# tvlearn/evo

Measured on AMD Instinct MI355X. Metric: E-step candidate-state evals/sec (NxS), full EM iteration, higher is better.
Workload: dtype f64; 1 GPU; ES3C D=256 H=512 S=200 N=100k f64 (north-star shape); algo=es3c, N_total=100000, N_rank0=100000, D=256, H=512, S=200, step=10 full EM iterations, world_size_rccl=1, ea=fit/randflip 10 parents x 1 child x 1 gen, states=p_init_Kn=1/H (init_states default), rng=device, mstep=device, parallelism=dp1

## Files before the change

evo_amd/_lib.py:

```python
import ctypes
import os

import numpy as np

_HERE = os.path.dirname(os.path.abspath(__file__))
LIB_PATH = os.path.join(_HERE, "libevo_amd.so")

MODEL_BSC, MODEL_SSSC = 0, 1

GEN_KEEP = {"s": 1, "z": 2, "y_mean": 4}
GEN_WHAT = {"y": 0, "s": 1, "z": 2, "y_mean": 3}

SEED_INCOMPLETE = 1

PSAMP_KEEP = {"slot": 1, "s": 2, "z": 4, "y": 8}
PSAMP_WHAT = {"slot": 0, "s": 1, "z": 2, "y": 3}

LLE_WHAT = {"s": 0, "inside": 1, "log_r": 2, "lpj": 3}

VALIDITY_BITS = (
    "have_data", "have_params", "have_cand", "B_valid", "rows_fresh", "stats_rows_valid", "yhat_valid", "rec_resident",
    "yrec_valid", "yrec_from_pass", "rec_in_stats", "keep_x_valid", "rec_uses_keep", "need_known", "res_need0",
    "res_need1", "res_need2", "cand_from_device", "lists_clean", "clist_clean", "acc_clean", "wq_copy_valid",
    "h_theta_fresh", "theta_bak_valid", "kn_lost", "last_estep_fused", "reduce_pending", "bins_dirty", "gen_kept",
    "prefetch_current", "census_current", "rows_kn_current",
)
VALIDITY_WORDS = ("gen", "kn_gen", "theta_gen", "pending_skip", "census_skip", "kn_refill", "pred_N")

KERNEL_IDS = {
    "lpj_resident": 0, "lpj_candidates": 1, "lpj_overflow": 2, "row_lse": 3, "vary_kn": 4,
    "stats": 5, "stats_overflow": 6, "gemm_f64": 7, "evolve": 8, "misc": 9, "mstep_device": 10,
    "lpj_pass": 11, "stats_pass": 12, "lpj_k3_4": 13, "lpj_k5_8": 14, "lpj_k9plus": 15,
    "stats_k3_4": 16, "stats_k5_8": 17, "stats_k9plus": 18, "allreduce": 19, "estep_fused": 20,
    "patches": 21, "init_states": 22,
}
KERNEL_IDS_EXTRA = {"posterior_sample": 23, "seed_states": 24, "loglik_proposal": 25, "loglik_lpj": 26, "loglik_fold": 27,
                    "remap_latents": 28}


def kernel_id(name):
    return KERNEL_IDS[name] if name in KERNEL_IDS else KERNEL_IDS_EXTRA[name]

_c_dp = ctypes.POINTER(ctypes.c_double)
_c_u8p = ctypes.POINTER(ctypes.c_uint8)
_c_i32p = ctypes.POINTER(ctypes.c_int32)
_c_u64p = ctypes.POINTER(ctypes.c_uint64)
_vp = ctypes.c_void_p
_I, _I64, _U64, _DBL = ctypes.c_int, ctypes.c_int64, ctypes.c_uint64, ctypes.c_double

SIGNATURES = {
    "evoamd_abi_version": (_I, []),
    "evoamd_last_error": (ctypes.c_char_p, []),
    "evoamd_device_count": (_I, [ctypes.POINTER(_I)]),
    "evoamd_ctx_create": (_I, [_I, ctypes.POINTER(_vp)]),
    "evoamd_ctx_destroy": (None, [_vp]),
    "evoamd_synchronize": (_I, [_vp]),
    "evoamd_debug_live_buffers": (_I, [ctypes.POINTER(_I64)]),
    "evoamd_debug_validity": (_I, [_vp, ctypes.POINTER(_I64)]),
    "evoamd_set_option": (_I, [_vp, ctypes.c_char_p, _I]),
    "evoamd_configure": (_I, [_vp, _I, _I64, _I, _I, _I, _I, _I]),
    "evoamd_upload_data": (_I, [_vp, _c_dp]),
    "evoamd_upload_states": (_I, [_vp, _c_u8p]),
    "evoamd_download_states": (_I, [_vp, _c_u8p]),
    "evoamd_upload_states_packed": (_I, [_vp, _c_u8p, _I64, _I64]),
    "evoamd_download_states_packed": (_I, [_vp, _c_u8p, _I64, _I64]),
    "evoamd_init_states": (_I, [_vp, _DBL, _U64, _I, _c_u8p]),
    "evoamd_seed_states": (_I, [_vp, _I, _c_i32p, _c_dp]),
    "evoamd_seed_states_ex": (_I, [_vp, _I, ctypes.c_uint, _c_i32p, _c_dp]),
    "evoamd_upload_lpj": (_I, [_vp, _c_dp]),
    "evoamd_download_lpj": (_I, [_vp, _c_dp]),
    "evoamd_set_params_bsc": (_I, [_vp, _c_dp, _DBL, _DBL, _c_dp]),
    "evoamd_set_params_sssc": (_I, [_vp, _c_dp, _c_dp, _c_dp, _c_dp, _DBL, _c_dp]),
    "evoamd_lpj_resident": (_I, [_vp]),
    "evoamd_lpj_candidates": (_I, [_vp, _c_u8p, _c_i32p, _I, _c_dp]),
    "evoamd_set_candidates": (_I, [_vp, _c_u8p, _c_i32p, _I, _c_dp]),
    "evoamd_lpj_shared": (_I, [_vp, _c_u8p, _I, _c_dp]),
    "evoamd_lpj_single": (_I, [_vp, _c_dp, _c_u8p, _I, _c_dp, _c_i32p]),
    "evoamd_vary_kn": (_I, [_vp, _I, _c_dp]),
    "evoamd_evolve_randflip": (_I, [_vp, _I, _I, _U64, _I]),
    "evoamd_estep": (_I, [_vp, _I, _I, _U64, _I, _I, ctypes.POINTER(_I)]),
    "evoamd_estep_counters": (_I, [_vp, ctypes.POINTER(_I64)]),
    "evoamd_evolve_states": (_I, [_vp, _I, _I, _I, _I, _I, _U64, _DBL, _DBL]),
    "evoamd_download_candidates": (_I, [_vp, _c_u8p, _c_i32p, _c_dp]),
    "evoamd_refine_states": (_I, [_vp, _I, _I, _I, _I, _I, _I, _U64, _U64, _DBL, _DBL, _I, _I, _I, _DBL, _c_dp,
                                  ctypes.POINTER(_I)]),
    "evoamd_posterior_scores": (_I, [_vp, _c_dp, _c_dp, _c_i32p, _c_i32p, _c_dp]),
    "evoamd_remap_latents": (_I, [_vp, _c_i32p, _I, _c_i32p, ctypes.POINTER(_I64)]),
    "evoamd_adopt_remapped_states": (_I, [_vp]),
    "evoamd_latent_map_counts": (_I, [_vp, ctypes.POINTER(_I64)]),
    "evoamd_acc_size": (_I64, [_vp]),
# ... 94 lines not shown
```

evo_amd/csrc/evo_amd.hip:

```cpp
#include "../../include/evo_amd.h"

#include <dlfcn.h>
#include <math.h>
#include <stdarg.h>
#include <stdio.h>
#include <stdlib.h>
#include <string.h>

#include <atomic>
#include <chrono>
#include <memory>
#include <string>
#include <type_traits>
#include <vector>

#include "common.hpp"
#include "gemm_f64.hpp"
#include "kernels_bsc.hpp"
#include "kernels_common.hpp"
#include "kernels_evolve.hpp"
#include "kernels_mstep.hpp"
#include "kernels_sssc.hpp"
#include "kernels_sssc_quad.hpp"
#include "kernels_fused.hpp"
// ... 67 lines not shown
    h = dlopen(nm, RTLD_NOW | RTLD_LOCAL);
    if (h) break;
  }
  if (!h) return fail(EVOAMD_E_RCCL, "cannot dlopen librccl: %s", dlerror());
  g_rccl.GetUniqueId = (int (*)(RcclId *))dlsym(h, "ncclGetUniqueId");
  g_rccl.CommInitRank = (int (*)(void **, int, RcclId, int))dlsym(h, "ncclCommInitRank");
  g_rccl.AllReduce =
      (int (*)(const void *, void *, size_t, int, int, void *, hipStream_t))dlsym(h, "ncclAllReduce");
  g_rccl.CommDestroy = (int (*)(void *))dlsym(h, "ncclCommDestroy");
  g_rccl.GetErrorString = (const char *(*)(int))dlsym(h, "ncclGetErrorString");
  if (!g_rccl.GetUniqueId || !g_rccl.CommInitRank || !g_rccl.AllReduce || !g_rccl.CommDestroy)
    return fail(EVOAMD_E_RCCL, "librccl is missing a required symbol");
  g_rccl.handle = h;
  return 0;
}
#define RCCL_TRY(expr)                                                                         \
  do {                                                                                         \
    int _r = (expr);                                                                           \
    if (_r != 0)                                                                               \
      return fail(EVOAMD_E_RCCL, "%s failed: %s", #expr,                                       \
                  g_rccl.GetErrorString ? g_rccl.GetErrorString(_r) : "?");                    \
  } while (0)

enum {
  KID_LPJ_RES = 0,
  KID_LPJ_CAND,
  KID_LPJ_OVF,
  KID_ROW_LSE,
  KID_VARY_KN,
  KID_STATS,
  KID_STATS_OVF,
  KID_GEMM,
  KID_EVOLVE,
  KID_MISC,
  KID_MSTEP,
  KID_LPJ_PASS,
  KID_STATS_PASS,
  KID_LPJ_K34,
  KID_LPJ_K58,
  KID_LPJ_K9P,
  KID_STATS_K34,
  KID_STATS_K58,
  KID_STATS_K9P,
  KID_ALLREDUCE,
  KID_ESTEP_FUSED,
  KID_PATCHES,
  KID_INIT_STATES,
  KID_POSTERIOR_SAMPLE,
  KID_SEED_STATES,
  KID_LLE_PROPOSAL,
  KID_LLE_LPJ,
  KID_LLE_FOLD,
  KID_REMAP,
  KID_COUNT
};

struct TimedSpan {
  hipEvent_t a, b;
  int kid;
};

static int sync_streams(evoamd_ctx *c);
static std::atomic<int64_t> g_live_dev{0}, g_live_pinned{0};

template <typename T>
class DevBuf {
  T *p_ = nullptr;
  size_t n_ = 0;

  hipError_t alloc_raw(size_t n) {
    reset();
    if (n == 0) n = 1;
    hipError_t e = hipMalloc((void **)&p_, n * sizeof(T));
    if (e != hipSuccess) {
      p_ = nullptr;
      return e;
    }
    n_ = n;
    g_live_dev++;
    return hipSuccess;
  }

 public:
  DevBuf() = default;
  DevBuf(const DevBuf &) = delete;
  DevBuf &operator=(const DevBuf &) = delete;
  DevBuf(DevBuf &&o) noexcept : p_(o.p_), n_(o.n_) { o.p_ = nullptr, o.n_ = 0; }
  DevBuf &operator=(DevBuf &&o) noexcept {
    if (this != &o) {
      reset();
      p_ = o.p_, n_ = o.n_;
      o.p_ = nullptr, o.n_ = 0;
    }
    return *this;
  }
  ~DevBuf() { reset(); }
  operator T *() const { return p_; }
  T *get() const { return p_; }
  size_t size() const { return n_; }
  void reset() {
    if (p_) {
      (void)hipFree(p_);
      g_live_dev--;
    }
    p_ = nullptr;
    n_ = 0;
// ... 153 lines not shown
  bool use_digest = true;
  bool spd_inverse = true;
  long spd_fallbacks = 0;
  bool rows_fresh = false;
  int model = 0;
  i64 N = 0;
  int D = 0, H = 0, S = 0, S_perm = 0, Cmax = 0, HW = 0, L = 0;
  DevBuf<double> Y, yy, y2sum;
  int ldY = 0;
  PinnedBuf<double> h_acc, h_par;
  PinnedBuf<double> h_theta;
  double *h_theta_dev = nullptr;
  bool h_theta_fresh = false;
  DevBuf<double> theta_bak;
  bool theta_bak_valid = false;
  unsigned long long mbox_seq = 0;
  DevBuf<unsigned> mbox_counter;
  PinnedBuf<int> h_err;
  DevBuf<u64> states, cand;
  DevBuf<u64> dig, cand_dig;
  DevBuf<double> lpj, cand_lpj;
  DevBuf<double> lpj_alt;
  DevBuf<int> cand_counts;
  DevBuf<u64> cand_raw, dupold;
  DevBuf<int> gen_start;
  DevBuf<unsigned> flags;
  DevBuf<double> rowmax, rowsum, partial, partial2, diag;
  DevBuf<uint8_t> stage;
  DevBuf<double> W, Wt, G, Psi, Bm, mus, pilbar_v;
  DevBuf<double2> GP;
  DevBuf<double4> DG;
  DevBuf<double4> D1;
  DevBuf<PairEntry> PT;
  DevBuf<double> pies;
  double *dpar = nullptr;
  PinnedBuf<double> h_dpar;
  DevBuf<double> colpart;
  DevBuf<double> gjwork;
  DevBuf<double> tmpA, tmpB, tmpC;
  double ljc = 0;
  double *acc = nullptr;
  i64 acc_n = 0;
  DevBuf<double> acc_base;
  i64 ovf_n = 0;
  DevBuf<double> Es_own;
  double *Es = nullptr;
  DevBuf<int> list1, list2, list3, list_n, err;
  DevBuf<int> clist, clist_n;
  size_t clist_words() const { return clist.size() / 3; }
  DevBuf<OvfRec> ovf_rec;
  unsigned long long kn_gen = 1, census_gen = 0;
  int census_opt = 1;
  int merge_small = 1;
  int stats_flat = 0;
  int fused_opt = 0;
  DevBuf<double> rowF;
  DevBuf<int> rowcnt, defer;
  DevBuf<double> fpart;
  DevBuf<unsigned long long> fprof;
  bool last_estep_fused = false;
  bool reduce_pending = false;
  long fused_calls = 0, unfused_calls = 0;
  int debug_poison_list = 0;
  int debug_fail_stats = 0;
  int census_skip = 0;
  DevBuf<double> tmp_y, tmp_lpj;
  DevBuf<u64> tmp_states;
  DevBuf<double> exact_buf;
  DevBuf<double> patch_img, patch_Y;
  DevBuf<double> patch_V;
  DevBuf<double> pred_buf, pred_Wt;
  DevBuf<int> pred_status;
  i64 pred_N = 0;
  int pred_D = 0;
  DevBuf<int> ps_slot, ps_status;
  DevBuf<u64> ps_s;
  DevBuf<double> ps_z, ps_y;
  i64 ps_N = 0, ps_T = 0;
  int ps_D = 0, ps_H = 0, ps_keep = -1;
  DevBuf<double> lle_d, lle_keep_d, lle_rho;
  DevBuf<int> lle_i;
  DevBuf<unsigned> lle_flags;
  DevBuf<u64> lle_keep_s, lle_hash;
  DevBuf<uint8_t> lle_keep_in;
  i64 lle_N = 0, lle_T = 0;
  int lle_H = 0, lle_keep = -1;
  DevBuf<uint8_t> codes_buf;
  unsigned long long rows_kn_gen = 0;
  int codes_path = -1;
  int init_home = -1;
  DevBuf<u64> init_scratch;
  DevBuf<double2> seed_gpt;
  DevBuf<double> seed_rows;
  DevBuf<double> refine_trace, score_buf;
  DevBuf<u64> remap_states, remap_dig;
  DevBuf<int> remap_i;
  DevBuf<unsigned long long> remap_sum, map_counts;
  i64 remap_N = 0;
  int remap_S = 0, remap_H = 0;
  bool kn_lost = false;
  i64 kn_refill = 0;
  DevBuf<double> gen_par, gen_y, gen_z, gen_ymean;
  DevBuf<u64> gen_sin, gen_s;
  i64 gen_N = 0;
  int gen_D = 0, gen_H = 0, gen_keep = -1;
  void *comm = nullptr;
  int rank = 0, world = 1;
  bool timing = false;
  unsigned timing_mask = 0xFFFFFFFFu;
  std::vector<TimedSpan> spans;
  std::vector<hipEvent_t> pool;
  double t_ms[KID_COUNT] = {0};
  i64 t_n[KID_COUNT] = {0};
};

static void drop_stats_products(evoamd_ctx *c) { c->yhat_valid = c->stats_rows_valid = c->rec_resident = c->yrec_from_pass = false; }
static void drop_prefetch(evoamd_ctx *c) { c->prefetch_gen = ~0ull; }
static void made_prefetch(evoamd_ctx *c) { c->prefetch_gen = c->gen; }
static void drop_B(evoamd_ctx *c) { c->B_valid = false; }
static void made_B(evoamd_ctx *c) { c->B_valid = true; }
static int next_theta_stamp(evoamd_ctx *c) { return ++c->theta_gen; }

static void on_configure(evoamd_ctx *c) {
  c->gen++;
  c->kn_gen++;
  c->census_gen = 0;
  c->pending_skip = c->census_skip = 0;
  c->have_data = c->have_params = c->have_cand = c->rows_fresh = c->acc_clean = c->clist_clean = false;
  c->h_theta_fresh = c->theta_bak_valid = c->yrec_valid = c->rec_in_stats = c->keep_x_valid = c->kn_lost = false;
  c->lists_clean = c->need_known = c->cand_from_device = false;
  if (c->model == EVOAMD_MODEL_SSSC) c->last_estep_fused = false;
  drop_stats_products(c);
  c->pred_N = 0;
  c->rel_frac = -1.0;
  c->pays_agreed = -1;
}
static void on_option(evoamd_ctx *c) { c->gen++; }
static void on_option_changes_derived(evoamd_ctx *c) { c->have_params = false; }
static void on_data_uploaded(evoamd_ctx *c) {
  c->have_data = true;
  c->gen++;
  c->B_valid = false;
  c->rec_resident = false;
}
static void on_masks_changed(evoamd_ctx *c, bool present) {
  c->yrec_valid = c->rec_resident = c->yrec_from_pass = false;
  if (present) c->B_valid = false;
}
static void on_yrec_uploaded(evoamd_ctx *c) { c->yrec_valid = true, c->rec_resident = c->yrec_from_pass = false; }
static void on_theta_installed(evoamd_ctx *c) {
  c->have_params = true;
  c->gen++;
  c->h_theta_fresh = false;
  drop_stats_products(c);
}
static void on_theta_update_begun(evoamd_ctx *c) { c->gen++; }
static void on_theta_updated(evoamd_ctx *c, bool backup_rode_along) {
  c->B_valid = false;
  if (backup_rode_along) c->theta_bak_valid = true;
  c->stats_rows_valid = false;
}
static void on_theta_restored(evoamd_ctx *c) {
  c->gen++;
  c->h_theta_fresh = false;
  c->B_valid = false;
  c->have_params = true;
  drop_prefetch(c);
}
static void on_theta_update_failed(evoamd_ctx *c) { c->prefetch_gen = ~0ull, c->have_params = false; }
static void made_theta_backup(evoamd_ctx *c) { c->theta_bak_valid = true; }
static void drop_theta_backup(evoamd_ctx *c) { c->theta_bak_valid = false; }
static void made_theta_mailbox(evoamd_ctx *c, bool holds_theta) { c->h_theta_fresh = holds_theta; }
enum KnBy { KN_BY_CALLER, KN_BY_SELECTION };
static void on_kn_changed(evoamd_ctx *c, KnBy by) {
  c->gen++;
  c->kn_gen++;
  if (by == KN_BY_CALLER) c->need_known = false;
}
static void on_kn_complete(evoamd_ctx *c) { c->kn_lost = false; }
static void on_kn_init_begun(evoamd_ctx *c) {
  c->kn_lost = true, c->kn_refill = 0;
  on_kn_changed(c, KN_BY_CALLER);
}
static void on_kn_rows_uploaded(evoamd_ctx *c, i64 n0, i64 n) {
  on_kn_changed(c, KN_BY_CALLER);
  if (c->kn_lost && n0 <= c->kn_refill && n0 + n > c->kn_refill) {
    c->kn_refill = n0 + n;
    if (c->kn_refill >= c->N) c->kn_lost = false;
  }
}
static void on_estep_route(evoamd_ctx *c, bool fused) { c->last_estep_fused = fused; }
static void on_lpj_overwritten(evoamd_ctx *c) { c->rows_fresh = false; }
static void made_row_stats(evoamd_ctx *c) { c->rows_fresh = true; }
static void on_lists_claimed(evoamd_ctx *c) {
  if (!c->lists_clean) c->pending_skip = 0;
  c->lists_clean = false;
}
static void made_clean_lists(evoamd_ctx *c) {
  c->lists_clean = c->model == EVOAMD_MODEL_SSSC;
  if (c->lists_clean) c->pending_skip = 0;
}
static void on_levels_skipped(evoamd_ctx *c, bool census_route, int skipped, int served, bool any) {
  if (census_route) {
    c->census_skip |= skipped;
    if (any && !(served & 2)) c->pending_skip |= 2;
  } else {
    c->pending_skip = (c->pending_skip | skipped) & ~served;
  }
}
static void made_selection(evoamd_ctx *c, bool census_cleared, bool acc_zeroed) {
  made_row_stats(c);
  if (census_cleared) {
    c->clist_clean = true;
    c->census_skip = 0;
  }
  c->acc_clean = acc_zeroed;
  made_clean_lists(c);
}
static void on_census_claimed(evoamd_ctx *c) { c->clist_clean = false, c->census_skip = 0; }
static void made_census(evoamd_ctx *c) { c->census_gen = c->kn_gen; }
static void on_census_poisoned(evoamd_ctx *c) { c->kn_gen++; }
static void on_cand_installed(evoamd_ctx *c, bool near_parents) { c->cand_from_device = near_parents; }
static void made_cand_lpj(evoamd_ctx *c) { c->have_cand = true; }
static void drop_cand_batch(evoamd_ctx *c) { c->have_cand = false, c->cand_from_device = false; }
static void made_fused_estep(evoamd_ctx *c, bool inkernel_census) {
  on_kn_changed(c, KN_BY_SELECTION);
  if (inkernel_census) made_census(c);
  made_row_stats(c);
  c->have_cand = false, c->cand_from_device = true;
  on_estep_route(c, true);
}
static void made_fused_rows(evoamd_ctx *c, bool reduced) { c->reduce_pending = !reduced; }
static void on_bins_append(evoamd_ctx *c) { c->bins_dirty = true; }
static void made_bins_clean(evoamd_ctx *c) { c->bins_dirty = false; }
static void on_stats_pass_begun(evoamd_ctx *c) {
  c->bins_dirty = false;
  c->acc_clean = false;
  drop_stats_products(c);
}
static void made_stats_rows(evoamd_ctx *c) { c->stats_rows_valid = true, c->rows_kn_gen = c->kn_gen; }
static void made_level_hints(evoamd_ctx *c, const double *dpar_host) {
  if (c->model != EVOAMD_MODEL_SSSC) return;
  for (int j = 0; j < 3; j++) {
    c->res_cnt[j] = dpar_host[DP_NGT2 + j];
    c->res_need[j] = c->res_cnt[j] > 0.0;
  }
  c->need_known = true;
}
static void made_wq_copy(evoamd_ctx *c, bool present) { c->wq_copy_valid = present; }
static void made_yhat(evoamd_ctx *c) { c->yhat_valid = true; }
static void made_yrec_from_pass(evoamd_ctx *c, bool in_stats) {
  c->yrec_valid = c->yrec_from_pass = true;
  if (in_stats) c->rec_in_stats = false;
}
static void drop_resident_rec(evoamd_ctx *c) { c->rec_resident = false; }
static void on_keep_mask(evoamd_ctx *c, bool uploaded) { c->keep_x_valid = uploaded; }
static void made_resident_rec(evoamd_ctx *c, bool uses_keep) { c->rec_uses_keep = uses_keep, c->rec_resident = true; }
static void made_predictive(evoamd_ctx *c, i64 N) { c->pred_N = N; }
static void made_generated(evoamd_ctx *c, int keep) { c->gen_keep = keep; }
static void made_posterior_samples(evoamd_ctx *c, int keep) { c->ps_keep = keep; }
static void made_remap(evoamd_ctx *c, i64 N, int S, int H_new) { c->remap_N = N, c->remap_S = S, c->remap_H = H_new; }
static void made_loglik_draws(evoamd_ctx *c, int keep) { c->lle_keep = keep; }

struct SpanGuard {
  evoamd_ctx *c;
  int kid;
  hipStream_t stream;
  hipEvent_t a = nullptr, b = nullptr;
  SpanGuard(evoamd_ctx *ctx, int k, hipStream_t s = nullptr) : c(ctx), kid(k), stream(s ? s : ctx->stream) {
    if (!c->timing || !((c->timing_mask >> k) & 1u)) return;
    auto get = [&]() {
      hipEvent_t e;
      if (!c->pool.empty()) {
        e = c->pool.back();
        c->pool.pop_back();
      } else {
        (void)hipEventCreate(&e);
      }
      return e;
    };
    a = get();
// ... 45 lines not shown
extern "C" int evoamd_device_count(int *count) {
  REQUIRE(count, "count is NULL");
  int n = 0;
  hipError_t e = hipGetDeviceCount(&n);
  if (e != hipSuccess) {
    *count = 0;
    return fail(EVOAMD_E_NODEVICE, "hipGetDeviceCount: %s", hipGetErrorString(e));
  }
  *count = n;
  return 0;
}

static int set_kernel_lds_limits() {
  HIP_TRY(hipFuncSetAttribute((const void *)sssc_stats_flat_kernel, hipFuncAttributeMaxDynamicSharedMemorySize, 150 * 1024));
  HIP_TRY(hipFuncSetAttribute((const void *)sssc_big_kernel<0>, hipFuncAttributeMaxDynamicSharedMemorySize,
                              136 * 1024));
  HIP_TRY(hipFuncSetAttribute((const void *)sssc_big_kernel<0, 0>, hipFuncAttributeMaxDynamicSharedMemorySize,
                              136 * 1024));
  HIP_TRY(hipFuncSetAttribute((const void *)sssc_big_kernel<0, 1>, hipFuncAttributeMaxDynamicSharedMemorySize,
                              136 * 1024));
  HIP_TRY(hipFuncSetAttribute((const void *)sssc_big_kernel<1>, hipFuncAttributeMaxDynamicSharedMemorySize,
                              136 * 1024));
  HIP_TRY(hipFuncSetAttribute((const void *)posterior_codes_kernel<CODES_LDS>, hipFuncAttributeMaxDynamicSharedMemorySize,
                              CODES_WAVES * CODES_LDS_H * (int)sizeof(double)));
  HIP_TRY(hipFuncSetAttribute((const void *)gemm_tn128_f64, hipFuncAttributeMaxDynamicSharedMemorySize,
                              (int)GEMM128_LDS_BYTES));
  HIP_TRY(hipFuncSetAttribute((const void *)gemm_tn128_rows_f64, hipFuncAttributeMaxDynamicSharedMemorySize,
                              (int)GEMM128_LDS_BYTES));
  HIP_TRY(hipFuncSetAttribute((const void *)gemm_tn128_sk_f64, hipFuncAttributeMaxDynamicSharedMemorySize,
                              (int)GEMM128_LDS_BYTES));
  HIP_TRY(hipFuncSetAttribute((const void *)gemm_tn128_sk_f32, hipFuncAttributeMaxDynamicSharedMemorySize,
                              (int)GEMM128_LDS_BYTES));
  HIP_TRY(hipFuncSetAttribute((const void *)gemm_tn128_store_f32, hipFuncAttributeMaxDynamicSharedMemorySize,
                              (int)GEMM128_LDS_BYTES));
  {
    const int lds = (int)(PRED_WAVES * pred_lds_doubles(PRED_MAX_K, true) * sizeof(double));
    const void *pk[] = {(const void *)predictive_kernel<1, true>, (const void *)predictive_kernel<2, true>,
                        (const void *)predictive_kernel<4, true>, (const void *)predictive_kernel<8, true>};
    for (const void *f : pk) HIP_TRY(hipFuncSetAttribute(f, hipFuncAttributeMaxDynamicSharedMemorySize, lds));
    const void *sk[] = {(const void *)posterior_sample_kernel<1, true>, (const void *)posterior_sample_kernel<2, true>,
                        (const void *)posterior_sample_kernel<4, true>, (const void *)posterior_sample_kernel<8, true>};
    for (const void *f : sk) HIP_TRY(hipFuncSetAttribute(f, hipFuncAttributeMaxDynamicSharedMemorySize, lds));
  }
  HIP_TRY(hipFuncSetAttribute((const void *)remap_latents_kernel, hipFuncAttributeMaxDynamicSharedMemorySize, REMAP_LDS_BYTES));
  HIP_TRY(hipFuncSetAttribute((const void *)seed_states_kernel<true>, hipFuncAttributeMaxDynamicSharedMemorySize, 150 * 1024));
  HIP_TRY(hipFuncSetAttribute((const void *)seed_states_kernel<false>, hipFuncAttributeMaxDynamicSharedMemorySize, 150 * 1024));
  HIP_TRY(hipFuncSetAttribute((const void *)seed_states_masked_kernel<true>, hipFuncAttributeMaxDynamicSharedMemorySize, 150 * 1024));
  HIP_TRY(hipFuncSetAttribute((const void *)seed_states_masked_kernel<false>, hipFuncAttributeMaxDynamicSharedMemorySize, 150 * 1024));
  {
    const void *wk[] = {(const void *)sssc_stats_wave_kernel<0, 4>,  (const void *)sssc_stats_wave_kernel<1, 4>,
                        (const void *)sssc_stats_wave_kernel<2, 4>,  (const void *)sssc_stats_wave_kernel<4, 4>,
                        (const void *)sssc_stats_wave_kernel<8, 4>,  (const void *)sssc_stats_wave_kernel<16, 4>,
                        (const void *)sssc_stats_wave_kernel<0, 1>,  (const void *)sssc_stats_wave_kernel<0, 8>,
                        (const void *)sssc_stats_wave_kernel<0, 16>};
    for (const void *f : wk) HIP_TRY(hipFuncSetAttribute(f, hipFuncAttributeMaxDynamicSharedMemorySize, 150 * 1024));
    HIP_TRY(hipFuncSetAttribute((const void *)pair_bins_reduce_kernel, hipFuncAttributeMaxDynamicSharedMemorySize, 3 * PB_TILE * 8));
    HIP_TRY(hipFuncSetAttribute((const void *)sssc_small_kernel<4, 1, 2, 256>, hipFuncAttributeMaxDynamicSharedMemorySize, 120 * 1024));
    HIP_TRY(hipFuncSetAttribute((const void *)sssc_small_kernel<8, 1, 2, 256>, hipFuncAttributeMaxDynamicSharedMemorySize, 120 * 1024));
  }
  {
    const void *fk[] = {(const void *)sssc_estep_fused_kernel<1, false>,  (const void *)sssc_estep_fused_kernel<1, true>,
                        (const void *)sssc_estep_fused_kernel<2, false>,  (const void *)sssc_estep_fused_kernel<2, true>,
                        (const void *)sssc_estep_fused_kernel<4, false>,  (const void *)sssc_estep_fused_kernel<4, true>,
                        (const void *)sssc_estep_fused_kernel<8, false>,  (const void *)sssc_estep_fused_kernel<8, true>,
                        (const void *)sssc_estep_fused_kernel<16, false>, (const void *)sssc_estep_fused_kernel<16, true>};
    for (const void *fp : fk) HIP_TRY(hipFuncSetAttribute(fp, hipFuncAttributeMaxDynamicSharedMemorySize, 160 * 1024));
  }
  return 0;
}

extern "C" int evoamd_ctx_create(int device, evoamd_ctx **out) {
  REQUIRE(out, "out is NULL");
  int n = 0;
  if (hipGetDeviceCount(&n) != hipSuccess || n <= 0)
    return fail(EVOAMD_E_NODEVICE, "no HIP device visible (libevo_amd needs an MI355X / gfx950 GPU)");
  REQUIRE(device >= 0 && device < n, "device index out of range");
  HIP_TRY(hipSetDevice(device));
  hipDeviceProp_t prop;
  HIP_TRY(hipGetDeviceProperties(&prop, device));
  if (strncmp(prop.gcnArchName, "gfx950", 6) != 0)
    return fail(EVOAMD_E_NODEVICE, "device %d is %s; libevo_amd is built for gfx950 only", device,
                prop.gcnArchName);
  std::unique_ptr<evoamd_ctx> guard(new evoamd_ctx());
  evoamd_ctx *c = guard.get();
  c->device = device;
  c->n_cu = prop.multiProcessorCount > 0 ? prop.multiProcessorCount : 256;
  {
    int prio_lo = 0, prio_hi = 0;
    HIP_TRY(hipDeviceGetStreamPriorityRange(&prio_lo, &prio_hi));
    HIP_TRY(hipStreamCreateWithPriority(&c->stream, hipStreamNonBlocking, prio_hi));
    HIP_TRY(hipStreamCreateWithPriority(&c->stream2, hipStreamNonBlocking, prio_lo));
  }
  HIP_TRY(hipEventCreateWithFlags(&c->ev_fork, hipEventDisableTiming));
  HIP_TRY(hipEventCreateWithFlags(&c->ev_join, hipEventDisableTiming));
  HIP_TRY(hipStreamCreateWithFlags(&c->stream_copy, hipStreamNonBlocking));
  HIP_TRY(hipEventCreateWithFlags(&c->ev_theta, hipEventDisableTiming));
  HIP_TRY(hipEventCreateWithFlags(&c->ev_theta_done, hipEventDisableTiming));
  HIP_TRY(hipEventCreateWithFlags(&c->ev_mbox, hipEventDisableTiming));
  HIP_TRY(hipEventCreateWithFlags(&c->ev_bak, hipEventDisableTiming));
  for (int i = 0; i < 16; i++) HIP_TRY(hipEventCreateWithFlags(&c->ev_chunk[i], hipEventDisableTiming));
  TRY(set_kernel_lds_limits());
  *out = guard.release();
  return 0;
}

static int sync_streams(evoamd_ctx *c) {
  for (hipStream_t s : {c->stream, c->stream2, c->stream_copy})
    if (s) HIP_TRY(hipStreamSynchronize(s));
  return 0;
// ... 61 lines not shown
  const char *err = nullptr;
  void (*after)(evoamd_ctx *) = nullptr;
};
#define OPT_INT(f) &evoamd_ctx::f, nullptr
#define OPT_BOOL(f) nullptr, &evoamd_ctx::f
static int opt_flag(int v) { return v != 0; }
static const OptionRow OPTIONS[] = {
    {"sssc_k8", OPT_INT(k8_mode), [](int v) { return v < 0 ? -1 : (int)(v != 0); }},
    {"ebsc_f32", OPT_BOOL(f32_opt), opt_flag},
    {"bsc_direct", OPT_BOOL(bsc_direct), opt_flag, 0, 0, nullptr, nullptr,
     on_option_changes_derived},
    {"reconstruct_in_stats", OPT_BOOL(rec_in_stats), opt_flag},
    {"codes_path", OPT_INT(codes_path), nullptr, -1, CODES_GMEM, nullptr, "codes_path: -1 (auto), 0 registers, 1 LDS, 2 global memory"},
    {"merge_select_fused", OPT_INT(merge_select_fused), opt_flag},
    {"prefetch_lpj", OPT_BOOL(prefetch_lpj), opt_flag},
    {"inverse_block", OPT_INT(spd_block), nullptr, 0, 0, [](int v) { return v == 0 || v == 16 || v == 32; },
     "inverse_block: 0 (auto), 16 or 32"},
    {"overlap_gemm", OPT_INT(overlap_gemm)},
    {"stats_stage", OPT_INT(stats_stage)},
    {"stats_waves", OPT_INT(stats_waves)},
    {"pair_bins", OPT_INT(pair_bins)},
    {"gemm_streamk", OPT_INT(gemm_streamk)},
    {"b_transposed", OPT_INT(b_tn_opt)},
    {"pair_bins_scale", OPT_INT(bins_scale), nullptr, 1, 64, nullptr, "pair_bins_scale: 1 .. 64"},
    {"pair_bins_nwg", OPT_INT(bins_nwg), nullptr, 0, 0, [](int v) { return v >= 256 && v <= 2048 && (v % 256) == 0; },
     "pair_bins_nwg: 256 .. 2048, multiple of 256"},
    {"pair_bins_auto", OPT_INT(bins_auto), opt_flag},
    {"pair_bins_min", OPT_INT(bins_min)},
    {"bsc_stats_wave", OPT_INT(bsc_wave_opt)},
    {"gemm_workspace", OPT_INT(gemm_ws_opt)},
    {"sssc_precision", OPT_INT(sssc_prec32), [](int v) { return (int)(v == 32); }, 0, 0, [](int v) { return v == 64 || v == 32; },
     "sssc_precision: 64 or 32"},
    {"lpj_main_unstaged", OPT_INT(main_unstaged), opt_flag},
    {"lpj_singular_screen", OPT_INT(sing_screen), nullptr, 0, 2, nullptr, "lpj_singular_screen: 0 (never), 1 (automatic) or 2 (always)"},
    {"gemm_grouped", OPT_INT(gemm_grouped), opt_flag},
    {"gemm_per_xcd", OPT_INT(gemm_per_xcd)},
    {"init_states_home", OPT_INT(init_home), nullptr, -1, 1, nullptr, "init_states_home: -1 (auto), 0 LDS, 1 global memory"},
    {"background_unit", OPT_INT(bg_unit), opt_flag},
    {"fold_clear", OPT_INT(fold_clear), opt_flag},
    {"early_fork", OPT_INT(early_fork)},
    {"merge_small_levels", OPT_INT(merge_small), opt_flag},
    {"stats_flat", OPT_INT(stats_flat), opt_flag},
    {"theta_copy_engine", OPT_INT(theta_copy_engine), opt_flag},
    {"census_lists", OPT_INT(census_opt), opt_flag},
    {"sk_spare", OPT_INT(sk_spare), nullptr, -1, 32, nullptr, "sk_spare: -1 (automatic) or 0 .. 32 workgroups per XCD"},
    {"stats_chunks", OPT_INT(stats_chunks), nullptr, 1, 16, nullptr, "stats_chunks: 1 .. 16"},
    {"mailbox_side_stream", OPT_INT(mbox_side), opt_flag},
    {"fused_estep", OPT_INT(fused_opt), nullptr, 0, 2, nullptr, "fused_estep: 0 (never), 1 (automatic) or 2 (whenever the shape allows it)"},
    {"debug_poison_list", OPT_INT(debug_poison_list), opt_flag},
    {"debug_fail_stats", OPT_INT(debug_fail_stats), opt_flag},
    {"state_digest", OPT_BOOL(use_digest), opt_flag},
    {"inverse_spd", OPT_BOOL(spd_inverse), opt_flag},
};
#undef OPT_INT
#undef OPT_BOOL

extern "C" int evoamd_set_option(evoamd_ctx *c, const char *name, int value) {
  REQUIRE(c && name, "bad arguments");
  on_option(c);
  for (const OptionRow &o : OPTIONS) {
    if (strcmp(name, o.name) != 0) continue;
    if (o.err && !(o.accepts ? o.accepts(value) : (value >= o.lo && value <= o.hi))) return fail(EVOAMD_E_INVALID, "%s", o.err);
    const int v = o.norm ? o.norm(value) : value;
    if (o.ifield) c->*o.ifield = v;
    else c->*o.bfield = v != 0;
    if (o.after) o.after(c);
    return 0;
  }
  return fail(EVOAMD_E_INVALID, "unknown option '%s'", name);
}

static int join_fork(evoamd_ctx *c);

extern "C" int evoamd_synchronize(evoamd_ctx *c) {
  REQUIRE(c, "ctx is NULL");
  TRY(join_fork(c));
  HIP_TRY(hipStreamSynchronize(c->stream));
  return 0;
}

static i64 acc_len(const evoamd_ctx *c) {
  const i64 H = c->H, D = c->D;
  return (c->model == EVOAMD_MODEL_BSC) ? H * D + H * H + H + 1 + 8 : 2 * H + 4 * H * H + D * H + D + 8;
}
struct AccLayout {
  i64 Wp, Wq, pies, sigma;
  i64 xs, xss, xsz, xszsz, s_sz, sz_sz, sWp, y2;
  i64 tail;
};
static AccLayout acc_layout(const evoamd_ctx *c) {
  AccLayout a = {};
  const i64 H = c->H, D = c->D;
  if (c->model == EVOAMD_MODEL_BSC) {
    a.Wp = 0;
    a.Wq = H * D;
    a.pies = a.Wq + H * H;
    a.sigma = a.pies + H;
    a.tail = a.sigma + 1;
  } else {
    a.xs = 0;
    a.xss = H;
    a.xsz = a.xss + H * H;
    a.xszsz = a.xsz + H;
    a.sWp = a.xszsz + H * H;
    a.s_sz = a.sWp + D * H;
    a.sz_sz = a.s_sz + H * H;
    a.y2 = a.sz_sz + H * H;
    a.tail = a.y2 + D;
  }
  return a;
}

static int alloc_pair_bins(evoamd_ctx *c, int scale) {
  const i64 N = c->N;
  const int H = c->H, S = c->S;
  c->pb_ent.reset();
  c->pb_gcnt.reset();
  c->pb_part.reset();
  c->pbins = PairBins{};
  c->bins_scale_cur = 0;
  if (H >= 2 && H <= 1024) {
    PairBins pb = {};
    pb.rf = std::max(1, PB_TILE / (2 * H));
    const int nfold = (H - 1 + 1) / 2;
    pb.nb = (int)cdiv(nfold, pb.rf);
    pb.nwg = c->bins_nwg;
    pb.nsh = std::max((i64)N * S >= (i64)8 << 20 ? 8 : 4, std::min(PB_NSH_MAX, 256 / std::max(1, pb.nb)));
    pb.cap = (int)std::max<i64>(64, (i64)scale * cdiv((i64)N * S, (i64)pb.nb * pb.nwg));
    const size_t ne = (size_t)pb.nb * pb.nwg * pb.cap;
    if (c->pb_ent.try_alloc(ne) && c->pb_part.try_alloc((size_t)pb.nb * pb.nsh * 3 * 2 * pb.rf * H) &&
        c->pb_gcnt.try_alloc((size_t)pb.nb * pb.nwg)) {
      pb.ent = c->pb_ent;
      pb.part = c->pb_part;
      pb.gcnt = c->pb_gcnt;
      HIP_TRY(hipMemsetAsync(pb.gcnt, 0, c->pb_gcnt.size() * sizeof(int), c->stream));
      c->pbins = pb;
      c->bins_scale_cur = scale;
      made_bins_clean(c);
    } else {
      c->pb_ent.reset();
      c->pb_part.reset();
      c->pb_gcnt.reset();
    }
  }
  return 0;
}

static int ensure_bins_capacity(evoamd_ctx *c) {
  if (c->model != EVOAMD_MODEL_SSSC || !c->need_known || !c->pbins.ent || c->bins_auto == 0) return 0;
  const double NS = (double)c->N * c->S;
  const double n34 = c->res_cnt[0] - c->res_cnt[1], n58 = c->res_cnt[1] - c->res_cnt[2];
  const double entries = (NS - c->res_cnt[0]) + 6.0 * n34 + 28.0 * n58;
  int want = (int)std::ceil(3.0 * 1.25 * entries / NS);
  if (want > 64) want = 64;
  if (want <= c->bins_scale_cur) return 0;
  HIP_TRY(hipStreamSynchronize(c->stream));
  if (c->stream2) HIP_TRY(hipStreamSynchronize(c->stream2));
  const int before = c->bins_scale_cur;
  TRY(alloc_pair_bins(c, want));
  if (!c->pbins.ent) {
    TRY(alloc_pair_bins(c, before));
    c->bins_auto = 0;
  }
  return 0;
}

static int configure_validate(const evoamd_ctx *c, int model, i64 N, int D, int H, int S, int S_perm, int Cmax) {
  REQUIRE(model == EVOAMD_MODEL_BSC || model == EVOAMD_MODEL_SSSC, "unknown model");
  REQUIRE(N > 0 && D > 0 && H > 0 && S > 0, "N, D, H, S must be positive");
  REQUIRE(S_perm == 0 || S_perm == 1, "S_perm must be 0 or 1");
  REQUIRE(Cmax >= 1 && Cmax <= 64 * VK_MAX_C_PER_LANE, "Cmax must be in [1, 256]");
  REQUIRE(S <= 64 * VK_MAX_S_PER_LANE, "S must be <= 1024");
  REQUIRE((i64)N * (S > Cmax ? S : Cmax) < 2147483647LL, "N * max(S, Cmax) must fit in int32");
  if (model == EVOAMD_MODEL_BSC && c->f32_opt)
    REQUIRE((H % 4) == 0 && (D % 4) == 0, "float32 mode needs H and D to be multiples of 4 (16-byte rows)");
  return 0;
}

static void configure_geometry(evoamd_ctx *c, int model, i64 N, int D, int H, int S, int S_perm, int Cmax) {
  c->model = model;
  c->N = N;
  c->D = D;
  c->H = H;
  c->S = S;
  c->S_perm = S_perm;
  c->Cmax = Cmax;
  c->HW = (H + 63) / 64;
  c->L = S + S_perm;
  c->ldY = (model == EVOAMD_MODEL_SSSC) ? D + 3 * H : D;
  c->f32 = model == EVOAMD_MODEL_BSC && c->f32_opt;
  c->acc_n = acc_len(c);
  c->pre_n = (model == EVOAMD_MODEL_SSSC) ? 4 + (i64)CS_SLICES * 3 * H : 4 + (i64)BSC_CS_SLICES * H;
  c->ovf_n = c->pre_n + ((model == EVOAMD_MODEL_SSSC) ? 2 * (i64)H * H : 0);
}

static void configure_drop(evoamd_ctx *c) {
  for (DevBuf<uint8_t> *b : {&c->mask_infr, &c->mask_x, &c->keep_x, &c->row_any}) b->reset();
  c->Yrec.reset();
  c->cand_raw.reset();
  c->dupold.reset();
  c->gen_start.reset();
  c->tmpWt.reset();
  c->Wt.reset();
  c->init_scratch.reset();
  c->seed_gpt.reset();
  c->seed_rows.reset();
  c->ps_slot.reset();
  c->ps_status.reset();
  c->ps_s.reset();
  c->ps_z.reset();
  c->ps_y.reset();
  made_posterior_samples(c, -1);
  c->lle_d.reset();
  c->lle_keep_d.reset();
  c->lle_rho.reset();
  c->lle_hash.reset();
  c->lle_i.reset();
  c->lle_flags.reset();
  c->lle_keep_s.reset();
  c->lle_keep_in.reset();
  made_loglik_draws(c, -1);
  c->huge.reset();
  c->huge_ctl.reset();
  c->huge_slots = c->huge_kc = 0;
  for (DevBuf<float> *b : {&c->Yf, &c->Ytf, &c->Wf, &c->Bf, &c->Esf}) b->reset();
  c->Yt.reset();
}

static int configure_alloc_common(evoamd_ctx *c) {
  const size_t N = (size_t)c->N, D = (size_t)c->D, H = (size_t)c->H, S = (size_t)c->S, Cmax = (size_t)c->Cmax, HW = (size_t)c->HW;
  TRY(c->Y.alloc(N * c->ldY));
  TRY(c->yy.alloc(N));
  TRY(c->y2sum.alloc(D));
  TRY(c->states.alloc(N * S * HW));
  TRY(c->cand.alloc(N * Cmax * HW));
  if (H <= DIG_MAX_H) {
    TRY(c->dig.alloc(N * S));
    TRY(c->cand_dig.alloc(N * Cmax));
  } else {
    c->dig.reset();
    c->cand_dig.reset();
  }
  TRY(c->lpj.alloc(N * c->L));
  TRY(c->lpj_alt.alloc(N * c->L));
  TRY(c->cand_lpj.alloc(N * Cmax));
// ... 31 lines not shown
  TRY(c->Wt.alloc(H * D));
  TRY(c->Bm.alloc(c->f32 ? 1 : N * H));
  if (c->f32) {
    c->ldYt = ((c->N + 3) / 4) * 4;
    TRY(c->Yf.alloc(N * D));
    TRY(c->Ytf.alloc(D * c->ldYt));
    TRY(c->Wf.alloc(D * H));
    TRY(c->Bf.alloc(N * H));
    TRY(c->Esf.alloc(N * H));
  }
  return 0;
}

static int configure_alloc_es3c(evoamd_ctx *c) {
  const size_t N = (size_t)c->N, H = (size_t)c->H;
  c->Es_own.reset();
  c->Es = c->Y + c->D;
  TRY(c->Psi.alloc(H * H));
  TRY(c->GP.alloc(H * H));
  TRY(c->DG.alloc(H));
  TRY(c->D1.alloc(H));
  TRY(c->PT.alloc(H * H));
  TRY(c->Bm.alloc(N * H));
  TRY(c->mus.alloc(H));
  TRY(c->pilbar_v.alloc(H));
  TRY(c->pies.alloc(H));
  TRY(c->rowF.alloc(N));
  TRY(c->rowcnt.alloc(N));
  TRY(c->defer.alloc(2 * (N + 1) + 2));
  TRY(c->fpart.alloc((size_t)3 * R3_THREADS));
  if (c->H > SSSC_KCAP) {
    const size_t slot = big_slot_doubles(c->H);
    c->huge_kc = c->H;
    c->huge_slots = (int)std::max<size_t>(1, std::min<size_t>(16, ((size_t)256 << 20) / (slot * sizeof(double))));
    TRY(c->huge.alloc(slot * (size_t)c->huge_slots));
    TRY(c->huge_ctl.alloc((size_t)c->huge_slots));
  }
  return 0;
}

static int configure_alloc_lists(evoamd_ctx *c) {
  const size_t words = list_cap(c->N * (i64)std::max(c->S, c->Cmax)) * LIST_SHARDS;
  TRY(c->list1.alloc(words));
  TRY(c->list2.alloc(words));
  TRY(c->list3.alloc(words));
  TRY(c->list_n.alloc(4 * LIST_SHARDS));
  c->clist.reset();
  c->clist_n.reset();
  c->ovf_rec.reset();
  if (c->census_opt) {
    TRY(c->clist.alloc(3 * list_cap(c->N * (i64)c->S) * LIST_SHARDS));
    TRY(c->clist_n.alloc(4 * LIST_SHARDS));
    TRY(c->ovf_rec.alloc((size_t)c->N * c->S));
  }
  return 0;
}

static int configure_alloc_host(evoamd_ctx *c) {
  const size_t par_n = (size_t)c->D * c->H + (size_t)c->H * c->H + 3 * (size_t)c->H;
  if (!c->h_err) TRY(c->h_err.alloc(4));
  if (!c->h_dpar) TRY(c->h_dpar.alloc(DP_COUNT + 8));
  TRY(c->h_acc.alloc((size_t)c->acc_n + DP_COUNT));
  TRY(c->h_par.alloc(par_n));
  c->h_theta_dev = nullptr;
  TRY(c->h_theta.alloc(par_n + MAILBOX_HDR, hipHostMallocCoherent | hipHostMallocMapped));
  memset(c->h_theta, 0, MAILBOX_HDR * sizeof(double));
  HIP_TRY(hipHostGetDevicePointer((void **)&c->h_theta_dev, c->h_theta, 0));
  if (!c->mbox_counter) {
    TRY(c->mbox_counter.alloc(1));
    HIP_TRY(hipMemset(c->mbox_counter, 0, sizeof(unsigned)));
  }
  return 0;
}

static int configure_clear(evoamd_ctx *c) {
  auto zero = [&](auto &b) { return hipMemsetAsync(b.get(), 0, b.size() * sizeof(*b.get()), c->stream); };
  if (c->huge_ctl) HIP_TRY(zero(c->huge_ctl));
  if (c->Yt) HIP_TRY(zero(c->Yt));
  if (c->f32) HIP_TRY(zero(c->Ytf));
  if (c->model == EVOAMD_MODEL_SSSC) {
    HIP_TRY(zero(c->defer));
    if (c->clist_n) HIP_TRY(zero(c->clist_n));
  }
  HIP_TRY(zero(c->Y));
  HIP_TRY(zero(c->flags));
  HIP_TRY(zero(c->cand_counts));
  HIP_TRY(zero(c->acc_base));
  HIP_TRY(zero(c->err));
  HIP_TRY(hipStreamSynchronize(c->stream));
  return 0;
}

extern "C" int evoamd_configure(evoamd_ctx *c, int model, int64_t N, int D, int H, int S, int S_perm,
                                int Cmax) {
  REQUIRE(c, "ctx is NULL");
  c->configured = false;
  TRY(configure_validate(c, model, N, D, H, S, S_perm, Cmax));
  HIP_TRY(hipSetDevice(c->device));
  configure_geometry(c, model, N, D, H, S, S_perm, Cmax);
  configure_drop(c);
  TRY(configure_alloc_common(c));
  if (model == EVOAMD_MODEL_BSC) {
    TRY(configure_alloc_ebsc(c));
  } else {
    TRY(configure_alloc_es3c(c));
    TRY(configure_alloc_lists(c));
// ... 833 lines not shown
static void with_cpl(int Cmax, F &&f) {
  if (Cmax <= 64) f(std::integral_constant<int, 1>{});
  else f(std::integral_constant<int, 4>{});
}

struct Es3cLists {
  ListOut o1, o2, o3;
  ListIn i1, i2, i3;
  ListIn cA, cB, cC;
  ListIn empty;
  ListOut none_out;
  ListIn none_in;
};

static Es3cLists es3c_lists(const evoamd_ctx *c, int cap) {
  Es3cLists ls = {};
  ls.o1 = {c->list1, c->list_n + 0 * LIST_SHARDS, cap};
  ls.o2 = {c->list2, c->list_n + 1 * LIST_SHARDS, cap};
  ls.o3 = {c->list3, c->list_n + 2 * LIST_SHARDS, cap};
  ls.i1 = {ls.o1.items, ls.o1.counts, cap};
  ls.i2 = {ls.o2.items, ls.o2.counts, cap};
  ls.i3 = {ls.o3.items, ls.o3.counts, cap};
  if (c->clist && c->clist_n) {
    ls.cA = {c->clist, c->clist_n, cap};
    ls.cB = {c->clist + c->clist_words(), c->clist_n + LIST_SHARDS, cap};
    ls.cC = {c->clist + 2 * c->clist_words(), c->clist_n + 2 * LIST_SHARDS, cap};
    ls.empty = {c->clist, c->clist_n + 3 * LIST_SHARDS, 0};
  }
  return ls;
}

template <int MODE, int TAG>
static int census_wavefront_levels(evoamd_ctx *c, const SsscArgs &a, const Es3cLists &ls, const bool need[3], bool few4,
                                   const LevelHints &lv, i64 total) {
  if (few4) {
    sssc_big_kernel<MODE, TAG><<<std::max(64u, level_grid(c, lv, 1, total * 256, 1024, 1)), 64, big_lds(SSSC_KCAP), c->stream>>>(
        a, need[1] ? ls.cB : ls.empty, ls.none_out, SSSC_KCAP, need[2] ? ls.cC : ls.empty, ls.i3);
    return 4;
  }
  sssc_big_kernel<MODE, TAG><<<std::max(256u, level_grid(c, lv, 2, total * 256, 8192, 1)), 64, big_lds(16), c->stream>>>(
      a, need[2] ? ls.cC : ls.empty, ls.o2, 16, ls.i3);
  if (!need[2]) return 4;
  sssc_big_kernel<MODE, TAG><<<level_grid(c, lv, 2, total * 256, 1024, 1), 64, big_lds(SSSC_KCAP), c->stream>>>(
      a, ls.i2, ls.none_out, SSSC_KCAP);
  return 2 | 4;
}

#define MAIN_LPJ_LDS_MAX (48 * 1024)

static size_t main_lpj_lds(int C, int H) {
  return ((size_t)(1024 / C + 2) * H + (H <= 512 ? (size_t)4 * H : 0)) * sizeof(double);
}

enum LpjRoute {
  LPJ_MASKED,
  LPJ_CENSUS,
  LPJ_CHAINS,
  LPJ_ROUND2
};
enum LpjMain {
  LPJ_MAIN_NONE,
  LPJ_MAIN_CENSUS,
  LPJ_MAIN_STAGED,
  LPJ_MAIN_UNSTAGED,
  LPJ_MAIN_SMALL
};

struct LpjPlan {
  LpjRoute route;
  LevelHints lv;
  int kid_main;
  i64 total;
  int cap;
  Es3cLists ls;
  bool need[3];
  bool any;
  LpjMain main;
  int rows_cap, stage_dg;
  size_t lds;
  unsigned grid;
  bool few4;
  bool k8;
  bool few_dense;
};

static void lpj_plan(const evoamd_ctx *c, const SsscArgs &a, int tag, const LevelHints &lv, int kid_main, LpjPlan &p) {
  p = LpjPlan{};
  p.lv = lv;
  p.kid_main = kid_main;
  p.total = a.N * (i64)a.C;
  p.cap = (int)list_cap(p.total);
  p.ls = es3c_lists(c, p.cap);
  levels_for(c, lv, p.need);
  p.any = p.need[0] || p.need[1] || p.need[2];
  const bool tables = !a.shared && (a.H % 2) == 0;
  const bool staged = tables && main_lpj_lds(a.C, a.H) <= MAIN_LPJ_LDS_MAX;
  if (a.mask)
    p.route = LPJ_MASKED;
  else if (tag == 0 && a.states == c->states && census_mode(c) && staged)
    p.route = LPJ_CENSUS;
  else
    p.route = c->census_opt ? LPJ_CHAINS : LPJ_ROUND2;
  p.stage_dg = a.H <= 512;
  p.grid = cdiv(p.total, 1024);
  if (staged) {
    p.main = p.route == LPJ_CENSUS ? (lv.levels_only ? LPJ_MAIN_NONE : LPJ_MAIN_CENSUS) : LPJ_MAIN_STAGED;
    p.rows_cap = 1024 / a.C + 2;
    p.lds = main_lpj_lds(a.C, a.H);
  } else if (tables && a.dig && c->main_unstaged) {
    p.main = LPJ_MAIN_UNSTAGED;
    p.lds = (p.stage_dg ? (size_t)4 * a.H : 0) * sizeof(double);
  } else {
    p.main = LPJ_MAIN_SMALL;
    p.grid = cdiv(p.total, 512);
  }
  p.few4 = p.route != LPJ_ROUND2 && few_above4(c, lv);
  p.k8 = p.route == LPJ_ROUND2 && use_k8_kernel(c, lv);
  p.few_dense = p.route == LPJ_ROUND2 && few_dense_states(c, lv);
}

static int lpj_sssc_masked(evoamd_ctx *c, const SsscArgs &a, const LpjPlan &p) {
  SpanGuard g(c, p.kid_main);
  const int gridm = (int)std::min<i64>(p.total, 65536);
  sssc_big_kernel<0><<<gridm, 64, big_lds(8), c->stream>>>(a, p.ls.none_in, p.ls.o3, 8);
  sssc_big_kernel<0><<<1024, 64, big_lds(SSSC_KCAP), c->stream>>>(a, p.ls.i3, p.ls.none_out, SSSC_KCAP);
  HIP_TRY(hipGetLastError());
  return 0;
}

template <int TAG>
static int lpj_sssc_main(evoamd_ctx *c, const SsscArgs &a, const LpjPlan &p) {
  if (p.main == LPJ_MAIN_NONE) return 0;
  SpanGuard g(c, p.kid_main);
  if (p.main == LPJ_MAIN_SMALL)
    sssc_small_kernel<2, 0, TAG, 512><<<p.grid, 512, 0, c->stream>>>(a, p.ls.none_in, p.ls.o1, PairBins{});
  else
    with_hw(a.HW, [&](auto hw) {
      constexpr int HWT = decltype(hw)::value;
      if (p.main == LPJ_MAIN_CENSUS)
        sssc_main_lpj_kernel<TAG, 512, HWT, 2, false><<<p.grid, 512, p.lds, c->stream>>>(a, p.ls.none_out, p.rows_cap, p.stage_dg);
      else if (p.main == LPJ_MAIN_STAGED)
        sssc_main_lpj_kernel<TAG, 512, HWT, 2><<<p.grid, 512, p.lds, c->stream>>>(a, p.ls.o1, p.rows_cap, p.stage_dg);
      else
        sssc_main_lpj_kernel<TAG, 512, HWT, 2, true, false><<<p.grid, 512, p.lds, c->stream>>>(a, p.ls.o1, 0, p.stage_dg);
    });
  HIP_TRY(hipGetLastError());
  DBG_SYNC(c, p.main == LPJ_MAIN_CENSUS ? "sssc lpj main (census)" : "sssc lpj main");
  return 0;
}

template <int TAG>
static int lpj_sssc_census_levels(evoamd_ctx *c, const SsscArgs &a, const LpjPlan &p, int &served) {
  const Es3cLists &ls = p.ls;
  SpanGuard g(c, KID_LPJ_OVF);
  if (p.need[0]) {
    SpanGuard gl(c, KID_LPJ_K34);
    sssc_quad_kernel<1, 0, TAG><<<quad_grid(c, p.lv, 0, p.total, 2048), 256, 0, c->stream>>>(a, ls.cA, ls.none_out, ls.o3, PairBins{}, nullptr);
  }
  DBG_SYNC(c, "sssc lpj quad level 3..4");
  if (p.need[1] && !p.few4) {
    SpanGuard gl(c, KID_LPJ_K58);
    sssc_quad_kernel<2, 0, TAG><<<quad_grid(c, p.lv, 1, p.total, 2048), 256, 0, c->stream>>>(a, ls.cB, ls.none_out, ls.o3, PairBins{}, nullptr);
  }
  DBG_SYNC(c, "sssc lpj quad level 5..8");
  SpanGuard gl(c, KID_LPJ_K9P);
  served = census_wavefront_levels<0, TAG>(c, a, ls, p.need, p.few4, p.lv, p.total);
  HIP_TRY(hipGetLastError());
  DBG_SYNC(c, p.few4 ? "sssc lpj census levels (merged)" : "sssc lpj census levels");
// ... 3 lines not shown
template <int TAG>
static int lpj_sssc_chain_levels(evoamd_ctx *c, const SsscArgs &a, const LpjPlan &p, int &served) {
  const Es3cLists &ls = p.ls;
  SpanGuard g(c, KID_LPJ_OVF);
  if (p.need[0])
    sssc_quad_kernel<1, 0, TAG><<<quad_grid(c, p.lv, 0, p.total, 2048), 256, 0, c->stream>>>(a, ls.i1, ls.o2, ls.o3, PairBins{}, nullptr);
  DBG_SYNC(c, "sssc lpj chain 3..4");
  if (p.few4) {
    sssc_big_kernel<0, TAG><<<std::max(64u, level_grid(c, p.lv, 1, p.total * 256, 1024, 1)), 64, big_lds(SSSC_KCAP), c->stream>>>(
        a, ls.i2, ls.none_out, SSSC_KCAP, ls.i3);
    served = 2 | 4;
  } else {
    if (p.need[1])
      sssc_quad_kernel<2, 0, TAG><<<quad_grid(c, p.lv, 1, p.total, 2048), 256, 0, c->stream>>>(a, ls.i2, ls.o3, ls.o3, PairBins{}, nullptr);
    DBG_SYNC(c, "sssc lpj chain 5..8");
    sssc_big_kernel<0, TAG><<<level_grid(c, p.lv, 2, p.total * 256, 1024, 1), 64, big_lds(SSSC_KCAP), c->stream>>>(
        a, ls.i3, ls.none_out, SSSC_KCAP);
    served = 4;
  }
  HIP_TRY(hipGetLastError());
  DBG_SYNC(c, p.few4 ? "sssc lpj chain wavefront level (merged)" : "sssc lpj chain wavefront level");
  return 0;
}

template <int TAG>
static int lpj_sssc_round2_levels(evoamd_ctx *c, const SsscArgs &a, const LpjPlan &p, int &served) {
  const Es3cLists &ls = p.ls;
  SpanGuard g(c, KID_LPJ_OVF);
  if (p.need[0])
    sssc_small_kernel<4, 0, TAG, 256><<<level_grid(c, p.lv, 0, p.total, 1024, 256), 256, 0, c->stream>>>(a, ls.i1, ls.o2, PairBins{}, ls.o3);
  DBG_SYNC(c, "sssc lpj K=4 level");
  bool merged23 = false;
  if (p.k8) {
    if (p.need[1])
      sssc_small_kernel<8, 0, TAG, 256><<<level_grid(c, p.lv, 1, p.total, 256, 256), 256, 0, c->stream>>>(a, ls.i2, ls.o3, PairBins{}, ls.o3);
  } else if (p.need[1] && p.few_dense) {
    sssc_big_kernel<0, TAG><<<level_grid(c, p.lv, 1, p.total * 256, 1024, 1), 64, big_lds(SSSC_KCAP), c->stream>>>(
        a, ls.i2, ls.none_out, SSSC_KCAP, ls.i3);
    merged23 = true;
  } else if (p.need[1]) {
    sssc_big_kernel<0, TAG><<<level_grid(c, p.lv, 1, p.total * 256, 4096, 1), 64, big_lds(8), c->stream>>>(a, ls.i2, ls.o3, 8);
  }
  DBG_SYNC(c, "sssc lpj K=8 level");
  if ((p.need[2] || c->sing_screen) && !merged23)
    sssc_big_kernel<0, TAG><<<level_grid(c, p.lv, 2, p.total * 256, 1024, 1), 64, big_lds(SSSC_KCAP), c->stream>>>(
        a, ls.i3, ls.none_out, SSSC_KCAP);
  served = (merged23 || p.need[2] || c->sing_screen) ? 4 : 0;
  HIP_TRY(hipGetLastError());
  DBG_SYNC(c, "sssc lpj wavefront level");
  return 0;
}

template <int TAG>
static int launch_sssc_lpj(evoamd_ctx *c, const SsscArgs &a, int kid_main, const LevelHints &lv) {
  TRY(zero_lists(c));
  LpjPlan p;
  lpj_plan(c, a, TAG, lv, kid_main, p);
  if (p.route == LPJ_MASKED) return lpj_sssc_masked(c, a, p);
  if (p.route == LPJ_CENSUS) TRY(ensure_census(c));
  TRY(lpj_sssc_main<TAG>(c, a, p));
  int served = 0;
  if (p.any)
    TRY(p.route == LPJ_CENSUS   ? lpj_sssc_census_levels<TAG>(c, a, p, served)
        : p.route == LPJ_CHAINS ? lpj_sssc_chain_levels<TAG>(c, a, p, served)
                                : lpj_sssc_round2_levels<TAG>(c, a, p, served));
  on_levels_skipped(c, p.route == LPJ_CENSUS, skip_mask(p.need), served, p.any);
  return 0;
}

static int launch_lpj(evoamd_ctx *c, const Batch &b, const LevelHints &lv) {
  if (c->model == EVOAMD_MODEL_BSC) return launch_bsc_lpj(c, b);
  SsscArgs a = sssc_args(c, b);
  if (b.tag == 0) return launch_sssc_lpj<0>(c, a, b.kid, lv);
  if (b.tag == 1) return launch_sssc_lpj<1>(c, a, b.kid, lv);
  return launch_sssc_lpj<2>(c, a, b.kid, lv);
}

static int check_err(evoamd_ctx *c) {
  int *e = c->h_err;
  HIP_TRY(hipMemcpyAsync(e, c->err, 4 * sizeof(int), hipMemcpyDeviceToHost, c->stream));
  HIP_TRY(hipStreamSynchronize(c->stream));
  if (e[0]) {
    HIP_TRY(hipMemsetAsync(c->err, 0, sizeof(int), c->stream));
    if (e[0] & 4) return fail(EVOAMD_E_INVALID, "internal: an ES3C overflow level was skipped although its list was not empty");
    if (e[0] & EVO_ERR_LIST_FULL) return fail(EVOAMD_E_INVALID, "internal: an ES3C overflow list was full, states were dropped");
    if (e[0] & EVO_ERR_BAD_ENTRY) return fail(EVOAMD_E_INVALID, "internal: an ES3C list entry or latent index read back from LDS was out of range");
    if (e[0] & 1) return fail(EVOAMD_E_KLIMIT, "ES3C: a state has more than %d active latents", SSSC_KCAP);
    return fail(EVOAMD_E_SINGULAR, "ES3C: exactly singular k x k system (the reference takes pinv here)");
  }
  return 0;
}

static int lpj_resident_launch(evoamd_ctx *c, double *out, const LevelHints &lv) {
  TRY(ensure_B(c));
  on_lpj_overwritten(c);
  if (c->S_perm) {
    allzero_lpj_kernel<<<cdiv(c->N, 256), 256, 0, c->stream>>>(c->yy, c->N, c->dpar, c->model == EVOAMD_MODEL_SSSC,
                                                               out, c->L, c->flags + 2 * c->N, c->err);
    HIP_TRY(hipGetLastError());
  }
  Batch b = {c->states, nullptr, c->Y, c->Bm, c->yy, c->N, c->S, 0, out, c->L, c->S_perm, c->flags, KID_LPJ_RES, 0};
  b.mask = c->mask_infr;
  SpanGuard pass(c, KID_LPJ_PASS);
  return launch_lpj(c, b, lv);
}

static int estep_resident_pass(evoamd_ctx *c) {
  if (c->prefetch_gen == c->gen) {
    drop_prefetch(c);
    std::swap(c->lpj, c->lpj_alt);
// ... 107 lines not shown
  TRY(c->tmp_lpj.ensure(c, (size_t)C + 2));
  TRY(c->tmp_y.ensure(c, (size_t)c->D + c->H + 2));
  TRY(c->stage.ensure(c, (size_t)C * c->H));
  if (c->model == EVOAMD_MODEL_SSSC) TRY(ensure_lists(c, C));
  double *dy = c->tmp_y, *db = c->tmp_y + c->D, *dyy = c->tmp_y + c->D + c->H;
  unsigned *dfl = (unsigned *)(c->tmp_lpj + C);
  HIP_TRY(hipMemcpyAsync(dy, y, (size_t)c->D * sizeof(double), hipMemcpyHostToDevice, c->stream));
  uint8_t *dmask = nullptr;
  if (x_infr) {
    TRY(c->stage.ensure(c, (size_t)C * c->H + c->D));
    dmask = c->stage + (size_t)C * c->H;
    HIP_TRY(hipMemcpyAsync(dmask, x_infr, (size_t)c->D, hipMemcpyHostToDevice, c->stream));
    mask_apply_kernel<<<cdiv(c->D, 256), 256, 0, c->stream>>>(dy, c->D, dmask, 1, c->D);
  }
  HIP_TRY(hipMemcpyAsync(c->stage, states_bool, (size_t)C * c->H, hipMemcpyHostToDevice, c->stream));
  HIP_TRY(hipMemsetAsync(dfl, 0, sizeof(unsigned), c->stream));
  pack_states_kernel<<<cdiv((i64)C * c->HW, 256), 256, 0, c->stream>>>(c->stage, c->tmp_states, C, c->H, c->HW);
  row_sqnorm_kernel<<<1, 256, 0, c->stream>>>(dy, c->D, 1, c->D, dyy);
  if (c->model == EVOAMD_MODEL_SSSC) TRY(launch_gemm_nn(c, dy, c->D, c->W, c->H, db, c->H, 1, c->H, c->D));
  Batch b = {c->tmp_states, nullptr, dy, db, dyy, 1, C, 1, c->tmp_lpj, C, 0, dfl, KID_MISC, 2};
  b.mask = dmask;
  TRY(launch_lpj(c, b, batch_hints(c, b.tag)));
  unsigned fl = 0;
  HIP_TRY(hipMemcpyAsync(lpj_out, c->tmp_lpj, (size_t)C * sizeof(double), hipMemcpyDeviceToHost, c->stream));
  HIP_TRY(hipMemcpyAsync(&fl, dfl, sizeof(unsigned), hipMemcpyDeviceToHost, c->stream));
  HIP_TRY(hipStreamSynchronize(c->stream));
  if (flags_out) {
    flags_out[0] = (fl & EVO_FLAG_NAN) ? 1 : 0;
    flags_out[1] = (fl & EVO_FLAG_NEGINF) ? 1 : 0;
    flags_out[2] = (fl & (EVO_FLAG_NEGINF | EVO_FLAG_POSINF)) ? 1 : 0;
  }
  if (c->model == EVOAMD_MODEL_SSSC) return check_err(c);
  return 0;
}

extern "C" int evoamd_lpj_single(evoamd_ctx *c, const double *y, const uint8_t *states_bool, int C,
                                 double *lpj_out, int32_t *flags_out) {
  return lpj_single_impl(c, y, nullptr, states_bool, C, lpj_out, flags_out);
}

extern "C" int evoamd_lpj_single_masked(evoamd_ctx *c, const double *y, const uint8_t *x_infr,
                                        const uint8_t *states_bool, int C, double *lpj_out, int32_t *flags_out) {
  REQUIRE(x_infr, "x_infr is NULL");
  return lpj_single_impl(c, y, x_infr, states_bool, C, lpj_out, flags_out);
}

static int estep_select(evoamd_ctx *c, int Mprime, double *sums_out) {
  on_kn_changed(c, KN_BY_SELECTION);
  {
    SpanGuard g(c, KID_VARY_KN);
    int *cl_n = census_mode(c) ? c->clist_n : nullptr;
    const i64 zero_n = c->fold_clear ? (i64)(c->ovf_n + c->acc_n) : 0;
    if (!c->fold_clear) cl_n = nullptr;
    with_spl(c->S, [&](auto spl) {
      with_cpl(c->Cmax, [&](auto cpl) {
        vary_kn_kernel<decltype(spl)::value, decltype(cpl)::value><<<cdiv(c->N, 4), 256, 0, c->stream>>>(
            c->states, c->lpj, c->cand, c->cand_lpj, c->cand_counts, c->N, c->S, c->S_perm, c->HW, c->Cmax, Mprime, c->rowmax,
            c->rowsum, c->partial, c->list_n, 4 * LIST_SHARDS, c->dig, c->cand_dig, (c->use_digest && c->dig) ? 1 : 0,
            c->pending_skip, c->err, cl_n, 4 * LIST_SHARDS, c->census_skip, c->acc_base, zero_n);
      });
    });
    reduce3_partials_kernel<<<1, R3_THREADS, 0, c->stream>>>(c->partial, cdiv(c->N, 4), c->dpar);
    HIP_TRY(hipGetLastError());
    DBG_SYNC(c, "vary_kn");
    made_selection(c, cl_n != nullptr, zero_n > 0);
  }
  if (sums_out) {
    HIP_TRY(hipMemcpyAsync(sums_out, c->dpar + DP_ECNT0, 2 * sizeof(double), hipMemcpyDeviceToHost, c->stream));
    HIP_TRY(hipStreamSynchronize(c->stream));
  }
  return 0;
}

extern "C" int evoamd_vary_kn(evoamd_ctx *c, int Mprime, double *sums_out) {
  REQUIRE(c && c->configured && c->have_cand, "no resident candidate batch (call lpj_candidates / evolve first)");
  TRY(estep_check_mprime(c, Mprime));
  REQUIRE_KN(c);
  HIP_TRY(hipSetDevice(c->device));
  return estep_select(c, Mprime, sums_out);
}

extern "C" int evoamd_set_estep_counts(evoamd_ctx *c, double sum_nunique, double sum_sub) {
  REQUIRE(c && c->configured, "configure first");
  HIP_TRY(hipSetDevice(c->device));
  double v[2] = {sum_nunique, sum_sub};
  HIP_TRY(hipMemcpyAsync(c->dpar + DP_ECNT0, v, sizeof(v), hipMemcpyHostToDevice, c->stream));
  HIP_TRY(hipStreamSynchronize(c->stream));
  return 0;
}

static int estep_children(evoamd_ctx *c, int n_parents, int n_children, uint64_t seed, int fit_parents) {
  {
    SpanGuard g(c, KID_EVOLVE);
    with_spl(c->S, [&](auto spl) {
      evolve_randflip_kernel<decltype(spl)::value><<<cdiv(c->N, 4), 256, 0, c->stream>>>(
          c->states, c->lpj, c->N, c->S, c->S_perm, c->H - c->bg_unit, c->HW, n_parents, n_children, c->Cmax, seed, fit_parents,
          c->cand, c->cand_counts, c->list_n, c->model == EVOAMD_MODEL_SSSC ? 4 * LIST_SHARDS : 0, c->cand_dig, c->pending_skip,
          c->err);
    });
    HIP_TRY(hipGetLastError());
    DBG_SYNC(c, "evolve");
    made_clean_lists(c);
    on_cand_installed(c, true);
  }
  TRY(eval_candidates(c));
  made_cand_lpj(c);
  return 0;
}

extern "C" int evoamd_evolve_randflip(evoamd_ctx *c, int n_parents, int n_children, uint64_t seed, int fit_parents) {
  TRY(estep_check_randflip(c, n_parents, n_children));
  REQUIRE_KN(c);
  HIP_TRY(hipSetDevice(c->device));
  return estep_children(c, n_parents, n_children, seed, fit_parents);
}

static bool fused_shape_ok(const evoamd_ctx *c, int n_parents, int n_children) {
  return c->model == EVOAMD_MODEL_SSSC && c->S_perm == 0 && !c->bg_unit && !c->mask_infr && c->use_digest && c->dig && census_mode(c) &&
// ... 493 lines not shown
  if (c->ar_gemm_pending) {
    c->ar_gemm_pending = false;
    const AccLayout a = acc_layout(c);
    SpanGuard g(c, KID_ALLREDUCE);
    RCCL_TRY(g_rccl.AllReduce(c->acc + a.sWp, c->acc + a.sWp, (size_t)(a.y2 - a.sWp),  8,  0,
                              c->comm, c->stream));
  }
  return 0;
}

static TailArgs make_tail_args(evoamd_ctx *c, const AccLayout &a, i64 N, bool census, int skipped) {
  TailArgs ta = {};
  ta.tail = c->acc + a.tail;
  ta.N = (double)N;
  ta.dpar = c->dpar;
  ta.flags = c->flags;
  ta.nflags3 = 3 * N;
  ta.nper = N;
  ta.err = c->err;
  ta.list_n = c->model == EVOAMD_MODEL_SSSC ? (census ? c->clist_n : c->list_n) : nullptr;
  ta.nshards = LIST_SHARDS;
  ta.skipped_mask = skipped;
  ta.census = c->census;
  ta.census_lists = census ? 1 : 0;
  ta.fly_n = (census && c->model == EVOAMD_MODEL_SSSC) ? c->list_n : nullptr;
  ta.fly_skip = c->pending_skip;
  return ta;
}

static double contraction_flops(const evoamd_ctx *c) {
  return c->model == EVOAMD_MODEL_SSSC ? 2.0 * (double)c->N * (c->D + 2.0 * c->H) * c->H : 2.0 * (double)c->N * c->D * c->H;
}

struct StatsPlan {
  AccLayout a;
  i64 N;
  int H, D;
  bool masked;
  LevelHints lv;
  bool gemm_timed;
  double gemm_flops;
  bool pays;
  bool early;
  bool fork_gemm;
  i64 rpb;
  int nblk;
  int nchunks;
  i64 rows_per_chunk;
  bool second_stream;
  int gemm_spare;
  int waves;
  bool census;
  bool bsc_wave;
};

struct StatsBlock {
  int ci;
  i64 n0, nc;
  int blk0, nblk_c;
};

struct StatsFlow {
  bool early_recorded = false;
  bool tail_done = false;
  bool served3 = false;
  int skipped = 0;
  int bsc_grid = 0;
  PairBins bsc_pb = {};
  PairBins pb = {};
};

struct Es3cPass {
  double *Es, *Ez, *Ed;
  SsscArgs sa = {};
  bool need[3] = {true, true, true};
  Es3cLists ls = {};
};

struct Es3cBlock {
  SsscArgs sc;
  i64 total;
  LevelHints lv;
  int flatG = 0;
  size_t flat_lds = 0;
  bool few4;
};

static bool stats_bins_pay(const evoamd_ctx *c) {
  return c->pbins.ent && (c->pair_bins == 2 || (c->pair_bins == 1 && c->N * (i64)c->S >= (i64)c->bins_min * 1024));
}

static int stats_per_cu(size_t lds_per_wg, int wave_lim) {
  int per_cu = (int)((160 * 1024) / lds_per_wg);
  if (per_cu > wave_lim) per_cu = wave_lim;
  if (per_cu > 8) per_cu = 8;
  if (per_cu < 1) per_cu = 1;
  return per_cu;
}

static int rows_written(evoamd_ctx *c, const StatsPlan &p, StatsFlow &fl) {
  if (p.second_stream && p.nchunks == 1 && p.early && !p.masked) {
    HIP_TRY(hipEventRecord(c->ev_chunk[0], c->stream));
    fl.early_recorded = true;
  }
  return 0;
}

static int reconstruct_rows(evoamd_ctx *c, const char *asked_msg = nullptr) {
  TRY(compute_reconstruction(c));
  if (asked_msg) REQUIRE(c->rec_in_stats, asked_msg);
  select_rec_kernel<<<cdiv(c->N, 4), 256, 0, c->stream>>>(c->Y, c->ldY, c->mask_x, c->mask_infr, c->yhat, c->N, c->D, c->Yrec);
  HIP_TRY(hipGetLastError());
  made_yrec_from_pass(c, true);
  return 0;
}

static int stats_plan(evoamd_ctx *c, bool fork_gemm, StatsPlan &p) {
  p = StatsPlan{};
  p.a = acc_layout(c);
  p.N = c->N;
  p.H = c->H;
  p.D = c->D;
  p.masked = c->mask_infr != nullptr;
  p.lv.known_tag = c->cand_from_device ? 1 : 2;
  p.lv.one_bit = c->cand_from_device;
  p.gemm_timed = c->timing && (c->timing_mask & ((1u << KID_MSTEP) | (1u << KID_MISC) |
                                                 (1u << KID_STATS) | (1u << KID_STATS_OVF)));
  const double gemm_flops = p.gemm_flops = contraction_flops(c);
  bool pays = (c->model == EVOAMD_MODEL_SSSC && gemm_flops >= 8e9) || (c->model == EVOAMD_MODEL_BSC && !c->comm && gemm_flops >= 5e10);
  const bool early = p.early = c->early_fork == 1 || (c->early_fork < 0 && gemm_flops < 2e10);
  if (c->model == EVOAMD_MODEL_SSSC && !c->comm && early && gemm_flops >= 5e8 && !c->mask_infr) pays = true;
  if (c->model == EVOAMD_MODEL_BSC && !c->comm && early && gemm_flops >= 5e8 && !c->mask_infr && c->bsc_wave_opt &&
      dig_for(c, c->states) && cdiv(c->S, 64) <= 4 && (size_t)5 * c->H * sizeof(double) <= 150 * 1024 && !c->f32)
    pays = true;
  if (c->comm && c->model == EVOAMD_MODEL_SSSC) {
    if (c->pays_agreed < 0) {
      double v = pays ? 1.0 : 0.0;
      TRY(evoamd_comm_allreduce_host(c, &v, 1, 1));
      c->pays_agreed = v > 0.0 ? 1 : 0;
    }
    pays = c->pays_agreed == 1;
  }
  p.pays = pays;
  p.fork_gemm = fork_gemm && (c->overlap_gemm == 2 || (c->overlap_gemm == 1 && pays)) &&
                (!c->comm || c->model == EVOAMD_MODEL_SSSC) && !p.gemm_timed && !c->mask_infr;
  p.rpb = ((std::max<i64>(256, cdiv(p.N, 128)) + 3) / 4) * 4;
  p.nblk = (int)cdiv(p.N, p.rpb);
  int nchunks = 1;
  if (!p.masked && !p.gemm_timed && c->overlap_gemm != 0 && c->stats_chunks > 1 && (gemm_flops >= 8e9 || c->overlap_gemm == 2))
    nchunks = std::min<int>(c->stats_chunks, p.nblk);
  p.waves = (c->stats_waves == 4 || c->stats_waves == 8 || c->stats_waves == 16)
                ? c->stats_waves
                : ((size_t)(4 * 2 + 3) * p.H * sizeof(double) <= 150 * 1024 ? 4 : 1);
  p.census = census_mode(c) && !p.masked && p.waves == 4;
  if (p.census) nchunks = 1;
  p.rows_per_chunk = (i64)cdiv(p.nblk, nchunks) * p.rpb;
  p.nchunks = nchunks = (int)cdiv(p.N, p.rows_per_chunk);
  p.second_stream = p.fork_gemm || nchunks > 1;
  {
    const double chain_us = c->H >= 256 ? 15.0 * cdiv(c->H, 32) : 8.5 * cdiv(c->H, 16);
    p.gemm_spare = !(p.fork_gemm && nchunks == 1) ? 0 : ((gemm_flops / 65e6 >= 3.0 * chain_us && c->H <= 512) ? 4 : 8);
  }
  const int SRb = (int)cdiv(c->S, 64);
  p.bsc_wave = c->model == EVOAMD_MODEL_BSC && c->bsc_wave_opt && dig_for(c, c->states) &&
               (SRb == 1 || SRb == 2 || SRb == 4 || SRb == 3) && nchunks == 1 && (size_t)5 * p.H * sizeof(double) <= 150 * 1024;
  return 0;
}

static int stats_bsc_wave(evoamd_ctx *c, const StatsPlan &p, const StatsBlock &blk, StatsFlow &fl) {
  const AccLayout &a = p.a;
  const i64 nc = blk.nc;
  const int H = p.H;
  const u64 *bdig = dig_for(c, c->states);
  const int SRb = (int)cdiv(c->S, 64);
  SpanGuard g(c, KID_STATS);
  const size_t ldsb = (size_t)5 * H * sizeof(double);
  const int per_cu = stats_per_cu(ldsb + 2048, 8);
  PairBins &bsc_pb = fl.bsc_pb;
  bsc_pb = PairBins{};
  if (stats_bins_pay(c)) bsc_pb = c->pbins;
  int sgrid = (int)std::min<i64>(cdiv(nc, 4), (i64)c->n_cu * per_cu * 2);
  if (sgrid > 2048) sgrid = 2048;
  if (bsc_pb.ent && sgrid > bsc_pb.nwg) sgrid = bsc_pb.nwg;
  PB_GRID_CHECK(bsc_pb, sgrid);
  if (bsc_pb.ent) on_bins_append(c);
  fl.bsc_grid = sgrid;
  void *EsP = c->f32 ? (void *)c->Esf : (void *)c->Es;
  double *csb = c->acc_base + 4;
#define BSC_WAVE(SR)                                                                                                      \
  bsc_stats_wave_kernel<SR><<<sgrid, 256, ldsb, c->stream>>>(c->states, c->lpj, c->rowmax, c->rowsum, c->yy, nc, c->S,     \
                                                            c->S_perm, H, c->HW, c->dpar, EsP, c->acc + a.Wq, c->partial2, \
                                                            bdig, c->f32 ? 1 : 0, bsc_pb, csb)
  if (SRb == 1) BSC_WAVE(1);
  else if (SRb == 2) BSC_WAVE(2);
  else BSC_WAVE(4);
#undef BSC_WAVE
  HIP_TRY(hipGetLastError());
  DBG_SYNC(c, "bsc stats (wave)");
  TRY(rows_written(c, p, fl));
  if (bsc_pb.ent) {
    pair_bins_reduce_kernel<<<bsc_pb.nb * bsc_pb.nsh, PB_RTHREADS, (size_t)3 * 2 * bsc_pb.rf * H * sizeof(double), c->stream>>>(
        bsc_pb, H, 0);
    HIP_TRY(hipGetLastError());
    made_bins_clean(c);
  }
  return 0;
}

static int stats_bsc_classic(evoamd_ctx *c, const StatsPlan &p, const StatsBlock &blk) {
  const AccLayout &a = p.a;
  const i64 n0 = blk.n0, nc = blk.nc;
  const int H = p.H;
  {
    SpanGuard g(c, KID_STATS);
    with_hw(c->HW, [&](auto hw) {
      bsc_stats_kernel<decltype(hw)::value><<<cdiv(nc, 4), 256, (size_t)4 * H * sizeof(double), c->stream>>>(
          c->states + (size_t)n0 * c->S * c->HW, c->lpj + (size_t)n0 * c->L, c->rowmax + n0, c->rowsum + n0, c->yy + n0, nc,
          c->S, c->S_perm, H, c->HW, c->dpar,
          c->f32 ? (void *)(c->Esf + (size_t)n0 * H) : (void *)(c->Es + (size_t)n0 * H), c->acc + a.Wq, c->partial2 + n0 / 4,
          dig_for(c, c->states) ? dig_for(c, c->states) + (size_t)n0 * c->S : nullptr, c->f32 ? 1 : 0);
    });
    HIP_TRY(hipGetLastError());
    DBG_SYNC(c, "bsc stats");
  }
  {
    SpanGuard g(c, KID_MISC);
    if (c->f32)
      colsum_partial_f32_kernel<<<dim3(cdiv(H, 64), blk.nblk_c), 256, 0, c->stream>>>(c->Esf + (size_t)n0 * H, H, nc, H, p.rpb,
                                                                                      c->colpart + (size_t)blk.blk0 * H);
    else
      colsum_partial_kernel<<<dim3(cdiv(H, 64), blk.nblk_c), 256, 0, c->stream>>>(c->Es + (size_t)n0 * H, H, nc, H, p.rpb,
                                                                                  c->colpart + (size_t)blk.blk0 * H);
    HIP_TRY(hipGetLastError());
  }
  return 0;
}

static int stats_bsc_block(evoamd_ctx *c, const StatsPlan &p, const StatsBlock &blk, StatsFlow &fl, const double *&Ywp, int &ldwp) {
  TRY(p.bsc_wave ? stats_bsc_wave(c, p, blk, fl) : stats_bsc_classic(c, p, blk));
  if (p.masked) {
    if (c->rec_in_stats) {
      TRY(reconstruct_rows(c));
    }
    REQUIRE(c->yrec_valid, "incomplete data: the M-step needs y_reconstructed (bsc.py:186); reconstruct or upload it");
    Ywp = c->Yrec;
    ldwp = p.D;
  }
  return 0;
}

static int stats_sssc_masked_block(evoamd_ctx *c, const StatsPlan &p, const Es3cPass &ep) {
  const i64 N = p.N;
  const int H = p.H;
  const i64 total = N * (i64)c->S;
// ... 46 lines not shown
static int stats_sssc_census_quads(evoamd_ctx *c, const StatsPlan &p, const Es3cPass &ep, const Es3cBlock &eb, StatsFlow &fl) {
  const bool *need = ep.need;
  const PairBins &pb = fl.pb;
  TRY(ensure_census(c));
  if (need[0] || need[1]) {
    SpanGuard g(c, KID_STATS_OVF);
    const unsigned gcap = pb.ent ? (unsigned)std::min(2048, pb.nwg) : 2048u;
    const size_t dl = (size_t)p.H * sizeof(double);
    if (need[0]) {
      SpanGuard gl(c, KID_STATS_K34);
      const unsigned qg = quad_grid(c, eb.lv, 0, eb.total, gcap);
      PB_GRID_CHECK(pb, qg);
      sssc_quad_kernel<1, 1, 2><<<qg, 256, dl, c->stream>>>(eb.sc, ep.ls.cA, ep.ls.none_out, ep.ls.o3, pb, c->ovf_rec);
    }
    if (need[1] && !eb.few4) {
      SpanGuard gl(c, KID_STATS_K58);
      const unsigned qg = quad_grid(c, eb.lv, 1, eb.total, gcap);
      PB_GRID_CHECK(pb, qg);
      sssc_quad_kernel<2, 1, 2><<<qg, 256, dl, c->stream>>>(eb.sc, ep.ls.cB, ep.ls.none_out, ep.ls.o3, pb, c->ovf_rec);
    }
    HIP_TRY(hipGetLastError());
    DBG_SYNC(c, "sssc stats quad levels");
  }
  return 0;
}

static int stats_sssc_main(evoamd_ctx *c, const StatsPlan &p, const Es3cPass &ep, const Es3cBlock &eb, const StatsBlock &blk,
                           StatsFlow &fl) {
  const PairBins &pb = fl.pb;
  const SsscArgs &sc = eb.sc;
  const ListOut &o1 = ep.ls.o1;
  const i64 nc = blk.nc;
  const int H = p.H;
  const bool census = p.census;
  if (eb.flatG >= 1) {
    SpanGuard g(c, KID_STATS);
    int fgrid = (int)std::min<i64>(cdiv(nc, eb.flatG), (i64)c->n_cu);
    if (pb.ent && fgrid > pb.nwg) fgrid = pb.nwg;
    PB_GRID_CHECK(pb, fgrid);
    sssc_stats_flat_kernel<<<fgrid, FLAT_T, eb.flat_lds, c->stream>>>(sc, pb, c->ovf_rec, eb.flatG);
    HIP_TRY(hipGetLastError());
    DBG_SYNC(c, "sssc stats main (flat)");
    return 0;
  }
  const int Wv = p.waves;
  size_t lds = (size_t)(Wv * 2 + 3) * H * sizeof(double);
  const size_t lds_static = 1024 + (size_t)Wv * 512 + 128;
  REQUIRE(lds <= 150 * 1024, "ES3C statistics: H too large for the LDS rows (H <= 3800)");
  const size_t lds_staged = lds + (size_t)(Wv + 4) * H * sizeof(double);
  const int stage = (H % 2) == 0 && 2 * (lds_staged + lds_static) <= 160 * 1024 && c->stats_stage != 0;
  if (stage) lds = lds_staged;
  const int per_cu = stats_per_cu(lds + lds_static, 32 / Wv);
  SpanGuard g(c, KID_STATS);
  int sgrid = (int)std::min<i64>(cdiv(nc, Wv), (i64)c->n_cu * per_cu * 4);
  if (pb.ent && sgrid > pb.nwg) sgrid = pb.nwg;
  PB_GRID_CHECK(pb, sgrid);
  auto wave4 = [&](auto hw) {
    constexpr int HWT = decltype(hw)::value;
    if (census)
      sssc_stats_wave_kernel<HWT, 4, true><<<sgrid, 256, lds, c->stream>>>(sc, o1, pb, stage, c->ovf_rec, eb.few4 ? 4 : 8);
    else
      sssc_stats_wave_kernel<HWT, 4><<<sgrid, 256, lds, c->stream>>>(sc, o1, pb, stage);
  };
  REQUIRE(!census || Wv == 4, "census lists need the 4-wave statistics kernel (option stats_waves)");
  if (Wv == 1) {
    sssc_stats_wave_kernel<0, 1><<<sgrid, 64, lds, c->stream>>>(sc, o1, pb, stage);
  } else if (Wv == 8) {
    sssc_stats_wave_kernel<0, 8><<<sgrid, 512, lds, c->stream>>>(sc, o1, pb, stage);
  } else if (Wv == 16) {
    sssc_stats_wave_kernel<0, 16><<<sgrid, 1024, lds, c->stream>>>(sc, o1, pb, stage);
  } else if (!stage || !sc.dig) {
    wave4(std::integral_constant<int, 0>{});
  } else {
    with_hw(c->HW, wave4);
  }
  HIP_TRY(hipGetLastError());
  DBG_SYNC(c, "sssc stats main");
  return 0;
}

static int stats_sssc_census_levels(evoamd_ctx *c, const Es3cPass &ep, const Es3cBlock &eb) {
  const bool *need = ep.need;
  if (need[0] || need[1] || need[2]) {
    SpanGuard g(c, KID_STATS_OVF);
    SpanGuard gl(c, KID_STATS_K9P);
    const int served = census_wavefront_levels<1, 2>(c, eb.sc, ep.ls, need, eb.few4, eb.lv, eb.total);
    on_levels_skipped(c, true, 0, served, true);
    HIP_TRY(hipGetLastError());
    DBG_SYNC(c, "sssc stats wavefront level (census)");
  }
  return 0;
}

static int stats_sssc_chain_levels(evoamd_ctx *c, const StatsPlan &p, const Es3cPass &ep, const Es3cBlock &eb, StatsFlow &fl) {
  const bool *need = ep.need;
  const PairBins &pb = fl.pb;
  const SsscArgs &sc = eb.sc;
  const i64 total = eb.total;
  const LevelHints &lv = eb.lv;
  if (need[0] || need[1] || need[2]) {
    SpanGuard g(c, KID_STATS_OVF);
    const size_t cs_lds = sc.cs ? (size_t)3 * p.H * sizeof(double) : 0;
    bool merged23 = false;
    if (need[0]) {
      const unsigned g4 = pb_clamp(pb, level_grid(c, lv, 0, total, 1024, 256));
      PB_GRID_CHECK(pb, g4);
      sssc_small_kernel<4, 1, 2, 256><<<g4, 256, cs_lds, c->stream>>>(sc, ep.ls.i1, ep.ls.o2, pb, ep.ls.o3);
    }
    if (c->k8_mode == 1) {
      if (need[1]) {
        const unsigned g8 = pb_clamp(pb, level_grid(c, lv, 1, total, 256, 256));
        PB_GRID_CHECK(pb, g8);
        sssc_small_kernel<8, 1, 2, 256><<<g8, 256, cs_lds, c->stream>>>(sc, ep.ls.i2, ep.ls.o3, pb, ep.ls.o3);
      }
    } else if (need[1] && few_dense_states(c, lv)) {
      sssc_big_kernel<1><<<level_grid(c, lv, 1, total * 256, 1024, 1), 64, big_lds(SSSC_KCAP), c->stream>>>(
          sc, ep.ls.i2, ep.ls.none_out, SSSC_KCAP, ep.ls.i3);
      fl.served3 = true;
      merged23 = true;
    } else if (need[1]) {
      sssc_big_kernel<1><<<level_grid(c, lv, 1, total * 256, 4096, 1), 64, big_lds(8), c->stream>>>(sc, ep.ls.i2, ep.ls.o3, 8);
    }
    if ((need[2] || c->sing_screen) && !merged23) {
      sssc_big_kernel<1><<<level_grid(c, lv, 2, total * 256, 1024, 1), 64, big_lds(SSSC_KCAP), c->stream>>>(
          sc, ep.ls.i3, ep.ls.none_out, SSSC_KCAP);
      fl.served3 = true;
    }
    HIP_TRY(hipGetLastError());
    DBG_SYNC(c, "sssc stats overflow levels");
  }
  return 0;
}

static int stats_sssc_block(evoamd_ctx *c, const StatsPlan &p, const Es3cPass &ep, const StatsBlock &blk, StatsFlow &fl,
                            bool debug_fail) {
  PairBins &pb = fl.pb;
  const Es3cBlock eb = sssc_block_setup(c, p, ep, blk);
  if (pb.ent) on_bins_append(c);
  if (blk.ci > 0) {
    census_lists_kernel<<<1, 256, 0, c->stream>>>(c->list_n, LIST_SHARDS, skip_mask(ep.need), c->err, c->census);
    HIP_TRY(hipGetLastError());
  }
  if (eb.flatG >= 1 && pb.ent) {
    const i64 per_bin = (i64)pb.nwg * pb.cap;
    pb.nwg = std::min(pb.nwg, c->n_cu);
    pb.cap = (int)std::min<i64>(per_bin / pb.nwg, 1 << 30);
  }
  if (p.census) TRY(stats_sssc_census_quads(c, p, ep, eb, fl));
  TRY(stats_sssc_main(c, p, ep, eb, blk, fl));
  if (debug_fail)
    return fail(EVOAMD_E_INVALID, "debug_fail_stats: statistics pass stopped after its main kernel");
  TRY(p.census ? stats_sssc_census_levels(c, ep, eb) : stats_sssc_chain_levels(c, p, ep, eb, fl));
  TRY(rows_written(c, p, fl));
  if (pb.ent) {
    SpanGuard g(c, KID_STATS);
    pair_bins_reduce_kernel<<<pb.nb * pb.nsh, PB_RTHREADS, (size_t)3 * 2 * pb.rf * p.H * sizeof(double), c->stream>>>(pb, p.H, blk.ci > 0);
    HIP_TRY(hipGetLastError());
    made_bins_clean(c);
    DBG_SYNC(c, "pair bins reduce");
  }
  fl.skipped = skip_mask(ep.need) & ~(fl.served3 ? 4 : 0);
  return 0;
}

static int stats_finish(evoamd_ctx *c, const StatsPlan &p, const Es3cPass &ep, StatsFlow &fl) {
  const AccLayout &a = p.a;
  const i64 N = p.N;
  const int H = p.H, D = p.D;
  const bool masked = p.masked;
  SpanGuard g(c, KID_MISC);
  if (c->model == EVOAMD_MODEL_BSC) {
    TailArgs ta = {};
    if (p.nchunks == 1 && !masked && !c->reduce_pending) {
      ta = make_tail_args(c, a, N, false, fl.skipped);
      fl.tail_done = true;
    }
    double *wq_copy = (!c->comm && !masked && c->tmpA) ? c->tmpA : nullptr;
    made_wq_copy(c, wq_copy != nullptr);
    const unsigned fgrid = cdiv((i64)H * H, 256) + (fl.tail_done ? 1 : 0);
    if (p.bsc_wave)
      bsc_finish_kernel<<<fgrid, 256, 0, c->stream>>>(c->acc + a.Wq, c->acc + a.pies, c->acc_base + 4, BSC_CS_SLICES, H,
                                                       c->partial2, fl.bsc_grid, c->acc + a.sigma, fl.bsc_pb, ta, wq_copy);
    else
      bsc_finish_kernel<<<fgrid, 256, 0, c->stream>>>(c->acc + a.Wq, c->acc + a.pies, c->colpart, p.nblk, H, c->partial2,
                                                       cdiv(N, 4), c->acc + a.sigma, PairBins{}, ta, wq_copy);
  } else {
    const SsscArgs &sa = ep.sa;
    const i64 nthr = (i64)H * H > D ? (i64)H * H : D;
    TailArgs ta = {};
    if (p.nchunks == 1 && !masked && !c->reduce_pending) {
      ta = make_tail_args(c, a, N, p.census, fl.skipped);
      fl.tail_done = true;
    }
    sssc_finish_kernel<<<cdiv(nthr, 256) + (fl.tail_done ? 1 : 0), 256, 0, c->stream>>>(
        c->acc + a.xss, c->acc + a.xszsz, c->acc + a.xs, c->acc + a.xsz, masked ? c->colpart : sa.cs,
        masked ? p.nblk : CS_SLICES, H, c->y2sum, c->acc + a.y2, D, sa.xss_o, sa.xszsz_o, masked ? nullptr : c->PT, fl.pb, ta);
  }
  HIP_TRY(hipGetLastError());
  DBG_SYNC(c, "colsum + finish");
  return 0;
}

static int stats_contract_block(evoamd_ctx *c, const StatsPlan &p, const Es3cPass &ep, const StatsBlock &blk, const StatsFlow &fl,
                                const double *Ywp, int ldwp) {
  const AccLayout &a = p.a;
  const i64 n0 = blk.n0, nc = blk.nc;
  const int H = p.H, D = p.D, ci = blk.ci;
  GemmTnOpts o;
  if (p.second_stream) {
    if (!fl.early_recorded) HIP_TRY(hipEventRecord(c->ev_chunk[ci], c->stream));
    HIP_TRY(hipStreamWaitEvent(c->stream2, c->ev_chunk[ci], 0));
    o.stream = c->stream2;
    o.spare = c->sk_spare >= 0 ? c->sk_spare : p.gemm_spare;
  }
  o.c_is_zero = true;
  o.accumulate = p.nchunks > 1;
  o.mirror = ci == p.nchunks - 1;
  if (c->model == EVOAMD_MODEL_BSC && c->f32)
    return launch_gemm_tn_f32(c, c->Esf + (size_t)n0 * H, H, c->Yf + (size_t)n0 * D, D, c->acc + a.Wp, D, H, D, nc, o);
  if (c->model == EVOAMD_MODEL_BSC)
    return launch_gemm_tn(c, c->Es + (size_t)n0 * H, H, Ywp + (size_t)n0 * ldwp, ldwp, c->acc + a.Wp, D, H, D, nc, o);
  o.sym_row0 = ((D + H) % GEMM_BM) == 0 ? D + H : -1;
  return launch_gemm_tn(c, c->Y + (size_t)n0 * c->ldY, c->ldY, ep.Ez + (size_t)n0 * c->ldY, c->ldY, c->acc + a.sWp, H,
                        D + 2 * H, H, nc, o);
}

static int stats_sssc_masked_products(evoamd_ctx *c, const StatsPlan &p, const Es3cPass &ep) {
  const AccLayout &a = p.a;
  const int H = p.H, D = p.D;
  TRY(reconstruct_rows(c, "ES3C on incomplete data needs do_reconstruction in every step (sssc.py:630-633)"));
  GemmTnOpts o;
  o.c_is_zero = true;
  o.sym_row0 = (H % GEMM_BM) == 0 ? H : -1;
  TRY(launch_gemm_tn(c, ep.Es, c->ldY, ep.Ez, c->ldY, c->acc + a.sWp + (size_t)D * H, H, 2 * H, H, p.N, o));
  o.sym_row0 = -1;
  return launch_gemm_tn(c, c->Yrec, D, ep.Ez, c->ldY, c->acc + a.sWp, H, D, H, p.N, o);
}

static int stats_epilogue(evoamd_ctx *c, const StatsPlan &p, const StatsFlow &fl) {
  const AccLayout &a = p.a;
  const i64 N = p.N;
  if (p.second_stream) {
    HIP_TRY(hipEventRecord(c->ev_join, c->stream2));
    if (p.fork_gemm)
      c->gemm_forked = true;
    else
      HIP_TRY(hipStreamWaitEvent(c->stream, c->ev_join, 0));
  }
  TRY(flush_reduce(c));
  {
    SpanGuard g(c, KID_MISC);
    if (!fl.tail_done) tail_kernel<<<1, 256, 0, c->stream>>>(make_tail_args(c, a, N, p.census, fl.skipped));
    HIP_TRY(hipGetLastError());
    DBG_SYNC(c, "stats contraction + tail");
    made_clean_lists(c);
    if (c->model == EVOAMD_MODEL_SSSC && c->mask_infr) {
      masked_sqsum_kernel<<<256, 256, 0, c->stream>>>(c->yhat, c->mask_infr, N * (i64)p.D, c->acc + a.tail + 7);
      HIP_TRY(hipGetLastError());
    }
  }
  if (c->comm && c->gemm_forked) {
    SpanGuard g(c, KID_ALLREDUCE);
    RCCL_TRY(g_rccl.AllReduce(c->acc, c->acc, (size_t)a.sWp,  8,  0, c->comm, c->stream));
    RCCL_TRY(g_rccl.AllReduce(c->acc + a.y2, c->acc + a.y2, (size_t)(c->acc_n - a.y2), 8, 0, c->comm, c->stream));
    c->ar_gemm_pending = true;
  } else if (c->comm) {
    SpanGuard g(c, KID_ALLREDUCE);
    RCCL_TRY(g_rccl.AllReduce(c->acc, c->acc, (size_t)c->acc_n,  8,  0, c->comm, c->stream));
  }
  return 0;
}

static int stats_sssc_pass(evoamd_ctx *c, const StatsPlan &p, Es3cPass &ep) {
  const AccLayout &a = p.a;
  const i64 N = p.N;
  const int H = p.H, D = p.D;
  ep.Es = c->model == EVOAMD_MODEL_SSSC ? c->Y + D : c->Es;
  ep.Ez = c->Y + D + H;
  ep.Ed = c->Y + D + 2 * H;
  if (c->model != EVOAMD_MODEL_SSSC) return 0;
  SsscArgs &sa = ep.sa;
  Batch b = {c->states, nullptr, c->Y, c->Bm, c->yy, N, c->S, 0, nullptr, c->L, c->S_perm, c->flags, KID_STATS, 0};
  b.mask = c->mask_infr;
  sa = sssc_args(c, b);
  sa.lpj_in = c->lpj;
  sa.rowmax = c->rowmax;
  sa.rowsum = c->rowsum;
  sa.Es = ep.Es;
  sa.Ez = ep.Ez;
  sa.Ed = ep.Ed;
  sa.ldE = c->ldY;
  sa.xss = c->acc + a.xss;
  sa.xszsz = c->acc + a.xszsz;
  sa.xss_o = c->acc_base + c->pre_n;
  sa.xszsz_o = c->acc_base + c->pre_n + (size_t)H * H;
  if (!p.masked) sa.cs = c->acc_base + 4;
  ep.ls = es3c_lists(c, (int)list_cap(N * (i64)c->S));
  levels_for(c, p.lv, ep.need);
  return zero_lists(c);
}

static int stats_compute(evoamd_ctx *c, bool fork_gemm = false) {
  REQUIRE(c && c->configured && c->have_data && c->have_params, "configure, upload_data and set_params first");
  REQUIRE_KN(c);
  StatsPlan p;
  TRY(stats_plan(c, fork_gemm, p));
  TRY(join_fork(c));
  HIP_TRY(hipSetDevice(c->device));
  TRY(ensure_bins_capacity(c));
  if (c->bins_dirty && c->pbins.gcnt)
    HIP_TRY(hipMemsetAsync(c->pbins.gcnt, 0, (size_t)c->pbins.nb * c->pbins.nwg * sizeof(int), c->stream));
  const bool debug_fail = c->debug_fail_stats != 0;
  c->debug_fail_stats = 0;
  if (!c->acc_clean)
    HIP_TRY(hipMemsetAsync(c->acc_base, 0, (size_t)(c->ovf_n + c->acc_n) * sizeof(double), c->stream));
  on_stats_pass_begun(c);
  TRY(ensure_B(c));
  if (!c->rows_fresh) {
    TRY(row_lse(c, c->lpj, p.N, c->L, c->rowmax, c->rowsum, c->dpar + DP_FS));
  }
  StatsFlow fl;
  std::unique_ptr<SpanGuard> pass(new SpanGuard(c, KID_STATS_PASS));
  TRY(c->colpart.ensure(c, (size_t)p.nblk * (c->model == EVOAMD_MODEL_BSC ? p.H : 3 * p.H)));
  Es3cPass ep;
  TRY(stats_sssc_pass(c, p, ep));
  const double *Ywp = c->Y;
  int ldwp = c->ldY;
  if (c->model == EVOAMD_MODEL_SSSC && !p.masked && stats_bins_pay(c)) fl.pb = c->pbins;
  for (int ci = 0; ci < p.nchunks; ci++) {
    const i64 n0 = (i64)ci * p.rows_per_chunk;
    const i64 nc = std::min<i64>(p.rows_per_chunk, p.N - n0);
    const StatsBlock blk = {ci, n0, nc, (int)(n0 / p.rpb), (int)cdiv(nc, p.rpb)};
    TRY(c->model == EVOAMD_MODEL_BSC ? stats_bsc_block(c, p, blk, fl, Ywp, ldwp)
        : p.masked                   ? stats_sssc_masked_block(c, p, ep)
                                     : stats_sssc_block(c, p, ep, blk, fl, debug_fail));
    if (ci == p.nchunks - 1) {
      TRY(stats_finish(c, p, ep, fl));
      pass.reset();
    }
    if (c->model == EVOAMD_MODEL_SSSC && p.masked) continue;
    TRY(stats_contract_block(c, p, ep, blk, fl, Ywp, ldwp));
  }
  if (c->model == EVOAMD_MODEL_SSSC && p.masked) TRY(stats_sssc_masked_products(c, p, ep));
  TRY(stats_epilogue(c, p, fl));
  made_stats_rows(c);
  return 0;
}

extern "C" int evoamd_stats(evoamd_ctx *c, double *acc_out) {
  REQUIRE(acc_out, "acc_out is NULL");
  TRY(stats_compute(c));
  HIP_TRY(hipMemcpyAsync(c->h_acc, c->acc, ((size_t)c->acc_n + DP_COUNT) * sizeof(double), hipMemcpyDeviceToHost,
                         c->stream));
  const int r = check_err(c);
  if (c->sssc_prec32 && c->model == EVOAMD_MODEL_SSSC) {
    const AccLayout a = acc_layout(c);
    for (i64 i = 0; i < a.sWp; i++) c->h_acc[i] = (double)(float)c->h_acc[i];
    for (i64 i = a.s_sz; i < a.y2; i++) c->h_acc[i] = (double)(float)c->h_acc[i];
  }
  memcpy(acc_out, c->h_acc, (size_t)c->acc_n * sizeof(double));
  if (!r) made_level_hints(c, c->h_acc + c->acc_n);
  return r;
}

static int launch_inverse_pivoted(evoamd_ctx *c, double *A, double *B, int n) {
  if (n <= GJR_N) {
    gj_inverse_reg_kernel<<<B ? 2 : 1, MS_T, 0, c->stream>>>(A, B, n, c->dpar + DP_STATUS);
    HIP_TRY(hipGetLastError());
    return 0;
  }
  double *mats[2] = {A, B};
  const dim3 ugrid(cdiv(n, 64), cdiv(n, 64));
  if (n <= 1024) {
    const int nmat = B ? 2 : 1;
    GjMats gm;
    gm.a[0] = A;
    gm.a[1] = B ? B : A;
    gm.w[0] = c->gjwork;
    gm.w[1] = c->gjwork + (size_t)n * n;
    double *Dp = c->gjwork + (size_t)2 * n * n;
    double *Pn = Dp + (size_t)64 * n;
// ... 1590 lines not shown
  TRY(d.alloc((size_t)n));
  HIP_TRY(hipMemcpyAsync(d, buf, (size_t)n * sizeof(double), hipMemcpyHostToDevice, c->stream));
  int rc = g_rccl.AllReduce(d, d, (size_t)n, 8, op == 1 ? 2 : 0, c->comm, c->stream);
  if (rc != 0) return fail(EVOAMD_E_RCCL, "ncclAllReduce failed: %s", g_rccl.GetErrorString ? g_rccl.GetErrorString(rc) : "?");
  HIP_TRY(hipMemcpyAsync(buf, d, (size_t)n * sizeof(double), hipMemcpyDeviceToHost, c->stream));
  HIP_TRY(hipStreamSynchronize(c->stream));
  return 0;
}

extern "C" int evoamd_comm_destroy(evoamd_ctx *c) {
  REQUIRE(c, "ctx is NULL");
  if (c->comm) {
    HIP_TRY(hipStreamSynchronize(c->stream));
    RCCL_TRY(g_rccl.CommDestroy(c->comm));
    c->comm = nullptr;
    c->world = 1;
    c->rank = 0;
  }
  return 0;
}

extern "C" int evoamd_timing_enable(evoamd_ctx *c, int on) {
  REQUIRE(c, "ctx is NULL");
  if (!on && c->timing) TRY(resolve_spans(c));
  c->timing = on != 0;
  c->timing_mask = (unsigned)on;
  return 0;
}

extern "C" int evoamd_timing_reset(evoamd_ctx *c) {
  REQUIRE(c, "ctx is NULL");
  TRY(resolve_spans(c));
  for (int i = 0; i < KID_COUNT; i++) {
    c->t_ms[i] = 0;
    c->t_n[i] = 0;
  }
  return 0;
}

extern "C" int evoamd_kernel_time_ms(evoamd_ctx *c, int kid, double *avg_ms, int64_t *launches) {
  REQUIRE(c && kid >= 0 && kid < KID_COUNT, "bad kernel id");
  TRY(resolve_spans(c));
  if (avg_ms) *avg_ms = c->t_n[kid] ? c->t_ms[kid] / (double)c->t_n[kid] : 0.0;
  if (launches) *launches = c->t_n[kid];
  return 0;
}

extern "C" const char *evoamd_kernel_name(int kid) {
  static const char *names[KID_COUNT] = {"lpj_resident", "lpj_candidates", "lpj_overflow", "row_lse",  "vary_kn",
                                         "stats",        "stats_overflow", "gemm_f64",     "evolve",   "misc", "mstep_device",
                                         "lpj_pass",     "stats_pass",     "lpj_k3_4",     "lpj_k5_8", "lpj_k9plus",
                                         "stats_k3_4",   "stats_k5_8",     "stats_k9plus", "allreduce",    "estep_fused",
                                         "patches",      "init_states",    "posterior_sample", "seed_states",
                                         "loglik_proposal", "loglik_lpj",  "loglik_fold",     "remap_latents"};
  return (kid >= 0 && kid < KID_COUNT) ? names[kid] : "?";
}
```

evo_amd/csrc/kernels_common.hpp:

```cpp
#pragma once
#include "common.hpp"
#include "kernels_mstep.hpp"

__device__ __forceinline__ void clear_lists_checked(int *__restrict__ list_n, int n_list, int skipped_mask,
                                                    int *__restrict__ err) {
  const int per = n_list / 4;
  for (int i = threadIdx.x; i < n_list; i += blockDim.x) {
    if (skipped_mask && list_n[i] != 0 && ((skipped_mask >> (i / per)) & 1)) atomicOr(err, 4);
    list_n[i] = 0;
  }
}

__global__ __launch_bounds__(256) void census_lists_kernel(int *__restrict__ list_n, int nshards, int skipped_mask,
                                                           int *__restrict__ err, double *__restrict__ census) {
  __shared__ int lvl[3];
  if (threadIdx.x < 3) lvl[threadIdx.x] = 0;
  __syncthreads();
  for (int i = threadIdx.x; i < 3 * nshards; i += 256) {
    const int v = list_n[i];
    if (v) atomicAdd(&lvl[i / nshards], v);
  }
  __syncthreads();
  if (threadIdx.x < 3) {
    if (lvl[threadIdx.x] != 0 && ((skipped_mask >> threadIdx.x) & 1)) atomicOr(err, 4);
// ... 354 lines not shown
#pragma unroll
  for (int i = 0; i < HW2; i++) v[i] = s2[i];
  u64 h = 0;
#pragma unroll
  for (int i = 0; i < HW2; i++) {
    h = (h ^ v[i].x) * 0x9E3779B97F4A7C15ull + (u64)(2 * i);
    h = (h ^ v[i].y) * 0x9E3779B97F4A7C15ull + (u64)(2 * i + 1);
  }
  return h;
}
__device__ __forceinline__ u64 hash_state(const u64 *sw, int HW) {
  switch (HW) {
    case 2: return hash_state_fixed<1>(sw);
    case 4: return hash_state_fixed<2>(sw);
    case 8: return hash_state_fixed<4>(sw);
    case 16: return hash_state_fixed<8>(sw);
    default: break;
  }
  u64 h = 0;
  if ((HW & 1) == 0) {
    const ulonglong2 *s2 = (const ulonglong2 *)sw;
    for (int w = 0; w < HW; w += 2) {
      const ulonglong2 v = s2[w >> 1];
      h = (h ^ v.x) * 0x9E3779B97F4A7C15ull + (u64)w;
      h = (h ^ v.y) * 0x9E3779B97F4A7C15ull + (u64)(w + 1);
    }
  } else {
    for (int w = 0; w < HW; w++) h = (h ^ sw[w]) * 0x9E3779B97F4A7C15ull + (u64)w;
  }
  return h;
}

#define VK_MAX_S_PER_LANE 16
#define VK_MAX_C_PER_LANE 4

__device__ __forceinline__ double readlane_f64(double v, int src) {
  const int lo = __builtin_amdgcn_readlane(__double2loint(v), src);
  const int hi = __builtin_amdgcn_readlane(__double2hiint(v), src);
  return __hiloint2double(hi, lo);
}

template <int SPL, int CPL>
__global__ __launch_bounds__(256) void vary_kn_kernel(u64 *__restrict__ states, double *__restrict__ lpj,
                                                      const u64 *__restrict__ cand,
                                                      const double *__restrict__ cand_lpj,
                                                      const int *__restrict__ counts, i64 N, int S,
                                                      int S_perm, int HW, int Cmax, int Mprime,
                                                      double *__restrict__ rowmax,
                                                      double *__restrict__ rowsum, double *__restrict__ fpartial,
                                                      int *__restrict__ list_n, int n_list,
                                                      u64 *__restrict__ dig, const u64 *__restrict__ cand_dig,
                                                      int dig_dedup, int skipped_mask, int *__restrict__ err,
                                                      int *__restrict__ clist_n = nullptr, int n_clist = 0, int census_skip = 0,
                                                      double *__restrict__ zero_ptr = nullptr, i64 zero_n = 0) {
  __shared__ int blk_uniq[4], blk_sub[4];
  if (blockIdx.x == 0 && list_n)
    clear_lists_checked(list_n, n_list, skipped_mask, err);
  if (blockIdx.x == 0 && clist_n) clear_lists_checked(clist_n, n_clist, census_skip, err);
  for (i64 i = (i64)blockIdx.x * 256 + threadIdx.x; i < zero_n; i += (i64)gridDim.x * 256) zero_ptr[i] = 0.0;
  __shared__ double wsum[4];
  __shared__ double new_v[4][64 * CPL];
  __shared__ int new_i[4][64 * CPL], old_i[4][64 * CPL];
  const int lane = lane_id(), wave = wave_id_uniform();
  const i64 n = (i64)blockIdx.x * 4 + wave;
  int n_uniq = 0, n_sub = 0;
  double f = 0.0;
  if (n < N) {
    const int L = S + S_perm;
    u64 *st_n = states + n * (i64)S * HW;
    double *lpj_n = lpj + n * L + S_perm;
    const u64 *cd_n = cand + n * (i64)Cmax * HW;
    const double *cl_n = cand_lpj + n * (i64)Cmax;
    int cnt = counts[n];
    if (cnt > Cmax) cnt = Cmax;
    double nv_raw[CPL], ov[SPL];
#pragma unroll
    for (int q = 0; q < CPL; q++) {
      const int c = lane + 64 * q;
      nv_raw[q] = (c < cnt) ? cl_n[c] : 0.0;
    }
#pragma unroll
    for (int q = 0; q < SPL; q++) {
      const int s = lane + 64 * q;
      ov[q] = (s < S) ? lpj_n[s] : 0.0;
    }
    u64 oh[SPL], ch[CPL];
#pragma unroll
    for (int q = 0; q < SPL; q++) {
      const int s = lane + 64 * q;
      u64 h = 0;
      if (s < S) h = dig_dedup ? dig[n * (i64)S + s] : hash_state(st_n + (i64)s * HW, HW);
      oh[q] = h;
    }
#pragma unroll
    for (int q = 0; q < CPL; q++) {
      const int c = lane + 64 * q;
      u64 h = 0;
      if (c < cnt) h = dig_dedup ? cand_dig[n * (i64)Cmax + c] : hash_state(cd_n + (i64)c * HW, HW);
      ch[q] = h;
    }
    u64 zero_hash = 0;
    for (int w = 0; w < HW; w++) zero_hash = (zero_hash ^ 0ull) * 0x9E3779B97F4A7C15ull + (u64)w;
    if (dig_dedup) zero_hash = 0;
    bool keep[CPL];
#pragma unroll
    for (int q = 0; q < CPL; q++) keep[q] = false;
    for (int c = 0; c < cnt; c++) {
// ... 68 lines not shown
      }
#pragma unroll
      for (int q = 0; q < CPL; q++) {
        const int c = lane + 64 * q;
        if (c < cnt && keep[q] && nrank[q] < M) {
          new_v[wave][nrank[q]] = nv[q];
          new_i[wave][nrank[q]] = c;
        }
      }
      __builtin_amdgcn_wave_barrier();
      __threadfence_block();
      int g = 0;
      {
        double ow[SPL];
#pragma unroll
        for (int q = 0; q < SPL; q++) ow[q] = (lane + 64 * q < S) ? ov[q] : INFINITY;
        for (int j = 0; j < M; j++) {
          double lm = ow[0];
#pragma unroll
          for (int q = 1; q < SPL; q++) lm = fmin(lm, ow[q]);
          const double gm = wave_min(lm);
          if (!(new_v[wave][j] > gm)) break;
          unsigned gi = 0xFFFFFFFFu;
#pragma unroll
          for (int q = 0; q < SPL; q++) {
            const u64 hit = __ballot(ow[q] == gm);
            if (gi == 0xFFFFFFFFu && hit != 0ull) gi = (unsigned)(64 * q + __ffsll((long long)hit) - 1);
          }
          if (lane == 0) old_i[wave][j] = (int)gi;
#pragma unroll
          for (int q = 0; q < SPL; q++)
            if ((unsigned)(lane + 64 * q) == gi) ow[q] = INFINITY;
          g++;
        }
      }
      __builtin_amdgcn_wave_barrier();
      __threadfence_block();
      n_sub = g;
#pragma unroll
      for (int q = 0; q < CPL; q++) {
        const int j = lane + 64 * q;
        if (j < g) {
          const int bi = new_i[wave][j], wi = old_i[wave][j];
          for (int w0 = 0; w0 < HW; w0 += 8) {
            u64 cv[8];
#pragma unroll
            for (int u = 0; u < 8; u++) cv[u] = (w0 + u < HW) ? cd_n[(i64)bi * HW + w0 + u] : 0ull;
#pragma unroll
            for (int u = 0; u < 8; u++)
              if (w0 + u < HW) st_n[(i64)wi * HW + w0 + u] = cv[u];
          }
          lpj_n[wi] = new_v[wave][j];
          if (dig) dig[n * (i64)S + wi] = cand_dig[n * (i64)Cmax + bi];
        }
      }
      for (int j = 0; j < g; j++) {
        const int wi = old_i[wave][j];
        const double v = new_v[wave][j];
#pragma unroll
        for (int q = 0; q < SPL; q++)
          if (lane + 64 * q == wi) ov[q] = v;
      }
    }
    double m = -INFINITY;
#pragma unroll
    for (int q = 0; q < SPL; q++)
      if (lane + 64 * q < S) m = fmax(m, ov[q]);
    const double perm = S_perm ? lpj_n[-1] : -INFINITY;
    if (S_perm && lane == 0) m = fmax(m, perm);
    m = wave_max(m);
    const double B = 0.0 - m;
    double z = 0.0;
#pragma unroll
    for (int q = 0; q < SPL; q++)
      if (lane + 64 * q < S) z += exp(ov[q] + B);
    if (S_perm && lane == 0) z += exp(perm + B);
    z = wave_sum(z);
    f = log(z) - B;
    if (lane == 0) {
      rowmax[n] = m;
      rowsum[n] = z;
    }
  }
  if (lane == 0) {
    blk_uniq[wave] = n_uniq;
    blk_sub[wave] = n_sub;
    wsum[wave] = f;
  }
  __syncthreads();
  if (threadIdx.x == 0) {
    const i64 nb = gridDim.x;
    fpartial[blockIdx.x] = ((wsum[0] + wsum[1]) + wsum[2]) + wsum[3];
    fpartial[nb + blockIdx.x] = (double)(blk_uniq[0] + blk_uniq[1] + blk_uniq[2] + blk_uniq[3]);
    fpartial[2 * nb + blockIdx.x] = (double)(blk_sub[0] + blk_sub[1] + blk_sub[2] + blk_sub[3]);
  }
}
```

evo_amd/csrc/kernels_sssc.hpp:

```cpp
#pragma once
#include "common.hpp"
#include "kernels_mstep.hpp"
#include "pair_bins.hpp"

struct __attribute__((aligned(64))) PairEntry {
  double g01;
  double L;
  double l00, l01, l10, l11;
  double pad[2];
};
__device__ __forceinline__ bool pair_singular_L(double L) { return L == __builtin_inf(); }
__device__ __forceinline__ bool pair_singular_lam(double l00) { return !(fabs(l00) <= 1.7976931348623157e308); }

struct __attribute__((aligned(16))) OvfRec {
  unsigned short idx[8];
  double qn;
  double pad;
  double z[8];
};
static_assert(sizeof(OvfRec) == 96, "OvfRec is six 16-byte loads");

#define CS_SLICES 16
struct SsscArgs {
  const u64 *states;
  const u64 *dig;
  const int *counts;
  const double *Bm;
  const double *yy;
  const double2 *GP;
  const double4 *DG;
  const double4 *D1;
  const PairEntry *PT;
  const double *mus;
  const double *pil_bar;
  double s2inv;
  const double *dpar;
  i64 N;
  int C;
  int shared;
  int H, HW;
  double *lpj_out;
  int ldo, col0;
  unsigned *flags;
  const double *lpj_in;
  const double *rowmax, *rowsum;
  double *Es, *Ez, *Ed;
  int ldE;
  double *cs;
  double *xss, *xszsz;
  double *xss_o, *xszsz_o;
  int *err;
  const int *sing_gen;
  int gen, screen;
  double *huge;
  int *huge_ctl;
  int huge_slots, huge_kc;
  const uint8_t *mask;
  const double *Wt;
  int D;
};

#define SSSC_KCAP 64

__device__ __forceinline__ bool sssc_exact_mode(const SsscArgs &a) {
  return a.screen == 2 || (a.screen == 1 && a.sing_gen != nullptr && *a.sing_gen == a.gen);
}

__device__ __forceinline__ bool lu2_exactly_singular(double a00, double a01, double a10, double a11) {
  const bool swap = fabs(a10) > fabs(a00);
  const double piv = swap ? a10 : a00, low = swap ? a00 : a10;
  if (piv == 0.0) return true;
  const double prow = swap ? a11 : a01, lrow = swap ? a01 : a11;
  const double l = __dmul_rn(low, __ddiv_rn(1.0, piv));
  return __dsub_rn(lrow, __dmul_rn(l, prow)) == 0.0;
}
__device__ __forceinline__ void pinv2_deficient(double a00, double a01, double a10, double a11, double &p00, double &p01,
                                                double &p10, double &p11) {
  const double f2 = a00 * a00 + a01 * a01 + a10 * a10 + a11 * a11;
  const double r = f2 > 0.0 ? 1.0 / f2 : 0.0;
  p00 = a00 * r;
  p01 = a10 * r;
  p10 = a01 * r;
  p11 = a11 * r;
}

__device__ __forceinline__ void pair_lam_singular_psi(double s, double G00, double G01, double G10, double G11, double P00,
                                                      double P01, double P10, double P11, double &l00, double &l01,
                                                      double &l10, double &l11) {
  double q00, q01, q10, q11;
  pinv2_deficient(P00, P01, P10, P11, q00, q01, q10, q11);
  const double M00 = s * G00 + q00, M01 = s * G01 + q01, M10 = s * G10 + q10, M11 = s * G11 + q11;
  if (lu2_exactly_singular(M00, M01, M10, M11)) {
    pinv2_deficient(M00, M01, M10, M11, l00, l01, l10, l11);
  } else {
    const double rm = 1.0 / (M00 * M11 - M01 * M10);
    l00 = M11 * rm;
    l01 = -M01 * rm;
    l10 = -M10 * rm;
    l11 = M00 * rm;
  }
}
// ... 492 lines not shown
      const int cw = __popcll(bits);
      if (cw) {
        const int h0 = __clzll((long long)bits);
        if (ktot == 0) idx0 = i * 64 + h0; else idx1 = i * 64 + h0;
        if (cw >= 2 && ktot == 0) idx1 = i * 64 + __clzll((long long)(bits & ~(0x8000000000000000ull >> h0)));
        ktot += cw;
      }
    }
  }
}

template <int BS, int PPT = 1>
__device__ __forceinline__ void append_begin(const ListOut &lo, int shard, const int (&value)[PPT],
                                             const bool (&over)[PPT], int *buf , int *ctl) {
  if (threadIdx.x == 0) ctl[0] = 0;
  lds_barrier();
#pragma unroll
  for (int p = 0; p < PPT; p++) {
    const u64 mask = __ballot(over[p]);
    if (mask != 0ull) {
      const int lane = lane_id();
      const int leader = __ffsll((long long)mask) - 1;
      int base = 0;
      if (lane == leader) base = atomicAdd(&ctl[0], __popcll(mask));
      base = __shfl(base, leader, 64);
      if (over[p]) buf[base + __popcll(mask & ((1ull << lane) - 1ull))] = value[p];
    }
  }
  lds_barrier();
  if (threadIdx.x == 0) {
    const int n = ctl[0];
    ctl[1] = n ? atomicAdd(&lo.counts[shard], n) : 0;
  }
}
template <int BS>
__device__ __forceinline__ void append_begin(const ListOut &lo, int shard, int value, bool over, int *buf, int *ctl) {
  const int v[1] = {value};
  const bool o[1] = {over};
  append_begin<BS, 1>(lo, shard, v, o, buf, ctl);
}
template <int BS>
__device__ __forceinline__ void append_end(const ListOut &lo, int shard, const int *buf, const int *ctl, int *err = nullptr) {
  lds_barrier();
  const int n = ctl[0], start = ctl[1];
  if (n == 0) return;
  if (start < 0 || start + n > lo.cap) {
    if (err && threadIdx.x == 0) atomicOr(err, EVO_ERR_LIST_FULL);
    return;
  }
  const i64 dst = (i64)shard * lo.cap + start;
  for (int i = threadIdx.x; i < n; i += BS) lo.items[dst + i] = buf[i];
}

__device__ __forceinline__ double sssc_k2_value(const int k, const int idx0, const int idx1, const double4 *D1t, const double *Bn,
                                                const PairEntry &pe, const double yyn, const double s, int *err) {
#pragma clang fp contract(off)
  double4 d0 = make_double4(0.0, 0.0, 0.0, 0.0), d1 = make_double4(0.0, 0.0, 0.0, 0.0);
  double b0 = 0.0, b1 = 0.0, g01 = 0.0, L = 0.0, l00 = 0.0, l01 = 0.0, l10 = 0.0, l11 = 0.0;
  if (k >= 1) {
    d0 = D1t[idx0];
    b0 = Bn[idx0];
    L = d0.y;
    l00 = d0.w;
  }
  if (k == 2) {
    d1 = D1t[idx1];
    b1 = Bn[idx1];
    g01 = pe.g01;
    L = pe.L;
    l00 = pe.l00;
    l01 = pe.l01;
    l10 = pe.l10;
    l11 = pe.l11;
    if (pair_singular_L(pe.L) && pair_singular_lam(pe.l00)) atomicOr(err, 2);
  }
  const double v0 = fma(-g01, d1.x, fma(-d0.z, d0.x, b0));
  const double v1 = fma(-d1.z, d1.x, fma(-g01, d0.x, b1));
  const double rr = fma(-d1.x, b1 + v1, fma(-d0.x, b0 + v0, yyn));
  const double t0 = fma(l01, v1, l00 * v0), t1 = fma(l11, v1, l10 * v0);
  const double quad = fma(v1, t1, v0 * t0);
  return fma(-0.5 * s, fma(-s, quad, rr), L);
}

template <int TAG, int BS, int HWT, int PPT, bool APPEND = true, bool STAGEB = true>
__global__ __launch_bounds__(BS) void sssc_main_lpj_kernel(SsscArgs a, ListOut lo, int rows_cap, int stage_dg) {
  a.s2inv = a.dpar[DP_S2INV];
  extern __shared__ double smem[];
  __shared__ int ovf_buf[BS * PPT];
  __shared__ int ovf_ctl[2];
  double *Bs = smem;
  double4 *DGs = (double4 *)(smem + (STAGEB ? (size_t)rows_cap * a.H : 0));
  const i64 total = a.N * (i64)a.C;
  const i64 t0 = (i64)blockIdx.x * (BS * PPT);
  const i64 n_first = t0 / a.C;
  i64 n_last = (t0 + BS * PPT - 1) / a.C;
  if (n_last > a.N - 1) n_last = a.N - 1;
  const int rows = (int)(n_last - n_first + 1);
  bool live[PPT], over[PPT];
  int nloc[PPT], c[PPT], ktot[PPT], idx0[PPT], idx1[PPT], tv[PPT];
  double yyn[PPT];
  const float rC = 1.0f / (float)a.C;
#pragma unroll
  for (int p = 0; p < PPT; p++) {
    const i64 t = t0 + threadIdx.x + (i64)p * BS;
    tv[p] = (int)t;
    live[p] = t < total;
    nloc[p] = c[p] = ktot[p] = idx0[p] = idx1[p] = 0;
    yyn[p] = 0.0;
    if (live[p]) {
      const int off = (int)(t - n_first * a.C);
      int r = (int)(((float)off + 0.5f) * rC);
      if (r * a.C > off) r--;
      if ((r + 1) * a.C <= off) r++;
      nloc[p] = r;
      c[p] = off - r * a.C;
      live[p] = !(a.counts && c[p] >= a.counts[n_first + r]);
    }
  }
  u64 dgv[PPT];
#pragma unroll
  for (int p = 0; p < PPT; p++) {
    dgv[p] = 0ull;
    if (a.dig) {
      const i64 tc = live[p] ? (n_first + nloc[p]) * (i64)a.C + c[p] : 0;
      dgv[p] = a.dig[tc];
    } else if (live[p]) {
      const i64 n = n_first + nloc[p];
      load_state_k2<HWT>(a.states + ((a.shared ? 0 : n * (i64)a.C) + c[p]) * a.HW, a.HW, ktot[p], idx0[p], idx1[p]);
    }
    yyn[p] = a.yy[live[p] ? n_first + nloc[p] : 0];
  }
  {
    if (STAGEB) {
      const double2 *src = (const double2 *)(a.Bm + n_first * a.H);
      double2 *dst = (double2 *)Bs;
      const int n2 = rows * a.H / 2;
      for (int i = threadIdx.x; i < n2; i += BS) dst[i] = src[i];
    }
    if (stage_dg)
      for (int i = threadIdx.x; i < a.H; i += BS) DGs[i] = a.D1[i];
  }
  PairEntry pe[PPT];
#pragma unroll
  for (int p = 0; p < PPT; p++) {
    if (a.dig && live[p]) {
      ktot[p] = dig_k(dgv[p]);
      idx0[p] = dig_idx(dgv[p], 0);
      idx1[p] = dig_idx(dgv[p], 1);
    }
    over[p] = live[p] && ktot[p] > 2;
    const bool pair = live[p] && ktot[p] == 2;
    pe[p] = a.PT[pair ? (i64)idx0[p] * a.H + idx1[p] : 0];
  }
  const int shard = (int)(blockIdx.x & (LIST_SHARDS - 1));
  if (APPEND)
    append_begin<BS, PPT>(lo, shard, tv, over, ovf_buf, ovf_ctl);
  else
    lds_barrier();
  const double4 *D1t = stage_dg ? DGs : a.D1;
  const double s = a.s2inv;
#pragma unroll
  for (int p = 0; p < PPT; p++) {
    if (live[p] && !over[p]) {
      const int k = ktot[p];
      const double *Bn = STAGEB ? Bs + (size_t)nloc[p] * a.H
                                : a.Bm + (n_first + nloc[p]) * (i64)a.H;
      const double val = sssc_k2_value(k, idx0[p], idx1[p], D1t, Bn, pe[p], yyn[p], s, a.err);
      unsigned fl = 0;
      const i64 n = n_first + nloc[p];
      a.lpj_out[n * a.ldo + a.col0 + c[p]] = clamp_lpj(val, fl);
      if (fl) {
        atomicOr(&a.flags[n], fl);
        atomicOr(&a.err[1], 1);
      }
    }
  }
  if (APPEND) append_end<BS>(lo, shard, ovf_buf, ovf_ctl, a.err);
}

template <int HWT, int W, bool CEN = false>
__global__ __launch_bounds__(64 * W, W == 4 ? 2 : 1) void sssc_stats_wave_kernel(SsscArgs a, ListOut lo, PairBins pb, int stage,
                                                                                const OvfRec *__restrict__ rec = nullptr,
                                                                                const int rec_kmax = 8) {
  a.s2inv = a.dpar[DP_S2INV];
  extern __shared__ double wrows[];
  __shared__ int bcnt[PB_MAX_BINS];
  constexpr int OVB = 64;
  __shared__ int obuf[W][2 * OVB];
  const int H = a.H, lane = lane_id(), wave = wave_id_uniform();
  double *rowS = wrows + (size_t)wave * 2 * H, *rowZ = rowS + H;
  double *accS = wrows + (size_t)W * 2 * H, *accZ = accS + H, *accD = accZ + H;
  double *rowB = accD + H + (size_t)wave * H;
  double4 *d1s = (double4 *)(accD + H + (size_t)W * H);
  const bool binned = pb.ent != nullptr;
  for (int i = threadIdx.x; i < 3 * H; i += 64 * W) accS[i] = 0.0;
  if (HWT > 0 || stage)
    for (int i = threadIdx.x; i < H; i += 64 * W) d1s[i] = a.D1[i];
  if (binned)
    for (int i = threadIdx.x; i < pb.nb; i += 64 * W) bcnt[i] = CEN ? pb.gcnt[(size_t)i * pb.nwg + blockIdx.x] : 0;
  __syncthreads();
  const int shard = (int)(blockIdx.x & (LIST_SHARDS - 1));
  const double s = a.s2inv;
  int ocnt = 0;
  auto flush_obuf = [&]() {
    int base = 0;
    if (lane == 0) base = atomicAdd(&lo.counts[shard], ocnt);
    base = __shfl(base, 0, 64);
    for (int i = lane; i < ocnt; i += 64) {
      const int pos = base + i;
      if (pos >= 0 && pos < lo.cap)
        lo.items[(i64)shard * lo.cap + pos] = obuf[wave][i];
      else
        atomicOr(a.err, EVO_ERR_LIST_FULL);
    }
    ocnt = 0;
    lds_wave_fence();
  };
  constexpr bool PF = HWT > 0;
  constexpr int HB = PF ? HWT : 1;
  struct Pre {
    double rmax, rsum, B[HB], l[4];
    u64 d[4];
  };
  auto issue = [&](i64 nn, Pre &p) {
    p.rmax = a.rowmax[nn];
    p.rsum = a.rowsum[nn];
    const double *Bnn = a.Bm + nn * H;
#pragma unroll
    for (int i = 0; i < HB; i++) {
      const int h = lane + 64 * i;
      p.B[i] = Bnn[h < H ? h : H - 1];
    }
    const double *lpn = a.lpj_in + nn * a.ldo + a.col0;
    const u64 *dgn = a.dig + nn * (i64)a.C;
#pragma unroll
    for (int u = 0; u < 4; u++) {
      const int c = 64 * u + lane, cc = c < a.C ? c : 0;
      p.d[u] = dgn[cc];
      p.l[u] = lpn[cc];
    }
  };
  const i64 n_first = (i64)blockIdx.x * W + wave, n_stride = (i64)gridDim.x * W;
  Pre cur = {};
  if (PF && n_first < a.N) issue(n_first, cur);
  for (i64 n = n_first; n < a.N; n += n_stride) {
    const i64 n_next = n + n_stride < a.N ? n + n_stride : n;
    for (int h = lane; h < 2 * H; h += 64) rowS[h] = 0.0;
    double rmax, rsum;
    const double *Bn = a.Bm + n * H;
    if (PF) {
      rmax = cur.rmax;
      rsum = cur.rsum + EVO_F64_TINY;
#pragma unroll
      for (int i = 0; i < HB; i++) {
        const int h = lane + 64 * i;
        if (h < H) rowB[h] = cur.B[i];
      }
      Bn = rowB;
    } else {
      rmax = a.rowmax[n];
      rsum = a.rowsum[n] + EVO_F64_TINY;
      if (stage) {
        for (int h = lane; h < H; h += 64) rowB[h] = Bn[h];
        Bn = rowB;
      }
    }
    const double4 *D1t = (PF || stage) ? d1s : a.D1;
    const double *lp = a.lpj_in + n * a.ldo + a.col0;
    lds_wave_fence();
    auto group = [&](const int c0, auto first_tag) {
      constexpr bool first = decltype(first_tag)::value;
      constexpr int RG = 4;
      bool live[RG];
      int k[RG], idx0[RG], idx1[RG];
      double l[RG];
#pragma unroll
      for (int u = 0; u < RG; u++) {
        const int c = c0 + 64 * u + lane;
        live[u] = c < a.C;
        k[u] = idx0[u] = idx1[u] = 0;
        l[u] = 0.0;
        if (first) {
          const u64 d = cur.d[u];
          k[u] = live[u] ? dig_k(d) : 0;
          idx0[u] = dig_idx(d, 0);
          idx1[u] = dig_idx(d, 1);
          l[u] = cur.l[u];
        } else {
          if (a.dig) {
            const u64 d = a.dig[n * (i64)a.C + (live[u] ? c : 0)];
            k[u] = live[u] ? dig_k(d) : 0;
            idx0[u] = dig_idx(d, 0);
            idx1[u] = dig_idx(d, 1);
          } else if (live[u]) {
            load_state_k2<0>(a.states + (n * (i64)a.C + c) * a.HW, a.HW, k[u], idx0[u], idx1[u]);
          }
          l[u] = lp[live[u] ? c : 0];
        }
      }
      bool over[RG];
      int n_over = 0, my_off[RG];
#pragma unroll
      for (int u = 0; u < RG; u++) {
        over[u] = live[u] && k[u] > 2;
        my_off[u] = 0;
        if (!CEN) {
          const u64 om = __ballot(over[u]);
          my_off[u] = n_over + __popcll(om & ((1ull << lane) - 1ull));
          n_over += __popcll(om);
        }
      }
      const bool o_direct = !CEN && n_over > OVB;
      int obase = 0;
      if (o_direct) {
        if (lane == 0) obase = atomicAdd(&lo.counts[shard], n_over);
        obase = __shfl(obase, 0, 64);
      }
      int ofirst = -1;
      bool omore = false;
      OvfRec orec = {};
      if (CEN) {
#pragma unroll
        for (int u = RG - 1; u >= 0; u--)
          if (over[u] && k[u] <= rec_kmax) {
            omore = ofirst >= 0;
            ofirst = u;
          }
      }
      bool act[RG], pair[RG];
      PairEntry pe[RG];
#pragma unroll
      for (int u = 0; u < RG; u++) {
        act[u] = live[u] && !over[u] && k[u] > 0;
        pair[u] = act[u] && k[u] == 2;
        pe[u] = a.PT[pair[u] ? (i64)idx0[u] * H + idx1[u] : 0];
      }
      if (CEN) {
        const OvfRec *rp = rec + (size_t)(n * a.C) + (ofirst >= 0 ? c0 + 64 * ofirst + lane : 0);
        const uint4 *r4 = (const uint4 *)rp;
        uint4 w0 = r4[0], w1 = r4[1], w2 = r4[2], w3 = r4[3], w4 = r4[4], w5 = r4[5];
        *(uint4 *)orec.idx = w0;
        orec.qn = __hiloint2double((int)w1.y, (int)w1.x);
        orec.z[0] = __hiloint2double((int)w2.y, (int)w2.x);
        orec.z[1] = __hiloint2double((int)w2.w, (int)w2.z);
        orec.z[2] = __hiloint2double((int)w3.y, (int)w3.x);
        orec.z[3] = __hiloint2double((int)w3.w, (int)w3.z);
        orec.z[4] = __hiloint2double((int)w4.y, (int)w4.x);
        orec.z[5] = __hiloint2double((int)w4.w, (int)w4.z);
        orec.z[6] = __hiloint2double((int)w5.y, (int)w5.x);
        orec.z[7] = __hiloint2double((int)w5.w, (int)w5.z);
      }
      if (first) {
        __builtin_amdgcn_sched_barrier(0);
        issue(n_next, cur);
        __builtin_amdgcn_sched_barrier(0);
      }
#pragma unroll
      for (int u = 0; u < RG; u++) {
        const double q = act[u] ? exp(l[u] + (0.0 - rmax)) : 0.0;
        if (q != 0.0) {
          const double qn = q / rsum;
          const double4 d0 = D1t[idx0[u]];
          const double b0 = Bn[idx0[u]];
          double g01 = 0.0, l00 = d0.w, l01 = 0.0, l10 = 0.0, l11 = 0.0, mu1 = 0.0, g11 = 0.0, bb1 = 0.0;
          if (pair[u]) {
            const double4 d1 = D1t[idx1[u]];
            g01 = pe[u].g01;
            l00 = pe[u].l00;
            l01 = pe[u].l01;
            l10 = pe[u].l10;
            l11 = pe[u].l11;
            mu1 = d1.x;
            g11 = d1.z;
            bb1 = Bn[idx1[u]];
            if (pair_singular_lam(pe[u].l00)) atomicOr(a.err, 2);
          }
          const double mu0 = d0.x;
          const double v0 = b0 - d0.z * mu0 - g01 * mu1;
          const double v1 = bb1 - g01 * mu0 - g11 * mu1;
          const double k0 = s * (l00 * v0 + l01 * v1) + mu0;
          const double k1 = s * (l10 * v0 + l11 * v1) + mu1;
          unsafeAtomicAdd(&rowS[idx0[u]], qn);
          unsafeAtomicAdd(&rowZ[idx0[u]], qn * k0);
          unsafeAtomicAdd(&accD[idx0[u]], qn * (l00 + k0 * k0));
          if (pair[u]) {
            unsafeAtomicAdd(&rowS[idx1[u]], qn);
            unsafeAtomicAdd(&rowZ[idx1[u]], qn * k1);
            unsafeAtomicAdd(&accD[idx1[u]], qn * (l11 + k1 * k1));
            const double pq = qn, pv = qn * (l01 + k0 * k1);
            const i64 o01 = (i64)idx0[u] * H + idx1[u];
            if (!binned) {
              unsafeAtomicAdd(&a.xss[o01], pq);
              unsafeAtomicAdd(&a.xszsz[o01], pv);
            } else {
              const double pw = qn * (l10 + k1 * k0);
              if (!pb_append(pb, bcnt, blockIdx.x, H, idx0[u], idx1[u], pq, pv, pw)) {
                unsafeAtomicAdd(&a.xss_o[o01], pq);
                unsafeAtomicAdd(&a.xszsz_o[o01], pv);
                unsafeAtomicAdd(&a.xszsz_o[(i64)idx1[u] * H + idx0[u]], pw);
              }
            }
          }
        }
      }
      if (CEN) {
        auto add_rec = [&](const OvfRec &r, int kk) {
          if (r.qn != 0.0) {
#pragma unroll
            for (int i = 0; i < 8; i++)
              if (i < kk) {
                const int h = (int)r.idx[i];
                unsafeAtomicAdd(&rowS[h], r.qn);
                unsafeAtomicAdd(&rowZ[h], r.z[i]);
// ... 17 lines not shown
      }
      if (!CEN && n_over) {
#pragma unroll
        for (int u = 0; u < RG; u++)
          if (over[u]) {
            const int e = (int)(n * a.C + c0 + 64 * u + lane);
            if (o_direct) {
              const int pos = obase + my_off[u];
              if (pos >= 0 && pos < lo.cap)
                lo.items[(i64)shard * lo.cap + pos] = e;
              else
                atomicOr(a.err, EVO_ERR_LIST_FULL);
            } else {
              obuf[wave][ocnt + my_off[u]] = e;
            }
          }
        if (!o_direct) {
          ocnt += n_over;
          if (ocnt >= OVB) {
            lds_wave_fence();
            flush_obuf();
          }
        }
      }
    };
    if (PF) {
      group(0, std::true_type{});
      for (int c0 = 4 * 64; c0 < a.C; c0 += 4 * 64) group(c0, std::false_type{});
    } else {
      for (int c0 = 0; c0 < a.C; c0 += 4 * 64) group(c0, std::false_type{});
    }
    lds_wave_fence();
    double *es = a.Es + n * a.ldE, *ez = a.Ez + n * a.ldE;
    for (int h = lane; h < H; h += 64) {
      const double vs = rowS[h], vz = rowZ[h];
      es[h] = vs;
      ez[h] = vz;
      if (vs != 0.0) {
        unsafeAtomicAdd(&accS[h], vs);
        unsafeAtomicAdd(&accZ[h], vz);
      }
    }
    lds_wave_fence();
  }
  if (ocnt) flush_obuf();
  __syncthreads();
  double *sl = a.cs + (size_t)(blockIdx.x % CS_SLICES) * 3 * H;
  for (int h = threadIdx.x; h < H; h += 64 * W) {
    if (accS[h] != 0.0) {
      unsafeAtomicAdd(&sl[h], accS[h]);
      unsafeAtomicAdd(&sl[H + h], accZ[h]);
    }
    if (accD[h] != 0.0) unsafeAtomicAdd(&sl[2 * H + h], accD[h]);
  }
  if (binned)
    for (int i = threadIdx.x; i < pb.nb; i += 64 * W) {
      const int cnt = bcnt[i];
      pb.gcnt[(size_t)i * pb.nwg + blockIdx.x] = cnt < pb.cap ? cnt : pb.cap;
    }
}

__global__ __launch_bounds__(256) void finish_sym_kernel(double *__restrict__ xss,
                                                              const double *__restrict__ xs, int H) {
  const i64 t = (i64)blockIdx.x * 256 + threadIdx.x;
  if (t >= (i64)H * H) return;
  const int i = (int)(t / H), j = (int)(t - (i64)i * H);
  if (i == j)
    xss[t] = xs[i];
  else if (i > j)
    xss[t] = xss[(i64)j * H + i];
}

template <int BAR>
__device__ __forceinline__ void big_bar() {
  if (BAR == 2)
    __syncthreads();
  else if (BAR == 1)
    lds_barrier();
  else
    lds_wave_fence();
}
template <int BAR, class F>
__device__ __forceinline__ void rows_of(const int lane, const int k, F f) {
  if (BAR == 2) {
    for (int r = lane; r < k; r += 64) f(r);
  } else {
    if (lane < k) f(lane);
  }
}
template <int BAR>
__device__ __forceinline__ int wave_idamax(const double *M, const int k, const int p, const int lane, double &m) {
  double v = -1.0;
  int vr = 0x7fffffff;
  rows_of<BAR>(lane, k, [&](int r) {
    if (r >= p) {
      const double x = fabs(M[r * k + p]);
      if (x > v || vr == 0x7fffffff) {
        v = x;
        vr = r;
      }
    }
  });
  m = wave_max(v);
  if (BAR == 2) return (int)wave_min_u32(v == m ? (unsigned)vr : 0x7fffffffu);
  return __ffsll((long long)__ballot(v == m)) - 1;
}
// ... 466 lines not shown
      if (q == 0.0) continue;
      qn = q / (a.rowsum[n] + EVO_F64_TINY);
    }
    double val = 0.0;
    int rc;
    if (huge) {
      int slot = -1;
      if (lane == 0) {
        int s0 = (int)(blockIdx.x % (unsigned)a.huge_slots);
        for (int tries = 0; tries < (1 << 22); tries++) {
          if (atomicCAS(&a.huge_ctl[s0], 0, 1) == 0) {
            slot = s0;
            break;
          }
          s0 = s0 + 1 < a.huge_slots ? s0 + 1 : 0;
          __builtin_amdgcn_s_sleep(8);
        }
      }
      slot = __shfl(slot, 0, 64);
      if (slot < 0) {
        if (lane == 0) {
          atomicOr(a.err, 1);
          if (MODE == 0) a.lpj_out[n * a.ldo + a.col0 + c] = EVO_F64_MIN;
        }
        continue;
      }
      __threadfence();
      BigLds Gl;
      Gl.carve(a.huge + (size_t)slot * big_slot_doubles(a.huge_kc), k);
      big_scan(sp, a.HW, k, Gl.idx, lane);
      __syncthreads();
      rc = big_solve<MODE, 2>(a, n, k, Gl, lane, exact, a.Bm + n * a.H, a.yy[n], val);
      if (MODE == 1) big_emit<2>(a, n, k, Gl, lane, qn);
      __syncthreads();
      __threadfence();
      if (lane == 0) atomicExch(&a.huge_ctl[slot], 0);
    } else {
      rc = big_solve<MODE, 1>(a, n, k, L, lane, exact, a.Bm + n * a.H, a.yy[n], val);
      if (MODE == 1) big_emit<1>(a, n, k, L, lane, qn);
    }
    if (MODE == 0) {
      if (lane == 0) {
        unsigned fl = 0;
        a.lpj_out[n * a.ldo + a.col0 + c] = clamp_lpj(rc == 2 ? __builtin_inf() : val, fl);
        if (fl) {
          atomicOr(&a.flags[n], fl);
          atomicOr(&a.err[1], 1);
        }
      }
    }
  }
}

__global__ __launch_bounds__(256) void sssc_finish_kernel(double *__restrict__ xss, double *__restrict__ xszsz,
                                                          double *__restrict__ xs, double *__restrict__ xsz,
                                                          const double *__restrict__ part, int nblk, int H,
                                                          const double *__restrict__ y2sum, double *__restrict__ y2out,
                                                          int D, const double *__restrict__ xss_o,
                                                          const double *__restrict__ xszsz_o,
                                                          const PairEntry *__restrict__ PT, PairBins pb,
                                                          TailArgs ta = TailArgs{}) {
  if (ta.tail && blockIdx.x == gridDim.x - 1) {
    tail_body(ta);
    return;
  }
  const i64 t = (i64)blockIdx.x * 256 + threadIdx.x;
  if (t < D) y2out[t] = y2sum[t];
  if (t >= (i64)H * H) return;
  const int i = (int)(t / H), j = (int)(t - (i64)i * H);
  const bool wide = H >= 3;
  if (i == j) {
    const double s = ordered_strided_sum(part + i, 3 * (i64)H, nblk);
    xs[i] = s;
    xss[t] = s;
  }
  if (wide ? (j == (i + 1 == H ? 0 : i + 1)) : (i == j)) xsz[i] = ordered_strided_sum(part + H + i, 3 * (i64)H, nblk);
  if (wide ? (j == (i + 2 >= H ? i + 2 - H : i + 2)) : (i == j))
    xszsz[(i64)i * H + i] = ordered_strided_sum(part + 2 * H + i, 3 * (i64)H, nblk);
  if (i < j) {
    const i64 tl = (i64)j * H + i;
    const double uss = xss[t], u = xszsz[t];
    double lower = u;
    if (PT && uss != 0.0) {
      const PairEntry pe = PT[t];
      lower = u + (pe.l10 - pe.l01) * uss;
    }
    double bq = 0.0, bu = 0.0, bl = 0.0;
    if (pb.part) pb_collect(pb, H, i, j, bq, bu, bl);
    const double ss = uss + xss_o[t] + bq;
    xss[t] = ss;
    xss[tl] = ss;
    xszsz[t] = u + xszsz_o[t] + bu;
    xszsz[tl] = lower + xszsz_o[tl] + bl;
  }
}

__global__ __launch_bounds__(256) void set_diag_kernel(double *__restrict__ M, const double *__restrict__ d, int H) {
  const int h = blockIdx.x * 256 + threadIdx.x;
  if (h < H) M[(i64)h * H + h] = d[h];
}

__global__ __launch_bounds__(256) void sssc_tables_kernel(const double *__restrict__ G, const double *__restrict__ Psi,
                                                          const double *__restrict__ mus,
                                                          const double *__restrict__ pil_bar,
                                                          const double *__restrict__ dpar, int H,
                                                          double4 *__restrict__ D1, PairEntry *__restrict__ PT,
                                                          double2 *__restrict__ GP, double4 *__restrict__ DG,
                                                          int *__restrict__ sing_gen, int gen) {
  const i64 t = (i64)blockIdx.x * 256 + threadIdx.x;
  if (t >= (i64)H * H) return;
  const int h0 = (int)(t / H), h1 = (int)(t - (i64)h0 * H);
  const double s = dpar[DP_S2INV];
  GP[t] = make_double2(G[t], Psi[t]);
  if (h0 == h1) {
    const double g = G[t], p = Psi[t];
    DG[h0] = make_double4(mus[h0], pil_bar[h0], g, p);
    const double T = 1.0 + s * p * g;
    double4 d = make_double4(mus[h0], pil_bar[h0] - 0.5 * log(fabs(T)), g, p / T);
    if (p == 0.0) {
      d.y = __builtin_inf();
      d.w = (s * g != 0.0) ? 1.0 / (s * g) : 0.0;
      atomicMax(sing_gen, gen);
    } else if (!(p > 0.0) && s * g + 1.0 / p == 0.0) {
      d.y = __builtin_inf();
      d.w = 0.0;
      atomicMax(sing_gen, gen);
    }
    D1[h0] = d;
    return;
  }
  if (h0 > h1) return;
  const double G00 = G[(i64)h0 * H + h0], G11 = G[(i64)h1 * H + h1], G01 = G[t], G10 = G[(i64)h1 * H + h0];
  const double P00 = Psi[(i64)h0 * H + h0], P11 = Psi[(i64)h1 * H + h1], P01 = Psi[t], P10 = Psi[(i64)h1 * H + h0];
  const double T00 = 1.0 + s * (P00 * G00 + P01 * G10);
  const double T01 = s * (P00 * G01 + P01 * G11);
  const double T10 = s * (P10 * G00 + P11 * G10);
  const double T11 = 1.0 + s * (P10 * G01 + P11 * G11);
  const double det = T00 * T11 - T01 * T10;
  const double rdet = 1.0 / det;
  PairEntry e;
  e.g01 = G01;
  e.L = pil_bar[h0] + pil_bar[h1] - 0.5 * log(fabs(det));
  e.l00 = (T11 * P00 - T01 * P10) * rdet;
  e.l01 = (T11 * P01 - T01 * P11) * rdet;
  e.l10 = (T00 * P10 - T10 * P00) * rdet;
// ... 15 lines not shown
```

evo_amd/csrc/pair_bins.hpp:

```cpp
#pragma once
#include "common.hpp"

#define PB_TILE 4096
#define PB_MAX_BINS 256
#define PB_NSH_MAX 16
#define PB_RTHREADS 1024
struct PairBins {
  double4 *ent;
  int *gcnt;
  double *part;
  int cap, nb, rf, nwg;
  int nsh;
};
__device__ __forceinline__ int pb_fold(int i, int H) { return i < H - 2 - i ? i : H - 2 - i; }

__device__ __forceinline__ bool pb_append(const PairBins &pb, int *bcnt, int wg, int H, int i, int j, double q,
                                          double vu, double vl) {
  const int f = pb_fold(i, H);
  const int bin = f / pb.rf;
  const int pos = atomicAdd(&bcnt[bin], 1);
  if (pos >= pb.cap) return false;
  const int r = 2 * (f - bin * pb.rf) + (i != f ? 1 : 0);
  const size_t at = ((size_t)bin * pb.nwg + wg) * pb.cap + pos;
  pb.ent[at] = make_double4(q, vu, vl, __longlong_as_double((long long)(((unsigned)r << 16) | (unsigned)j)));
  return true;
}

__global__ __launch_bounds__(PB_RTHREADS) void pair_bins_reduce_kernel(PairBins pb, int H, int accumulate) {
  extern __shared__ double pb_tile[];
  constexpr int NW = PB_RTHREADS / 64;
  __shared__ int pre_sh[NW][65];
  const int NSH = pb.nsh;
  const int bin = blockIdx.x / NSH, sh = blockIdx.x - bin * NSH;
  const int slots = 2 * pb.rf * H;
  double *tq = pb_tile, *tu = pb_tile + slots, *tl = pb_tile + 2 * slots;
  for (int i = threadIdx.x; i < 3 * slots; i += PB_RTHREADS) pb_tile[i] = 0.0;
  lds_barrier();
  const int lane = lane_id(), wave = wave_id_uniform();
  for (int j0 = 0; sh + NSH * (wave + NW * j0) < pb.nwg; j0 += 64) {
    const int w = sh + NSH * (wave + NW * (j0 + lane));
    int n = 0;
    if (w < pb.nwg) {
      const size_t reg = (size_t)bin * pb.nwg + w;
      n = pb.gcnt[reg];
      if (n > pb.cap) n = pb.cap;
      if (n != 0) pb.gcnt[reg] = 0;
    }
    int incl = n;
#pragma unroll
    for (int o = 1; o < 64; o <<= 1) {
      const int t = __shfl_up(incl, o, 64);
      if (lane >= o) incl += t;
    }
    pre_sh[wave][lane + 1] = incl;
    if (lane == 0) pre_sh[wave][0] = 0;
    lds_wave_fence();
    const int T = pre_sh[wave][64];
    for (int t0 = 0; t0 < T; t0 += 256) {
      double4 v[4];
      bool on[4];
#pragma unroll
      for (int u = 0; u < 4; u++) {
        const int t = t0 + 64 * u + lane;
        on[u] = t < T;
        int lo = 0, hi = 64;
#pragma unroll
        for (int it = 0; it < 6; it++) {
          const int mid = (lo + hi) >> 1;
          if (pre_sh[wave][mid] <= t)
            lo = mid;
          else
            hi = mid;
        }
        const int wr = sh + NSH * (wave + NW * (j0 + lo));
        const size_t at = on[u] ? ((size_t)bin * pb.nwg + wr) * pb.cap + (t - pre_sh[wave][lo]) : 0;
        v[u] = pb.ent[at];
      }
#pragma unroll
      for (int u = 0; u < 4; u++)
        if (on[u]) {
          const unsigned k = (unsigned)__double_as_longlong(v[u].w);
          const int t = (int)(k >> 16) * H + (int)(k & 0xFFFFu);
          unsafeAtomicAdd(&tq[t], v[u].x);
          unsafeAtomicAdd(&tu[t], v[u].y);
          unsafeAtomicAdd(&tl[t], v[u].z);
        }
    }
    lds_wave_fence();
  }
  lds_barrier();
  double *out = pb.part + (size_t)blockIdx.x * 3 * slots;
  for (int i = threadIdx.x; i < 3 * slots; i += PB_RTHREADS) out[i] = accumulate ? out[i] + pb_tile[i] : pb_tile[i];
}

__device__ __forceinline__ void pb_collect(const PairBins &pb, int H, int i, int j, double &bq, double &bu, double &bl) {
  const int f = pb_fold(i, H), bin = f / pb.rf;
  const int slots = 2 * pb.rf * H;
  const int slot = (2 * (f - bin * pb.rf) + (i != f ? 1 : 0)) * H + j;
  const double *p = pb.part + (size_t)bin * pb.nsh * 3 * slots + slot;
  bq = bu = bl = 0.0;
  for (int sh = 0; sh < pb.nsh; sh++, p += 3 * slots) {
    bq += p[0];
    bu += p[slots];
    bl += p[2 * slots];
  }
}
```

include/evo_amd.h:

```cpp
#ifndef EVO_AMD_H
#define EVO_AMD_H

#include <stddef.h>
#include <stdint.h>

#ifdef __cplusplus
extern "C" {
#endif

#define EVOAMD_ABI_VERSION 1

enum {
  EVOAMD_OK = 0,
  EVOAMD_E_INVALID = -1,
  EVOAMD_E_HIP = -2,
  EVOAMD_E_NODEVICE = -3,
  EVOAMD_E_RCCL = -4,
  EVOAMD_E_KLIMIT = -5,
  EVOAMD_E_SINGULAR = -6
};

enum { EVOAMD_MODEL_BSC = 0, EVOAMD_MODEL_SSSC = 1 };

#define EVOAMD_KCAP 64
// ... 127 lines not shown
                            int fill_all, int add_noise, int64_t counters[4]);
int evoamd_download_posterior_samples(evoamd_ctx *ctx, int what, void *out);

enum { EVOAMD_LLE_S = 0, EVOAMD_LLE_INSIDE = 1, EVOAMD_LLE_LOG_R = 2, EVOAMD_LLE_LPJ = 3 };
int evoamd_loglik_estimate(evoamd_ctx *ctx, int n_samples, uint64_t seed, uint64_t first_index, double prior_mix,
                           int keep_draws, double *ll_out, double *F_out, double *mass_out, double *ess_out,
                           int32_t *n_outside_out, int64_t counters[2], double *sum_out);
int evoamd_download_loglik_draws(evoamd_ctx *ctx, int what, void *out);

int evoamd_patches_merge_samples(evoamd_ctx *ctx, int H, int W, int C, int ph, int pw, int shift, int method,
                                 int t0, int n_draws, double *imgs_out, double *mean_out, double *std_out);
int evoamd_patches_merge_predictive(evoamd_ctx *ctx, int H, int W, int C, int ph, int pw, int shift, int what,
                                    double *img_out);

int evoamd_remap_latents(evoamd_ctx *ctx, const int32_t *index, int H_new, int32_t *n_replaced_out, int64_t *sum_out);
int evoamd_adopt_remapped_states(evoamd_ctx *ctx);
int evoamd_latent_map_counts(evoamd_ctx *ctx, int64_t *counts_out);

int evoamd_comm_unique_id(uint8_t id_out[128]);
int evoamd_comm_init(evoamd_ctx *ctx, const uint8_t id[128], int rank, int world);
int evoamd_comm_allreduce_host(evoamd_ctx *ctx, double *buf, int64_t n, int op);
int evoamd_comm_destroy(evoamd_ctx *ctx);

enum {
  EVOAMD_K_LPJ_RESIDENT = 0,
  EVOAMD_K_LPJ_CANDIDATES = 1,
  EVOAMD_K_LPJ_OVERFLOW = 2,
  EVOAMD_K_ROW_LSE = 3,
  EVOAMD_K_VARY_KN = 4,
  EVOAMD_K_STATS = 5,
  EVOAMD_K_STATS_OVERFLOW = 6,
  EVOAMD_K_GEMM = 7,
  EVOAMD_K_EVOLVE = 8,
  EVOAMD_K_MISC = 9,
  EVOAMD_K_MSTEP_DEVICE = 10,
  EVOAMD_K_LPJ_PASS = 11,
  EVOAMD_K_STATS_PASS = 12,
  EVOAMD_K_LPJ_K3_4 = 13,
  EVOAMD_K_LPJ_K5_8 = 14,
  EVOAMD_K_LPJ_K9PLUS = 15,
  EVOAMD_K_STATS_K3_4 = 16,
  EVOAMD_K_STATS_K5_8 = 17,
  EVOAMD_K_STATS_K9PLUS = 18,
  EVOAMD_K_ALLREDUCE = 19,
  EVOAMD_K_ESTEP_FUSED = 20,
  EVOAMD_K_PATCHES = 21,
  EVOAMD_K_INIT_STATES = 22,
  EVOAMD_K_POSTERIOR_SAMPLE = 23,
  EVOAMD_K_SEED_STATES = 24,
  EVOAMD_K_LOGLIK_PROPOSAL = 25,
  EVOAMD_K_LOGLIK_LPJ = 26,
  EVOAMD_K_LOGLIK_FOLD = 27,
  EVOAMD_K_REMAP = 28,
  EVOAMD_K_COUNT = 29
};
int evoamd_timing_enable(evoamd_ctx *ctx, int on);
int evoamd_timing_reset(evoamd_ctx *ctx);
int evoamd_kernel_time_ms(evoamd_ctx *ctx, int kernel_class, double *avg_ms, int64_t *launches);
const char *evoamd_kernel_name(int kernel_class);

#ifdef __cplusplus
}
#endif
#endif
```

Baseline: 5.155 billion state evals/s.

## Cache per-state kappa from the LPJ pass and reuse it in SSSC stats

During the SSSC LPJ pass, per-state kappa values (double2) are now written for resident and candidate states. They are carried through the selection step via vary_kn, and generation counters track whether they are still valid. When the cache is valid, a specialised stats kernel reads the cached values instead of recomputing the per-state solve. Pair-state contributions go into a fourth pair-bin plane, and an extra finish pass corrects the diagonal and upper/lower cross terms. This adds N*(S+Cmax) double2 of memory, extra writes in the LPJ and selection kernels, and more bookkeeping, in exchange for cheaper M-step statistics at large N*S.

```diff
diff --git a/evo_amd/_lib.py b/evo_amd/_lib.py
--- a/evo_amd/_lib.py
+++ b/evo_amd/_lib.py
@@ -35,7 +35,7 @@
     "patches": 21, "init_states": 22,
 }
 KERNEL_IDS_EXTRA = {"posterior_sample": 23, "seed_states": 24, "loglik_proposal": 25, "loglik_lpj": 26, "loglik_fold": 27,
-                    "remap_latents": 28}
+                    "remap_latents": 28, "stats_kappa": 29}
 
 
 def kernel_id(name):
diff --git a/evo_amd/csrc/evo_amd.hip b/evo_amd/csrc/evo_amd.hip
--- a/evo_amd/csrc/evo_amd.hip
+++ b/evo_amd/csrc/evo_amd.hip
@@ -143,6 +143,7 @@
   KID_LLE_LPJ,
   KID_LLE_FOLD,
   KID_REMAP,
+  KID_STATS_KAPPA,
   KID_COUNT
 };
 
@@ -402,6 +403,11 @@
   unsigned long long kn_gen = 1, census_gen = 0;
   int census_opt = 1;
   int merge_small = 1;
+  DevBuf<double2> kap, cand_kap;
+  unsigned long long kap_gen = ~0ull, cand_kap_gen = ~0ull;
+  bool kap_carry = false;
+  int stats_kappa = 1;
+  int kappa_min = 16384;
   int stats_flat = 0;
   int fused_opt = 0;
   DevBuf<double> rowF;
@@ -479,6 +485,7 @@
   c->have_data = c->have_params = c->have_cand = c->rows_fresh = c->acc_clean = c->clist_clean = false;
   c->h_theta_fresh = c->theta_bak_valid = c->yrec_valid = c->rec_in_stats = c->keep_x_valid = c->kn_lost = false;
   c->lists_clean = c->need_known = c->cand_from_device = false;
+  c->kap_gen = c->cand_kap_gen = ~0ull, c->kap_carry = false;
   if (c->model == EVOAMD_MODEL_SSSC) c->last_estep_fused = false;
   drop_stats_products(c);
   c->pred_N = 0;
@@ -523,10 +530,13 @@
 static void made_theta_mailbox(evoamd_ctx *c, bool holds_theta) { c->h_theta_fresh = holds_theta; }
 enum KnBy { KN_BY_CALLER, KN_BY_SELECTION };
 static void on_kn_changed(evoamd_ctx *c, KnBy by) {
+  c->kap_carry = by == KN_BY_SELECTION && c->kap_gen == c->gen && c->cand_kap_gen == c->gen;
   c->gen++;
   c->kn_gen++;
   if (by == KN_BY_CALLER) c->need_known = false;
 }
+static void made_kappa(evoamd_ctx *c, bool written) { c->kap_gen = written ? c->gen : ~0ull; }
+static void made_cand_kappa(evoamd_ctx *c, bool written) { c->cand_kap_gen = written ? c->gen : ~0ull; }
 static void on_kn_complete(evoamd_ctx *c) { c->kn_lost = false; }
 static void on_kn_init_begun(evoamd_ctx *c) {
   c->kn_lost = true, c->kn_refill = 0;
@@ -558,8 +568,10 @@
     c->pending_skip = (c->pending_skip | skipped) & ~served;
   }
 }
-static void made_selection(evoamd_ctx *c, bool census_cleared, bool acc_zeroed) {
+static void made_selection(evoamd_ctx *c, bool census_cleared, bool acc_zeroed, bool kappa_carried) {
   made_row_stats(c);
+  if (kappa_carried && c->kap_carry) c->kap_gen = c->gen;
+  c->kap_carry = false;
   if (census_cleared) {
     c->clist_clean = true;
     c->census_skip = 0;
@@ -570,13 +582,14 @@
 static void on_census_claimed(evoamd_ctx *c) { c->clist_clean = false, c->census_skip = 0; }
 static void made_census(evoamd_ctx *c) { c->census_gen = c->kn_gen; }
 static void on_census_poisoned(evoamd_ctx *c) { c->kn_gen++; }
-static void on_cand_installed(evoamd_ctx *c, bool near_parents) { c->cand_from_device = near_parents; }
+static void on_cand_installed(evoamd_ctx *c, bool near_parents) { c->cand_from_device = near_parents, c->cand_kap_gen = ~0ull; }
 static void made_cand_lpj(evoamd_ctx *c) { c->have_cand = true; }
-static void drop_cand_batch(evoamd_ctx *c) { c->have_cand = false, c->cand_from_device = false; }
+static void drop_cand_batch(evoamd_ctx *c) { c->have_cand = false, c->cand_from_device = false, c->cand_kap_gen = ~0ull; }
 static void made_fused_estep(evoamd_ctx *c, bool inkernel_census) {
   on_kn_changed(c, KN_BY_SELECTION);
   if (inkernel_census) made_census(c);
   made_row_stats(c);
+  c->kap_carry = false;
   c->have_cand = false, c->cand_from_device = true;
   on_estep_route(c, true);
 }
@@ -728,9 +741,10 @@
                         (const void *)sssc_stats_wave_kernel<2, 4>,  (const void *)sssc_stats_wave_kernel<4, 4>,
                         (const void *)sssc_stats_wave_kernel<8, 4>,  (const void *)sssc_stats_wave_kernel<16, 4>,
                         (const void *)sssc_stats_wave_kernel<0, 1>,  (const void *)sssc_stats_wave_kernel<0, 8>,
-                        (const void *)sssc_stats_wave_kernel<0, 16>};
+                        (const void *)sssc_stats_wave_kernel<0, 16>, (const void *)sssc_stats_wave_kernel<1, 4, true, true>};
     for (const void *f : wk) HIP_TRY(hipFuncSetAttribute(f, hipFuncAttributeMaxDynamicSharedMemorySize, 150 * 1024));
-    HIP_TRY(hipFuncSetAttribute((const void *)pair_bins_reduce_kernel, hipFuncAttributeMaxDynamicSharedMemorySize, 3 * PB_TILE * 8));
+    HIP_TRY(hipFuncSetAttribute((const void *)pair_bins_reduce_kernel<3>, hipFuncAttributeMaxDynamicSharedMemorySize, 3 * PB_TILE * 8));
+    HIP_TRY(hipFuncSetAttribute((const void *)pair_bins_reduce_kernel<4>, hipFuncAttributeMaxDynamicSharedMemorySize, 4 * PB_TILE * 8));
     HIP_TRY(hipFuncSetAttribute((const void *)sssc_small_kernel<4, 1, 2, 256>, hipFuncAttributeMaxDynamicSharedMemorySize, 120 * 1024));
     HIP_TRY(hipFuncSetAttribute((const void *)sssc_small_kernel<8, 1, 2, 256>, hipFuncAttributeMaxDynamicSharedMemorySize, 120 * 1024));
   }
@@ -898,13 +912,21 @@
     {"state_digest", OPT_BOOL(use_digest), opt_flag},
     {"inverse_spd", OPT_BOOL(spd_inverse), opt_flag},
 };
+static const OptionRow OPTIONS_LATER[] = {
+  {"stats_kappa", OPT_INT(stats_kappa), nullptr, 0, 2, nullptr, "stats_kappa: 0 (never), 1 (automatic) or 2 (wherever the shape allows it)"},
+  {"stats_kappa_min", OPT_INT(kappa_min), nullptr, 0, 1 << 20, nullptr, "stats_kappa_min: 0 .. 1048576 (x 1024 resident states)"},
+};
 #undef OPT_INT
 #undef OPT_BOOL
 
 extern "C" int evoamd_set_option(evoamd_ctx *c, const char *name, int value) {
   REQUIRE(c && name, "bad arguments");
   on_option(c);
-  for (const OptionRow &o : OPTIONS) {
+  std::vector<const OptionRow *> rows;
+  for (const OptionRow &o : OPTIONS) rows.push_back(&o);
+  for (const OptionRow &o : OPTIONS_LATER) rows.push_back(&o);
+  for (const OptionRow *row : rows) {
+    const OptionRow &o = *row;
     if (strcmp(name, o.name) != 0) continue;
     if (o.err && !(o.accepts ? o.accepts(value) : (value >= o.lo && value <= o.hi))) return fail(EVOAMD_E_INVALID, "%s", o.err);
     const int v = o.norm ? o.norm(value) : value;
@@ -973,8 +995,9 @@
     pb.nwg = c->bins_nwg;
     pb.nsh = std::max((i64)N * S >= (i64)8 << 20 ? 8 : 4, std::min(PB_NSH_MAX, 256 / std::max(1, pb.nb)));
     pb.cap = (int)std::max<i64>(64, (i64)scale * cdiv((i64)N * S, (i64)pb.nb * pb.nwg));
+    pb.planes = 3;
     const size_t ne = (size_t)pb.nb * pb.nwg * pb.cap;
-    if (c->pb_ent.try_alloc(ne) && c->pb_part.try_alloc((size_t)pb.nb * pb.nsh * 3 * 2 * pb.rf * H) &&
+    if (c->pb_ent.try_alloc(ne) && c->pb_part.try_alloc((size_t)pb.nb * pb.nsh * (c->model == EVOAMD_MODEL_SSSC ? 4 : 3) * 2 * pb.rf * H) &&
         c->pb_gcnt.try_alloc((size_t)pb.nb * pb.nwg)) {
       pb.ent = c->pb_ent;
       pb.part = c->pb_part;
@@ -1011,6 +1034,10 @@
   return 0;
 }
 
+static bool kappa_wanted(const evoamd_ctx *c) {
+  return c->stats_kappa == 2 || (c->stats_kappa == 1 && c->N * (i64)c->S >= (i64)c->kappa_min * 1024);
+}
+
 static int configure_validate(const evoamd_ctx *c, int model, i64 N, int D, int H, int S, int S_perm, int Cmax) {
   REQUIRE(model == EVOAMD_MODEL_BSC || model == EVOAMD_MODEL_SSSC, "unknown model");
   REQUIRE(N > 0 && D > 0 && H > 0 && S > 0, "N, D, H, S must be positive");
@@ -1036,7 +1063,7 @@
   c->ldY = (model == EVOAMD_MODEL_SSSC) ? D + 3 * H : D;
   c->f32 = model == EVOAMD_MODEL_BSC && c->f32_opt;
   c->acc_n = acc_len(c);
-  c->pre_n = (model == EVOAMD_MODEL_SSSC) ? 4 + (i64)CS_SLICES * 3 * H : 4 + (i64)BSC_CS_SLICES * H;
+  c->pre_n = (model == EVOAMD_MODEL_SSSC) ? 4 + (i64)CS_SLICES * 4 * H : 4 + (i64)BSC_CS_SLICES * H;
   c->ovf_n = c->pre_n + ((model == EVOAMD_MODEL_SSSC) ? 2 * (i64)H * H : 0);
 }
 
@@ -1174,6 +1201,15 @@
     TRY(c->clist.alloc(3 * list_cap(c->N * (i64)c->S) * LIST_SHARDS));
     TRY(c->clist_n.alloc(4 * LIST_SHARDS));
     TRY(c->ovf_rec.alloc((size_t)c->N * c->S));
+  }
+  c->kap.reset();
+  c->cand_kap.reset();
+  if (c->census_opt && kappa_wanted(c) && c->dig && (c->H % 2) == 0 && !c->sssc_prec32 &&
+      (size_t)(4 * 2 + 4) * c->H * sizeof(double) <= 150 * 1024) {
+    if (!c->kap.try_alloc((size_t)c->N * c->S) || !c->cand_kap.try_alloc((size_t)c->N * c->Cmax)) {
+      c->kap.reset();
+      c->cand_kap.reset();
+    }
   }
   return 0;
 }
@@ -2113,6 +2149,10 @@
   return ((size_t)(1024 / C + 2) * H + (H <= 512 ? (size_t)4 * H : 0)) * sizeof(double);
 }
 
+static bool kappa_shape_ok(const evoamd_ctx *c) {
+  return kappa_wanted(c) && c->kap && c->cand_kap && census_mode(c) && (c->H % 2) == 0 && !c->sssc_prec32;
+}
+
 enum LpjRoute {
   LPJ_MASKED,
   LPJ_CENSUS,
@@ -2143,6 +2183,7 @@
   bool few4;
   bool k8;
   bool few_dense;
+  bool kappa;
 };
 
 static void lpj_plan(const evoamd_ctx *c, const SsscArgs &a, int tag, const LevelHints &lv, int kid_main, LpjPlan &p) {
@@ -2175,6 +2216,9 @@
     p.main = LPJ_MAIN_SMALL;
     p.grid = cdiv(p.total, 512);
   }
+  p.kappa = kappa_shape_ok(c) && !lv.levels_only &&
+            (p.main == LPJ_MAIN_CENSUS || p.main == LPJ_MAIN_STAGED || p.main == LPJ_MAIN_UNSTAGED) &&
+            ((tag == 0 && a.states == c->states && a.C == c->S) || (tag == 1 && a.states == c->cand && a.C == c->Cmax));
   p.few4 = p.route != LPJ_ROUND2 && few_above4(c, lv);
   p.k8 = p.route == LPJ_ROUND2 && use_k8_kernel(c, lv);
   p.few_dense = p.route == LPJ_ROUND2 && few_dense_states(c, lv);
@@ -2284,10 +2328,14 @@
 }
 
 template <int TAG>
-static int launch_sssc_lpj(evoamd_ctx *c, const SsscArgs &a, int kid_main, const LevelHints &lv) {
+static int launch_sssc_lpj(evoamd_ctx *c, const SsscArgs &a_in, int kid_main, const LevelHints &lv) {
   TRY(zero_lists(c));
   LpjPlan p;
-  lpj_plan(c, a, TAG, lv, kid_main, p);
+  lpj_plan(c, a_in, TAG, lv, kid_main, p);
+  SsscArgs a = a_in;
+  if (p.kappa) a.kap_out = TAG == 0 ? c->kap.get() : c->cand_kap.get();
+  if (TAG == 0 && a.states == c->states) made_kappa(c, p.kappa);
+  if (TAG == 1 && a.states == c->cand) made_cand_kappa(c, p.kappa);
   if (p.route == LPJ_MASKED) return lpj_sssc_masked(c, a, p);
   if (p.route == LPJ_CENSUS) TRY(ensure_census(c));
   TRY(lpj_sssc_main<TAG>(c, a, p));
@@ -2501,18 +2549,20 @@
     int *cl_n = census_mode(c) ? c->clist_n : nullptr;
     const i64 zero_n = c->fold_clear ? (i64)(c->ovf_n + c->acc_n) : 0;
     if (!c->fold_clear) cl_n = nullptr;
+    const bool kap_carry = c->kap_carry && c->kap && c->cand_kap;
     with_spl(c->S, [&](auto spl) {
       with_cpl(c->Cmax, [&](auto cpl) {
         vary_kn_kernel<decltype(spl)::value, decltype(cpl)::value><<<cdiv(c->N, 4), 256, 0, c->stream>>>(
             c->states, c->lpj, c->cand, c->cand_lpj, c->cand_counts, c->N, c->S, c->S_perm, c->HW, c->Cmax, Mprime, c->rowmax,
             c->rowsum, c->partial, c->list_n, 4 * LIST_SHARDS, c->dig, c->cand_dig, (c->use_digest && c->dig) ? 1 : 0,
-            c->pending_skip, c->err, cl_n, 4 * LIST_SHARDS, c->census_skip, c->acc_base, zero_n);
+            c->pending_skip, c->err, cl_n, 4 * LIST_SHARDS, c->census_skip, c->acc_base, zero_n,
+            kap_carry ? c->kap.get() : nullptr, kap_carry ? c->cand_kap.get() : nullptr);
       });
     });
     reduce3_partials_kernel<<<1, R3_THREADS, 0, c->stream>>>(c->partial, cdiv(c->N, 4), c->dpar);
     HIP_TRY(hipGetLastError());
     DBG_SYNC(c, "vary_kn");
-    made_selection(c, cl_n != nullptr, zero_n > 0);
+    made_selection(c, cl_n != nullptr, zero_n > 0, kap_carry);
   }
   if (sums_out) {
     HIP_TRY(hipMemcpyAsync(sums_out, c->dpar + DP_ECNT0, 2 * sizeof(double), hipMemcpyDeviceToHost, c->stream));
@@ -3112,6 +3162,7 @@
   int waves;
   bool census;
   bool bsc_wave;
+  bool kappa;
 };
 
 struct StatsBlock {
@@ -3214,6 +3265,8 @@
                 : ((size_t)(4 * 2 + 3) * p.H * sizeof(double) <= 150 * 1024 ? 4 : 1);
   p.census = census_mode(c) && !p.masked && p.waves == 4;
   if (p.census) nchunks = 1;
+  p.kappa = p.census && kappa_shape_ok(c) && c->kap_gen == c->gen && !c->stats_flat && c->stats_stage != 0 &&
+            (c->stats_waves == 0 || c->stats_waves == 4);
   p.rows_per_chunk = (i64)cdiv(p.nblk, nchunks) * p.rpb;
   p.nchunks = nchunks = (int)cdiv(p.N, p.rows_per_chunk);
   p.second_stream = p.fork_gemm || nchunks > 1;
@@ -3259,7 +3312,7 @@
   DBG_SYNC(c, "bsc stats (wave)");
   TRY(rows_written(c, p, fl));
   if (bsc_pb.ent) {
-    pair_bins_reduce_kernel<<<bsc_pb.nb * bsc_pb.nsh, PB_RTHREADS, (size_t)3 * 2 * bsc_pb.rf * H * sizeof(double), c->stream>>>(
+    pair_bins_reduce_kernel<3><<<bsc_pb.nb * bsc_pb.nsh, PB_RTHREADS, (size_t)3 * 2 * bsc_pb.rf * H * sizeof(double), c->stream>>>(
         bsc_pb, H, 0);
     HIP_TRY(hipGetLastError());
     made_bins_clean(c);
@@ -3412,6 +3465,18 @@
   if (stage) lds = lds_staged;
   const int per_cu = stats_per_cu(lds + lds_static, 32 / Wv);
   SpanGuard g(c, KID_STATS);
+  if (p.kappa) {
+    SpanGuard gk(c, KID_STATS_KAPPA);
+    const size_t ldk = (size_t)(4 * 2 + 4) * H * sizeof(double);
+    const int per_cu_k = stats_per_cu(ldk + lds_static, 32 / 4);
+    int kgrid = (int)std::min<i64>(cdiv(nc, 4), (i64)c->n_cu * per_cu_k * 4);
+    if (pb.ent && kgrid > pb.nwg) kgrid = pb.nwg;
+    PB_GRID_CHECK(pb, kgrid);
+    sssc_stats_wave_kernel<1, 4, true, true><<<kgrid, 256, ldk, c->stream>>>(sc, o1, pb, 1, c->ovf_rec, eb.few4 ? 4 : 8);
+    HIP_TRY(hipGetLastError());
+    DBG_SYNC(c, "sssc stats main (kappa)");
+    return 0;
+  }
   int sgrid = (int)std::min<i64>(cdiv(nc, Wv), (i64)c->n_cu * per_cu * 4);
   if (pb.ent && sgrid > pb.nwg) sgrid = pb.nwg;
   PB_GRID_CHECK(pb, sgrid);
@@ -3514,7 +3579,10 @@
   TRY(rows_written(c, p, fl));
   if (pb.ent) {
     SpanGuard g(c, KID_STATS);
-    pair_bins_reduce_kernel<<<pb.nb * pb.nsh, PB_RTHREADS, (size_t)3 * 2 * pb.rf * p.H * sizeof(double), c->stream>>>(pb, p.H, blk.ci > 0);
+    if (pb.planes == 4)
+      pair_bins_reduce_kernel<4><<<pb.nb * pb.nsh, PB_RTHREADS, (size_t)4 * 2 * pb.rf * p.H * sizeof(double), c->stream>>>(pb, p.H, blk.ci > 0);
+    else
+      pair_bins_reduce_kernel<3><<<pb.nb * pb.nsh, PB_RTHREADS, (size_t)3 * 2 * pb.rf * p.H * sizeof(double), c->stream>>>(pb, p.H, blk.ci > 0);
     HIP_TRY(hipGetLastError());
     made_bins_clean(c);
     DBG_SYNC(c, "pair bins reduce");
@@ -3552,9 +3620,14 @@
       ta = make_tail_args(c, a, N, p.census, fl.skipped);
       fl.tail_done = true;
     }
+    if (p.kappa)
+      sssc_finish_kernel<<<H, 256, 0, c->stream>>>(c->acc + a.xss, c->acc + a.xszsz, c->acc + a.xs, c->acc + a.xsz, sa.cs, CS_SLICES,
+                                                   H, c->y2sum, c->acc + a.y2, D, sa.xss_o, sa.xszsz_o, c->PT, fl.pb, TailArgs{}, 2,
+                                                   c->err, c->D1, sa.cs, sa.cs1);
     sssc_finish_kernel<<<cdiv(nthr, 256) + (fl.tail_done ? 1 : 0), 256, 0, c->stream>>>(
         c->acc + a.xss, c->acc + a.xszsz, c->acc + a.xs, c->acc + a.xsz, masked ? c->colpart : sa.cs,
-        masked ? p.nblk : CS_SLICES, H, c->y2sum, c->acc + a.y2, D, sa.xss_o, sa.xszsz_o, masked ? nullptr : c->PT, fl.pb, ta);
+        masked ? p.nblk : CS_SLICES, H, c->y2sum, c->acc + a.y2, D, sa.xss_o, sa.xszsz_o, masked ? nullptr : c->PT, fl.pb, ta,
+        p.kappa ? 1 : 0, c->err);
   }
   HIP_TRY(hipGetLastError());
   DBG_SYNC(c, "colsum + finish");
@@ -3655,6 +3728,8 @@
   sa.xss_o = c->acc_base + c->pre_n;
   sa.xszsz_o = c->acc_base + c->pre_n + (size_t)H * H;
   if (!p.masked) sa.cs = c->acc_base + 4;
+  sa.cs1 = c->acc_base + 4 + (size_t)CS_SLICES * 3 * H;
+  if (p.kappa) sa.kap_in = c->kap;
   ep.ls = es3c_lists(c, (int)list_cap(N * (i64)c->S));
   levels_for(c, p.lv, ep.need);
   return zero_lists(c);
@@ -3687,6 +3762,7 @@
   const double *Ywp = c->Y;
   int ldwp = c->ldY;
   if (c->model == EVOAMD_MODEL_SSSC && !p.masked && stats_bins_pay(c)) fl.pb = c->pbins;
+  if (p.kappa) fl.pb.planes = 4;
   for (int ci = 0; ci < p.nchunks; ci++) {
     const i64 n0 = (i64)ci * p.rows_per_chunk;
     const i64 nc = std::min<i64>(p.rows_per_chunk, p.N - n0);
@@ -5383,6 +5459,7 @@
                                          "lpj_pass",     "stats_pass",     "lpj_k3_4",     "lpj_k5_8", "lpj_k9plus",
                                          "stats_k3_4",   "stats_k5_8",     "stats_k9plus", "allreduce",    "estep_fused",
                                          "patches",      "init_states",    "posterior_sample", "seed_states",
-                                         "loglik_proposal", "loglik_lpj",  "loglik_fold",     "remap_latents"};
+                                         "loglik_proposal", "loglik_lpj",  "loglik_fold",     "remap_latents",
+                                         "stats_kappa"};
   return (kid >= 0 && kid < KID_COUNT) ? names[kid] : "?";
 }
diff --git a/evo_amd/csrc/kernels_common.hpp b/evo_amd/csrc/kernels_common.hpp
--- a/evo_amd/csrc/kernels_common.hpp
+++ b/evo_amd/csrc/kernels_common.hpp
@@ -430,7 +430,9 @@
                                                       u64 *__restrict__ dig, const u64 *__restrict__ cand_dig,
                                                       int dig_dedup, int skipped_mask, int *__restrict__ err,
                                                       int *__restrict__ clist_n = nullptr, int n_clist = 0, int census_skip = 0,
-                                                      double *__restrict__ zero_ptr = nullptr, i64 zero_n = 0) {
+                                                      double *__restrict__ zero_ptr = nullptr, i64 zero_n = 0,
+                                                      double2 *__restrict__ kap = nullptr,
+                                                      const double2 *__restrict__ cand_kap = nullptr) {
   __shared__ int blk_uniq[4], blk_sub[4];
   if (blockIdx.x == 0 && list_n)
     clear_lists_checked(list_n, n_list, skipped_mask, err);
@@ -605,6 +607,7 @@
           }
           lpj_n[wi] = new_v[wave][j];
           if (dig) dig[n * (i64)S + wi] = cand_dig[n * (i64)Cmax + bi];
+          if (kap) kap[n * (i64)S + wi] = cand_kap[n * (i64)Cmax + bi];
         }
       }
       for (int j = 0; j < g; j++) {
diff --git a/evo_amd/csrc/kernels_sssc.hpp b/evo_amd/csrc/kernels_sssc.hpp
--- a/evo_amd/csrc/kernels_sssc.hpp
+++ b/evo_amd/csrc/kernels_sssc.hpp
@@ -42,11 +42,14 @@
   double *lpj_out;
   int ldo, col0;
   unsigned *flags;
+  double2 *kap_out;
+  const double2 *kap_in;
   const double *lpj_in;
   const double *rowmax, *rowsum;
   double *Es, *Ez, *Ed;
   int ldE;
   double *cs;
+  double *cs1;
   double *xss, *xszsz;
   double *xss_o, *xszsz_o;
   int *err;
@@ -645,8 +648,9 @@
   for (int i = threadIdx.x; i < n; i += BS) lo.items[dst + i] = buf[i];
 }
 
-__device__ __forceinline__ double sssc_k2_value(const int k, const int idx0, const int idx1, const double4 *D1t, const double *Bn,
-                                                const PairEntry &pe, const double yyn, const double s, int *err) {
+__device__ __forceinline__ double sssc_k2_value_kappa(const int k, const int idx0, const int idx1, const double4 *D1t,
+                                                      const double *Bn, const PairEntry &pe, const double yyn, const double s,
+                                                      int *err, double &kap0, double &kap1) {
 #pragma clang fp contract(off)
   double4 d0 = make_double4(0.0, 0.0, 0.0, 0.0), d1 = make_double4(0.0, 0.0, 0.0, 0.0);
   double b0 = 0.0, b1 = 0.0, g01 = 0.0, L = 0.0, l00 = 0.0, l01 = 0.0, l10 = 0.0, l11 = 0.0;
@@ -672,7 +676,14 @@
   const double rr = fma(-d1.x, b1 + v1, fma(-d0.x, b0 + v0, yyn));
   const double t0 = fma(l01, v1, l00 * v0), t1 = fma(l11, v1, l10 * v0);
   const double quad = fma(v1, t1, v0 * t0);
+  kap0 = fma(s, t0, d0.x);
+  kap1 = fma(s, t1, d1.x);
   return fma(-0.5 * s, fma(-s, quad, rr), L);
+}
+__device__ __forceinline__ double sssc_k2_value(const int k, const int idx0, const int idx1, const double4 *D1t, const double *Bn,
+                                                const PairEntry &pe, const double yyn, const double s, int *err) {
+  double kap0, kap1;
+  return sssc_k2_value_kappa(k, idx0, idx1, D1t, Bn, pe, yyn, s, err, kap0, kap1);
 }
 
 template <int TAG, int BS, int HWT, int PPT, bool APPEND = true, bool STAGEB = true>
@@ -758,10 +769,18 @@
       const int k = ktot[p];
       const double *Bn = STAGEB ? Bs + (size_t)nloc[p] * a.H
                                 : a.Bm + (n_first + nloc[p]) * (i64)a.H;
-      const double val = sssc_k2_value(k, idx0[p], idx1[p], D1t, Bn, pe[p], yyn[p], s, a.err);
+      double kap0, kap1;
+      const double val = sssc_k2_value_kappa(k, idx0[p], idx1[p], D1t, Bn, pe[p], yyn[p], s, a.err, kap0, kap1);
       unsigned fl = 0;
       const i64 n = n_first + nloc[p];
       a.lpj_out[n * a.ldo + a.col0 + c[p]] = clamp_lpj(val, fl);
+      if (a.kap_out) {
+        typedef double kap_v2 __attribute__((ext_vector_type(2)));
+        kap_v2 kv;
+        kv.x = kap0;
+        kv.y = kap1;
+        __builtin_nontemporal_store(kv, (kap_v2 *)&a.kap_out[n * a.C + c[p]]);
+      }
       if (fl) {
         atomicOr(&a.flags[n], fl);
         atomicOr(&a.err[1], 1);
@@ -771,7 +790,7 @@
   if (APPEND) append_end<BS>(lo, shard, ovf_buf, ovf_ctl, a.err);
 }
 
-template <int HWT, int W, bool CEN = false>
+template <int HWT, int W, bool CEN = false, bool KAP = false>
 __global__ __launch_bounds__(64 * W, W == 4 ? 2 : 1) void sssc_stats_wave_kernel(SsscArgs a, ListOut lo, PairBins pb, int stage,
                                                                                 const OvfRec *__restrict__ rec = nullptr,
                                                                                 const int rec_kmax = 8) {
@@ -783,11 +802,12 @@
   const int H = a.H, lane = lane_id(), wave = wave_id_uniform();
   double *rowS = wrows + (size_t)wave * 2 * H, *rowZ = rowS + H;
   double *accS = wrows + (size_t)W * 2 * H, *accZ = accS + H, *accD = accZ + H;
+  double *accS1 = accD + H;
   double *rowB = accD + H + (size_t)wave * H;
   double4 *d1s = (double4 *)(accD + H + (size_t)W * H);
   const bool binned = pb.ent != nullptr;
-  for (int i = threadIdx.x; i < 3 * H; i += 64 * W) accS[i] = 0.0;
-  if (HWT > 0 || stage)
+  for (int i = threadIdx.x; i < (KAP ? 4 : 3) * H; i += 64 * W) accS[i] = 0.0;
+  if (!KAP && (HWT > 0 || stage))
     for (int i = threadIdx.x; i < H; i += 64 * W) d1s[i] = a.D1[i];
   if (binned)
     for (int i = threadIdx.x; i < pb.nb; i += 64 * W) bcnt[i] = CEN ? pb.gcnt[(size_t)i * pb.nwg + blockIdx.x] : 0;
@@ -810,19 +830,22 @@
     lds_wave_fence();
   };
   constexpr bool PF = HWT > 0;
-  constexpr int HB = PF ? HWT : 1;
+  constexpr int HB = (PF && !KAP) ? HWT : 1;
   struct Pre {
     double rmax, rsum, B[HB], l[4];
     u64 d[4];
+    double2 kp[KAP ? 4 : 1];
   };
   auto issue = [&](i64 nn, Pre &p) {
     p.rmax = a.rowmax[nn];
     p.rsum = a.rowsum[nn];
-    const double *Bnn = a.Bm + nn * H;
-#pragma unroll
-    for (int i = 0; i < HB; i++) {
-      const int h = lane + 64 * i;
-      p.B[i] = Bnn[h < H ? h : H - 1];
+    if (!KAP) {
+      const double *Bnn = a.Bm + nn * H;
+#pragma unroll
+      for (int i = 0; i < HB; i++) {
+        const int h = lane + 64 * i;
+        p.B[i] = Bnn[h < H ? h : H - 1];
+      }
     }
     const double *lpn = a.lpj_in + nn * a.ldo + a.col0;
     const u64 *dgn = a.dig + nn * (i64)a.C;
@@ -831,6 +854,7 @@
       const int c = 64 * u + lane, cc = c < a.C ? c : 0;
       p.d[u] = dgn[cc];
       p.l[u] = lpn[cc];
+      if (KAP) p.kp[u] = a.kap_in[nn * (i64)a.C + cc];
     }
   };
   const i64 n_first = (i64)blockIdx.x * W + wave, n_stride = (i64)gridDim.x * W;
@@ -844,12 +868,14 @@
     if (PF) {
       rmax = cur.rmax;
       rsum = cur.rsum + EVO_F64_TINY;
-#pragma unroll
-      for (int i = 0; i < HB; i++) {
-        const int h = lane + 64 * i;
-        if (h < H) rowB[h] = cur.B[i];
-      }
-      Bn = rowB;
+      if (!KAP) {
+#pragma unroll
+        for (int i = 0; i < HB; i++) {
+          const int h = lane + 64 * i;
+          if (h < H) rowB[h] = cur.B[i];
+        }
+        Bn = rowB;
+      }
     } else {
       rmax = a.rowmax[n];
       rsum = a.rowsum[n] + EVO_F64_TINY;
@@ -867,18 +893,21 @@
       bool live[RG];
       int k[RG], idx0[RG], idx1[RG];
       double l[RG];
+      double2 kp[RG];
 #pragma unroll
       for (int u = 0; u < RG; u++) {
         const int c = c0 + 64 * u + lane;
         live[u] = c < a.C;
         k[u] = idx0[u] = idx1[u] = 0;
         l[u] = 0.0;
+        kp[u] = make_double2(0.0, 0.0);
         if (first) {
           const u64 d = cur.d[u];
           k[u] = live[u] ? dig_k(d) : 0;
           idx0[u] = dig_idx(d, 0);
           idx1[u] = dig_idx(d, 1);
           l[u] = cur.l[u];
+          if (KAP) kp[u] = cur.kp[u];
         } else {
           if (a.dig) {
             const u64 d = a.dig[n * (i64)a.C + (live[u] ? c : 0)];
@@ -889,6 +918,7 @@
             load_state_k2<0>(a.states + (n * (i64)a.C + c) * a.HW, a.HW, k[u], idx0[u], idx1[u]);
           }
           l[u] = lp[live[u] ? c : 0];
+          if (KAP) kp[u] = a.kap_in[n * (i64)a.C + (live[u] ? c : 0)];
         }
       }
       bool over[RG];
@@ -926,7 +956,7 @@
       for (int u = 0; u < RG; u++) {
         act[u] = live[u] && !over[u] && k[u] > 0;
         pair[u] = act[u] && k[u] == 2;
-        pe[u] = a.PT[pair[u] ? (i64)idx0[u] * H + idx1[u] : 0];
+        if (!KAP) pe[u] = a.PT[pair[u] ? (i64)idx0[u] * H + idx1[u] : 0];
       }
       if (CEN) {
         const OvfRec *rp = rec + (size_t)(n * a.C) + (ofirst >= 0 ? c0 + 64 * ofirst + lane : 0);
@@ -951,7 +981,28 @@
 #pragma unroll
       for (int u = 0; u < RG; u++) {
         const double q = act[u] ? exp(l[u] + (0.0 - rmax)) : 0.0;
-        if (q != 0.0) {
+        if (KAP) {
+          if (q != 0.0) {
+            const double qn = q / rsum;
+            const double k0 = kp[u].x, k1 = kp[u].y;
+            unsafeAtomicAdd(&rowS[idx0[u]], qn);
+            unsafeAtomicAdd(&rowZ[idx0[u]], qn * k0);
+            unsafeAtomicAdd(&accD[idx0[u]], qn * (k0 * k0));
+            if (pair[u]) {
+              unsafeAtomicAdd(&rowS[idx1[u]], qn);
+              unsafeAtomicAdd(&rowZ[idx1[u]], qn * k1);
+              unsafeAtomicAdd(&accD[idx1[u]], qn * (k1 * k1));
+              const double pv = qn * (k0 * k1);
+              if (!binned || !pb_append(pb, bcnt, blockIdx.x, H, idx0[u], idx1[u], qn, pv, 0.0, true)) {
+                const i64 o01 = (i64)idx0[u] * H + idx1[u];
+                unsafeAtomicAdd(&a.xss[o01], qn);
+                unsafeAtomicAdd(&a.xszsz[o01], pv);
+              }
+            } else {
+              unsafeAtomicAdd(&accS1[idx0[u]], qn);
+            }
+          }
+        } else if (q != 0.0) {
           const double qn = q / rsum;
           const double4 d0 = D1t[idx0[u]];
           const double b0 = Bn[idx0[u]];
@@ -1075,6 +1126,7 @@
       unsafeAtomicAdd(&sl[H + h], accZ[h]);
     }
     if (accD[h] != 0.0) unsafeAtomicAdd(&sl[2 * H + h], accD[h]);
+    if (KAP && accS1[h] != 0.0) unsafeAtomicAdd(&a.cs1[(size_t)(blockIdx.x % CS_SLICES) * H + h], accS1[h]);
   }
   if (binned)
     for (int i = threadIdx.x; i < pb.nb; i += 64 * W) {
@@ -1647,6 +1699,39 @@
   }
 }
 
+__device__ __forceinline__ void sssc_kappa_diag_body(const double *__restrict__ xss, double *__restrict__ cs,
+                                                     const double *__restrict__ cs1, int H,
+                                                     const double4 *__restrict__ D1,
+                                                     const PairEntry *__restrict__ PT, const PairBins &pb) {
+  __shared__ double red[256];
+  const int i = blockIdx.x;
+  double acc = 0.0;
+  for (int j = threadIdx.x; j < H; j += 256) {
+    if (j == i) continue;
+    const int lo = i < j ? i : j, hi = i < j ? j : i;
+    const i64 t = (i64)lo * H + hi;
+    double P = xss[t];
+    if (pb.part && pb.planes == 4) P += pb_collect_pair_q(pb, H, lo, hi);
+    if (P != 0.0) {
+      const PairEntry pe = PT[t];
+      acc += (i < j ? pe.l00 : pe.l11) * P;
+    }
+  }
+  red[threadIdx.x] = acc;
+  __syncthreads();
+  for (int o = 128; o > 0; o >>= 1) {
+    if ((int)threadIdx.x < o) red[threadIdx.x] += red[threadIdx.x + o];
+    __syncthreads();
+  }
+  if (threadIdx.x == 0) {
+    double p1 = 0.0;
+    for (int sl = 0; sl < CS_SLICES; sl++) p1 += cs1[(size_t)sl * H + i];
+    double add = red[0];
+    if (p1 != 0.0) add += D1[i].w * p1;
+    cs[2 * H + i] += add;
+  }
+}
+
 __global__ __launch_bounds__(256) void sssc_finish_kernel(double *__restrict__ xss, double *__restrict__ xszsz,
                                                           double *__restrict__ xs, double *__restrict__ xsz,
                                                           const double *__restrict__ part, int nblk, int H,
@@ -1654,7 +1739,15 @@
                                                           int D, const double *__restrict__ xss_o,
                                                           const double *__restrict__ xszsz_o,
                                                           const PairEntry *__restrict__ PT, PairBins pb,
-                                                          TailArgs ta = TailArgs{}) {
+                                                          TailArgs ta = TailArgs{}, int kappa = 0,
+                                                          int *__restrict__ err = nullptr,
+                                                          const double4 *__restrict__ D1 = nullptr,
+                                                          double *__restrict__ cs = nullptr,
+                                                          const double *__restrict__ cs1 = nullptr) {
+  if (kappa == 2) {
+    sssc_kappa_diag_body(xss, cs, cs1, H, D1, PT, pb);
+    return;
+  }
   if (ta.tail && blockIdx.x == gridDim.x - 1) {
     tail_body(ta);
     return;
@@ -1680,12 +1773,23 @@
       const PairEntry pe = PT[t];
       lower = u + (pe.l10 - pe.l01) * uss;
     }
-    double bq = 0.0, bu = 0.0, bl = 0.0;
-    if (pb.part) pb_collect(pb, H, i, j, bq, bu, bl);
-    const double ss = uss + xss_o[t] + bq;
+    double bq = 0.0, bu = 0.0, bl = 0.0, bp = 0.0;
+    if (pb.part) pb_collect(pb, H, i, j, bq, bu, bl, bp);
+    double upper = u;
+    if (kappa) {
+      const double P = uss + bp;
+      lower = u;
+      if (P != 0.0) {
+        const PairEntry pe = PT[t];
+        if (pair_singular_lam(pe.l00)) atomicOr(err, 2);
+        upper = u + pe.l01 * P;
+        lower = u + pe.l10 * P;
+      }
+    }
+    const double ss = uss + xss_o[t] + bq + bp;
     xss[t] = ss;
     xss[tl] = ss;
-    xszsz[t] = u + xszsz_o[t] + bu;
+    xszsz[t] = upper + xszsz_o[t] + bu;
     xszsz[tl] = lower + xszsz_o[tl] + bl;
   }
 }
diff --git a/evo_amd/csrc/pair_bins.hpp b/evo_amd/csrc/pair_bins.hpp
--- a/evo_amd/csrc/pair_bins.hpp
+++ b/evo_amd/csrc/pair_bins.hpp
@@ -11,21 +11,24 @@
   double *part;
   int cap, nb, rf, nwg;
   int nsh;
+  int planes;
 };
 __device__ __forceinline__ int pb_fold(int i, int H) { return i < H - 2 - i ? i : H - 2 - i; }
 
 __device__ __forceinline__ bool pb_append(const PairBins &pb, int *bcnt, int wg, int H, int i, int j, double q,
-                                          double vu, double vl) {
+                                          double vu, double vl, bool pair_state = false) {
   const int f = pb_fold(i, H);
   const int bin = f / pb.rf;
   const int pos = atomicAdd(&bcnt[bin], 1);
   if (pos >= pb.cap) return false;
   const int r = 2 * (f - bin * pb.rf) + (i != f ? 1 : 0);
   const size_t at = ((size_t)bin * pb.nwg + wg) * pb.cap + pos;
-  pb.ent[at] = make_double4(q, vu, vl, __longlong_as_double((long long)(((unsigned)r << 16) | (unsigned)j)));
+  const unsigned long long key = (pair_state ? 1ull << 32 : 0ull) | (((unsigned)r << 16) | (unsigned)j);
+  pb.ent[at] = make_double4(q, vu, vl, __longlong_as_double((long long)key));
   return true;
 }
 
+template <int NP>
 __global__ __launch_bounds__(PB_RTHREADS) void pair_bins_reduce_kernel(PairBins pb, int H, int accumulate) {
   extern __shared__ double pb_tile[];
   constexpr int NW = PB_RTHREADS / 64;
@@ -33,8 +36,8 @@
   const int NSH = pb.nsh;
   const int bin = blockIdx.x / NSH, sh = blockIdx.x - bin * NSH;
   const int slots = 2 * pb.rf * H;
-  double *tq = pb_tile, *tu = pb_tile + slots, *tl = pb_tile + 2 * slots;
-  for (int i = threadIdx.x; i < 3 * slots; i += PB_RTHREADS) pb_tile[i] = 0.0;
+  double *tq = pb_tile, *tu = pb_tile + slots, *tl = pb_tile + 2 * slots, *tp = pb_tile + (NP - 1) * slots;
+  for (int i = threadIdx.x; i < NP * slots; i += PB_RTHREADS) pb_tile[i] = 0.0;
   lds_barrier();
   const int lane = lane_id(), wave = wave_id_uniform();
   for (int j0 = 0; sh + NSH * (wave + NW * j0) < pb.nwg; j0 += 64) {
@@ -79,29 +82,52 @@
 #pragma unroll
       for (int u = 0; u < 4; u++)
         if (on[u]) {
-          const unsigned k = (unsigned)__double_as_longlong(v[u].w);
+          const unsigned long long key = (unsigned long long)__double_as_longlong(v[u].w);
+          const unsigned k = (unsigned)key;
           const int t = (int)(k >> 16) * H + (int)(k & 0xFFFFu);
-          unsafeAtomicAdd(&tq[t], v[u].x);
-          unsafeAtomicAdd(&tu[t], v[u].y);
-          unsafeAtomicAdd(&tl[t], v[u].z);
+          if (NP == 4 && (key >> 32) != 0ull) {
+            unsafeAtomicAdd(&tp[t], v[u].x);
+            unsafeAtomicAdd(&tu[t], v[u].y);
+            unsafeAtomicAdd(&tl[t], v[u].y);
+          } else {
+            unsafeAtomicAdd(&tq[t], v[u].x);
+            unsafeAtomicAdd(&tu[t], v[u].y);
+            unsafeAtomicAdd(&tl[t], v[u].z);
+          }
         }
     }
     lds_wave_fence();
   }
   lds_barrier();
-  double *out = pb.part + (size_t)blockIdx.x * 3 * slots;
-  for (int i = threadIdx.x; i < 3 * slots; i += PB_RTHREADS) out[i] = accumulate ? out[i] + pb_tile[i] : pb_tile[i];
+  double *out = pb.part + (size_t)blockIdx.x * NP * slots;
+  for (int i = threadIdx.x; i < NP * slots; i += PB_RTHREADS) out[i] = accumulate ? out[i] + pb_tile[i] : pb_tile[i];
 }
 
-__device__ __forceinline__ void pb_collect(const PairBins &pb, int H, int i, int j, double &bq, double &bu, double &bl) {
+__device__ __forceinline__ void pb_collect(const PairBins &pb, int H, int i, int j, double &bq, double &bu, double &bl,
+                                           double &bp) {
   const int f = pb_fold(i, H), bin = f / pb.rf;
   const int slots = 2 * pb.rf * H;
   const int slot = (2 * (f - bin * pb.rf) + (i != f ? 1 : 0)) * H + j;
-  const double *p = pb.part + (size_t)bin * pb.nsh * 3 * slots + slot;
-  bq = bu = bl = 0.0;
-  for (int sh = 0; sh < pb.nsh; sh++, p += 3 * slots) {
+  const int np = pb.planes == 4 ? 4 : 3;
+  const double *p = pb.part + (size_t)bin * pb.nsh * np * slots + slot;
+  bq = bu = bl = bp = 0.0;
+  for (int sh = 0; sh < pb.nsh; sh++, p += (size_t)np * slots) {
     bq += p[0];
     bu += p[slots];
     bl += p[2 * slots];
+    if (np == 4) bp += p[3 * slots];
   }
 }
+__device__ __forceinline__ void pb_collect(const PairBins &pb, int H, int i, int j, double &bq, double &bu, double &bl) {
+  double bp;
+  pb_collect(pb, H, i, j, bq, bu, bl, bp);
+}
+__device__ __forceinline__ double pb_collect_pair_q(const PairBins &pb, int H, int i, int j) {
+  const int f = pb_fold(i, H), bin = f / pb.rf;
+  const int slots = 2 * pb.rf * H;
+  const int slot = (2 * (f - bin * pb.rf) + (i != f ? 1 : 0)) * H + j;
+  const double *p = pb.part + (size_t)bin * pb.nsh * 4 * slots + 3 * (size_t)slots + slot;
+  double bp = 0.0;
+  for (int sh = 0; sh < pb.nsh; sh++, p += (size_t)4 * slots) bp += p[0];
+  return bp;
+}
diff --git a/include/evo_amd.h b/include/evo_amd.h
--- a/include/evo_amd.h
+++ b/include/evo_amd.h
@@ -203,7 +203,8 @@
   EVOAMD_K_LOGLIK_LPJ = 26,
   EVOAMD_K_LOGLIK_FOLD = 27,
   EVOAMD_K_REMAP = 28,
-  EVOAMD_K_COUNT = 29
+  EVOAMD_K_STATS_KAPPA = 29,
+  EVOAMD_K_COUNT = 30
 };
 int evoamd_timing_enable(evoamd_ctx *ctx, int on);
 int evoamd_timing_reset(evoamd_ctx *ctx);
```

Result: faster. 5.234 billion state evals/s, median of 6 (+1.5%).
